# estebanpw/repkiller

Measured on AMD Instinct MI355X. Metric: fragments/sec filtered + achieved HBM GB/s, 50M-frag human self-cmp, 1/2/4/8 GPU, higher is better.
Workload: dtype u64/f64; 1 GPU; cfg3: 50M fragments, 3 Gbp human-scale self-comparison; fragments_per_gpu=50000000, genome_bp=3000000000, parallelism=single GPU

## Files before the change

repkiller_amd/csrc/rk_api.hip:

```cpp
#include <algorithm>
#include <cstdio>
#include <cstdlib>
#include <cstring>
#include <string>
#include <vector>

#include "rk_ctx.h"

namespace rk {
const char *const kKernelNames[KID_COUNT] = {
    "k_prep_keys",     "k_digit_hist",      "k_digit_scatter", "k_gather_proc",
    "k_sort_keys",     "k_csr_fill_x",      "k_run_bounds",    "k_sweep_tile",
    "k_sweep_fast",    "k_sweep_fast_more", "k_sweep_wave",    "k_csr_fill_y",    "k_jump",
    "k_assign_gid",    "k_group_offsets",   "k_build_records",
    "k_sort_small",    "k_sort_groups_reg", "k_sort_groups_lds", "k_sort_groups_split",
    "k_emit",          "k_part (sharded)", "exchange (sharded)", "k_aux (sharded)",
    "k_row_keys (sharded)", "k_fill_y (sharded)", "k_y_results (sharded)", "k_x_own (sharded)",
    "k_merge_yx (sharded)", "k_sort_segments", "k_sweep_long32", "k_nw_order_hist",
    "k_onesweep", "k_nw_xchunk", "k_nw_fill_y", "k_nw_assign", "k_nw_xcount", "k_nw_x_bits",
    "k_heap_segments", "k_seg_fine (order)", "k_seg_fine (members)", "k_seg_fine (Y)",
};
}

namespace rk {

void collect_kernel_timing(rk_ctx *ctx) {
  g_ktimer = nullptr;
  if (ctx->kt.n) (void)hipEventSynchronize(ctx->kt.ev[2 * ctx->kt.n - 1]);
  if (ctx->kt.tier_counts) {
    const uint32_t nb = ctx->kt.tier_nblk;
    std::vector<uint32_t> h((size_t)KernelTimer::TIERS * nb);
    if (hipMemcpy(h.data(), ctx->kt.tier_counts, (size_t)GS_NTIER * nb * 4,
                  hipMemcpyDeviceToHost) == hipSuccess) {
      for (int u = 0; u < GS_NTIER; ++u) {
        double mem = 0;
        for (uint32_t b = 0; b < nb; ++b) mem += h[(size_t)u * nb + b];
        const int sl = ctx->kt.tier_slot[u];
        if (sl >= 0 && sl < ctx->kt.n) ctx->kt.bytes[sl] = 12.0 * mem;
        const int s2 = u == GS_NTIER - 1 ? ctx->kt.tier_slot[GS_NTIER] : -1;
        if (s2 >= 0 && s2 < ctx->kt.n) ctx->kt.bytes[s2] = 12.0 * mem;
      }
    }
    ctx->kt.tier_counts = nullptr;
  }
  bool any_units = false;
  for (int i = 0; i < ctx->kt.n; ++i) any_units |= ctx->kt.unit_bytes[i] > 0.0;
  if (any_units) {
    std::vector<uint32_t> u(ctx->kt.n);
    if (hipMemcpy(u.data(), ctx->kt.units, (size_t)ctx->kt.n * 4, hipMemcpyDeviceToHost) ==
        hipSuccess)
      for (int i = 0; i < ctx->kt.n; ++i)
        if (ctx->kt.unit_bytes[i] > 0.0) ctx->kt.bytes[i] = ctx->kt.unit_bytes[i] * u[i];
  }
  for (int i = 0; i < ctx->kt.n; ++i) {
    float ms = 0;
    if (hipEventElapsedTime(&ms, ctx->kt.ev[2 * i], ctx->kt.ev[2 * i + 1]) == hipSuccess) {
      const int k = ctx->kt.kid[i];
      ctx->kt_ms[k] += ms;
      ctx->kt_bytes[k] += ctx->kt.bytes[i];
      ctx->kt_launches[k]++;
    }
  }
  ctx->kt.n = 0;
}

int readback(rk_ctx *ctx, const uint32_t *dev, uint32_t count) {
  ++ctx->readbacks;
  HIPCHK(ctx, hipMemcpyAsync(ctx->host, dev, count * sizeof(uint32_t), hipMemcpyDeviceToHost,
                             ctx->stream));
  HIPCHK(ctx, hipStreamSynchronize(ctx->stream));
  return RK_OK;
}

int err_status(rk_ctx *ctx, uint32_t bits) {
  if (bits & ERRB_UB_BUCKET) {
    ctx->err = "xStart/10 >= vsize: the reference indexes FragmentsDatabase out of bounds "
               "(FragmentsDatabase.cpp:96-97)";
    return RK_E_UB_BUCKET;
  }
  if (bits & ERRB_UB_CENTER) {
    ctx->err = "a fragment centre probes past an occupancy array "
               "(SequenceOcupationList.cpp:17,80)";
    return RK_E_UB_CENTER;
  }
  if (bits & ERRB_INTERNAL) {
    ctx->err = "device consistency check failed";
    return RK_E_INTERNAL;
  }
  return RK_OK;
}

int resolve_axis(rk_ctx *ctx, const Axis &ax, SweepScratch sc, bool fast32, uint32_t *sweeps) {
  uint32_t *counters = sc.counters;
  uint8_t *rpend = sc.rpend;
  RunList rl{sc.runs, sc.wpend, 0, 0, fast32};
  build_runs(ax, rl, sc.dev_count, ctx->host + 128, ctx->stream);
  HIPCHK(ctx, hipGetLastError());
  if (!fast32) HIPCHK(ctx, hipMemsetAsync(rpend, 1, ax.m, ctx->stream));
  *sweeps = 0;
  for (;;) {
    if (*sweeps > ax.m + 2) {
      ctx->err = "occupancy sweeps did not converge";
      return RK_E_INTERNAL;
    }
    occupancy_sweep(ax, rl, rpend, counters, *sweeps == 0, ctx->stream);
    HIPCHK(ctx, hipGetLastError());
    ++*sweeps;
    static const uint32_t blind = [] {
      const char *e = getenv("RK_SWEEP_BLIND");
      const int v = e ? atoi(e) : 3;
      return (uint32_t)(v < 1 ? 1 : v > 8 ? 8 : v);
    }();
    if (*sweeps < blind && ax.m > 0) continue;
    int rc = readback(ctx, counters, PEND_WORDS);
    if (rc) return rc;
    uint64_t pending = 0;
    for (uint32_t k = 0; k < PEND_WORDS; ++k) pending += ctx->host[k];
    if (!pending) break;
  }
  return RK_OK;
}

__global__ void k_pend_flag(const uint32_t *counters, uint32_t *pend) {
  uint32_t s = 0;
  for (uint32_t k = threadIdx.x; k < PEND_WORDS; k += 64) s |= counters[k];
  if (__ballot(s != 0) && threadIdx.x == 0) *pend = 1u;
}

int resolve_axis_queued(rk_ctx *ctx, const Axis &ax, SweepScratch sc, uint32_t sweeps,
                        uint32_t *pend, uint32_t *junk) {
  if (!ax.m) return RK_OK;
  RunList rl{sc.runs, sc.wpend, 0, 0, true};
  build_runs(ax, rl, sc.dev_count, ctx->host + 128, ctx->stream);
  for (uint32_t s = 0; s < sweeps; ++s)
    occupancy_sweep(ax, rl, sc.rpend, junk && s + 1 < sweeps ? junk : sc.counters, s == 0,
                    ctx->stream, !junk);
  if (pend) k_pend_flag<<<1, 64, 0, ctx->stream>>>(sc.counters, pend);
  HIPCHK(ctx, hipGetLastError());
  return RK_OK;
}

}

static const char *kPhaseNames[RK_N_PHASES] = {
    "prep_keys",      "order_csr",  "gather_proc", "occupancy_csr", "sweep_x", "sweep_y",
    "group_roots",    "member_csr", "group_sort",  "emit",
};

namespace {

using rk::align_up;
using rk::Carve;
using rk::readback;
using rk::err_status;

struct Plan {
  uint64_t n, vsize, max_x, max_y;
  uint32_t nbx, nby;
};

struct Work {
  uint32_t *ctrl;
  uint32_t *pkey_in, *tk, *tv, *tk2, *tv2;
  uint32_t *radix, *radix2;
  size_t radix_words;
  rk::Proc p;
  rk::Csr cx, cy;
  uint32_t *isnew, *newrank, *sgid, *gmem, *goff, *tag, *otag;
  void *gsort;
  uint64_t *reckey;
  uint32_t *rpend, *runs, *rlen_at, *rbeg_at;
  uint8_t *wpend;
  uint32_t *scan;
  size_t scan_cap;
};

size_t carve(Carve &c, const Plan &pl, Work &w) {
  const size_t n = pl.n + 1;
  w.ctrl = c.take<uint32_t>(64 + rk::PEND_WORDS);
  w.pkey_in = c.take<uint32_t>(n);
  w.tk = c.take<uint32_t>(n);
  w.tv = c.take<uint32_t>(n);
  w.tk2 = c.take<uint32_t>(n);
  w.tv2 = c.take<uint32_t>(n);
  w.radix_words = rk::radix_scratch_words((uint32_t)n);
  w.radix = c.take<uint32_t>(w.radix_words);
  w.radix2 = c.take<uint32_t>(w.radix_words);
  w.p.rec = c.take<ulonglong2>(2 * n + 64);
  {
    char *r = reinterpret_cast<char *>(w.p.rec);
    const size_t o1 = rk::align_up(16 * n + 64), o2 = o1 + rk::align_up(8 * n + 64),
                 o3 = o2 + rk::align_up(4 * n + 64);
    w.p.hrec = reinterpret_cast<ulonglong2 *>(r);
    w.reckey = reinterpret_cast<uint64_t *>(r + o1);
    w.tag = reinterpret_cast<uint32_t *>(r + o2);
    w.otag = reinterpret_cast<uint32_t *>(r + o3);
  }
  w.p.ys = c.take<uint64_t>(n);
  w.p.pkey = c.take<uint32_t>(n);
  w.p.row = c.take<uint32_t>(n);
  w.p.xrec = c.take<ulonglong2>(n);
  w.p.yrec = c.take<ulonglong2>(n);
  w.p.ylenhi = nullptr;
  w.p.keyx = c.take<uint32_t>(n);
  w.p.keyy = c.take<uint32_t>(n);
  w.p.par = c.take<uint32_t>(n);
  w.p.gid = c.take<uint32_t>(n);
  w.p.grow = nullptr;
  for (rk::Csr *cs : {&w.cx, &w.cy}) {
    cs->key = c.take<uint32_t>(n);
    cs->ent = c.take<uint32_t>(n);
    cs->cen = cs->len = nullptr;
    cs->state = c.take<uint8_t>(n);
    cs->pk = c.take<uint2>(n);
    cs->nbd = c.take<uint8_t>(n);
  }
  w.isnew = c.take<uint32_t>(n);
  w.newrank = c.take<uint32_t>(n);
  w.sgid = c.take<uint32_t>(n);
  w.gmem = c.take<uint32_t>(n);
  w.goff = c.take<uint32_t>(n);
  w.gsort = c.take<uint8_t>(rk::groupsort_scratch_bytes((uint32_t)n));
  w.rpend = c.take<uint32_t>(n / 4 + 1);
  w.wpend = c.take<uint8_t>(n / 64 + 1);
  w.runs = c.take<uint32_t>(rk::runs_scratch_words((uint32_t)n));
  w.rlen_at = c.take<uint32_t>(n);
  w.rbeg_at = c.take<uint32_t>(n);
  w.scan_cap = rk::scan_blocks(n + 1) + 64;
  w.scan = c.take<uint32_t>(w.scan_cap);
  return c.off;
}

int ensure_ws(rk_ctx *ctx, const Plan &pl, Work &w) {
  Carve probe{nullptr};
  size_t need = carve(probe, pl, w);
  if (need > ctx->ws_cap) {
    if (ctx->ws) (void)hipFree(ctx->ws);
    ctx->ws = nullptr;
    ctx->ws_cap = 0;
    hipError_t e = hipMalloc(&ctx->ws, need);
    if (e != hipSuccess) {
      ctx->err = std::string("workspace hipMalloc(") + std::to_string(need) + "): " +
                 hipGetErrorString(e);
      return e == hipErrorOutOfMemory ? RK_E_NOMEM : RK_E_HIP;
    }
    ctx->ws_cap = need;
  }
  Carve real{(char *)ctx->ws};
  carve(real, pl, w);
  return RK_OK;
}

rk::SweepScratch sweep_scratch(const Work &w) {
  return rk::SweepScratch{w.runs, w.wpend, reinterpret_cast<uint8_t *>(w.rpend), w.ctrl + 64,
                          w.ctrl + 2};
}

int ensure_wide(rk_ctx *ctx, size_t n1, Work &w) {
  const size_t n = n1 + 1;
  auto carve_wide = [&](Carve &c) {
    w.p.ylenhi = c.take<uint32_t>(n);
    w.cx.cen = c.take<uint64_t>(n);
    w.cx.len = c.take<uint64_t>(n);
    w.cy.cen = c.take<uint64_t>(n);
    w.cy.len = c.take<uint64_t>(n);
  };
  Carve probe{nullptr};
  carve_wide(probe);
  const size_t need = probe.off;
  if (need > ctx->ws_wide_cap) {
    if (ctx->ws_wide) (void)hipFree(ctx->ws_wide);
    ctx->ws_wide = nullptr;
    ctx->ws_wide_cap = 0;
    hipError_t e = hipMalloc(&ctx->ws_wide, need);
    if (e != hipSuccess) {
      ctx->err = std::string("64-bit workspace hipMalloc: ") + hipGetErrorString(e);
      return e == hipErrorOutOfMemory ? RK_E_NOMEM : RK_E_HIP;
    }
    ctx->ws_wide_cap = need;
  }
  Carve c{(char *)ctx->ws_wide};
  carve_wide(c);
  return RK_OK;
}

void mark(rk_ctx *ctx, int ph) {
  if (!ctx->profiling) return;
  if (ph == RK_PH_PREP) {
    ctx->kt.n = 0;
    rk::g_ktimer = &ctx->kt;
  }
  (void)hipEventRecord(ctx->pev[ph], ctx->stream);
  ctx->pev_used[ph] = true;
}

void collect_phases(rk_ctx *ctx) {
  if (!ctx->profiling) return;
  rk::collect_kernel_timing(ctx);
  (void)hipEventSynchronize(ctx->pev[RK_N_PHASES]);
  for (int ph = 0; ph < RK_N_PHASES; ++ph) {
    if (!ctx->pev_used[ph]) continue;
    int nx = ph + 1;
    while (nx <= RK_N_PHASES && !ctx->pev_used[nx]) ++nx;
    if (nx > RK_N_PHASES) break;
    float ms = 0;
    if (hipEventElapsedTime(&ms, ctx->pev[ph], ctx->pev[nx]) == hipSuccess) {
      ctx->phase_ms[ph] += ms;
      ctx->phase_calls[ph]++;
    }
  }
  for (auto &u : ctx->pev_used) u = false;
}

struct NWork {
  uint32_t *ctrl, *ahist, *yhist, *ehist;
  uint32_t *astatus, *ystatus, *xcnt, *xoff;
  uint4 *Ra, *Rb, *yrec, *erec;
  rk::Csr cx, cy;
  uint32_t *xpos, *xbits;
  uint32_t *par, *isnew, *newrank, *sgid, *tag, *otag, *mrow, *goff;
  uint64_t *reckey;
  void *gsort;
  uint32_t *rpend, *runs, *rlen_at, *rbeg_at;
  uint8_t *wpend;
  uint32_t *scan;
  size_t scan_cap;
  uint32_t *chist, *coff;
};

size_t carve_nw(Carve &c, uint64_t n1, uint32_t nbx, NWork &w) {
  const size_t n = n1 + 1;
  const size_t sw = rk::nw_status_words((uint32_t)n);
  w.astatus = c.take<uint32_t>(sw);
  w.ystatus = c.take<uint32_t>(sw);
  w.xcnt = c.take<uint32_t>((size_t)3 * (nbx / 64 + 2) + 64);
  w.xoff = c.take<uint32_t>((size_t)3 * (nbx / 64 + 2) + 64);
  w.Ra = c.take<uint4>(n);
  w.Rb = c.take<uint4>(n);
  w.yrec = c.take<uint4>(n);
  w.erec = c.take<uint4>(n);
  for (rk::Csr *cs : {&w.cx, &w.cy}) {
    cs->key = c.take<uint32_t>(n);
    cs->ent = c.take<uint32_t>(n);
    cs->cen = cs->len = nullptr;
    cs->state = c.take<uint8_t>(n);
    cs->pk = c.take<uint2>(n);
    cs->nbd = c.take<uint8_t>(n);
  }
  w.xpos = c.take<uint32_t>(n);
  w.xbits = c.take<uint32_t>(n / 32 + 2);
  w.par = c.take<uint32_t>(n);
  w.isnew = c.take<uint32_t>(n);
  w.newrank = c.take<uint32_t>(n);
  w.sgid = c.take<uint32_t>(n);
  w.tag = c.take<uint32_t>(n);
  w.otag = c.take<uint32_t>(n);
  w.mrow = c.take<uint32_t>(n);
  w.goff = c.take<uint32_t>(n);
  w.reckey = c.take<uint64_t>(n);
  w.gsort = c.take<uint8_t>(rk::groupsort_scratch_bytes((uint32_t)n));
  w.rpend = c.take<uint32_t>(n / 4 + 1);
  w.wpend = c.take<uint8_t>(n / 64 + 1);
  w.runs = c.take<uint32_t>(rk::runs_scratch_words((uint32_t)n));
  w.rlen_at = c.take<uint32_t>(n);
  w.rbeg_at = c.take<uint32_t>(n);
  w.scan_cap = rk::scan_blocks(n + 1) + 64;
  w.scan = c.take<uint32_t>(w.scan_cap);
  w.chist = c.take<uint32_t>(rk::nw_seg_words(n));
  w.coff = c.take<uint32_t>(rk::nw_seg_words(n));
  return c.off;
}

constexpr size_t NW_CTRL_WORDS = 64 + 3 * rk::PEND_WORDS;
constexpr size_t NW_SMALL_WORDS = NW_CTRL_WORDS + 3 * 4096;

int ensure_nw_small(rk_ctx *ctx, NWork &w) {
  if (!ctx->nw_small) {
    const hipError_t e = hipMalloc(&ctx->nw_small, NW_SMALL_WORDS * sizeof(uint32_t));
    if (e != hipSuccess) {
      ctx->nw_small = nullptr;
      ctx->err = std::string("record-pipeline control hipMalloc: ") + hipGetErrorString(e);
      return e == hipErrorOutOfMemory ? RK_E_NOMEM : RK_E_HIP;
    }
  }
  w.ctrl = static_cast<uint32_t *>(ctx->nw_small);
  w.ahist = w.ctrl + NW_CTRL_WORDS;
  w.yhist = w.ahist + 4096;
  w.ehist = w.ahist + 8192;
  return RK_OK;
}

int ensure_nw(rk_ctx *ctx, uint64_t n, uint32_t nbx, NWork &w) {
  Carve probe{nullptr};
  const size_t need = carve_nw(probe, n, nbx, w);
  if (need > ctx->ws_nw_cap) {
    if (ctx->ws_nw) (void)hipFree(ctx->ws_nw);
    ctx->ws_nw = nullptr;
    ctx->ws_nw_cap = 0;
    hipError_t e = hipMalloc(&ctx->ws_nw, need);
    if (e == hipErrorOutOfMemory && (ctx->ws || ctx->ws_wide)) {
      (void)hipGetLastError();
      if (ctx->ws) (void)hipFree(ctx->ws);
      if (ctx->ws_wide) (void)hipFree(ctx->ws_wide);
      ctx->ws = ctx->ws_wide = nullptr;
      ctx->ws_cap = ctx->ws_wide_cap = 0;
      e = hipMalloc(&ctx->ws_nw, need);
    }
    if (e != hipSuccess) {
      ctx->err = std::string("record-pipeline workspace hipMalloc(") + std::to_string(need) +
                 "): " + hipGetErrorString(e);
      return e == hipErrorOutOfMemory ? RK_E_NOMEM : RK_E_HIP;
    }
    ctx->ws_nw_cap = need;
  }
  Carve real{(char *)ctx->ws_nw};
  carve_nw(real, n, nbx, w);
  return RK_OK;
}

bool record_pipeline_enabled() {
  static const bool on = [] {
    const char *e = std::getenv("RK_RECORD_PIPELINE");
    return !(e && e[0] == '0');
  }();
  return on;
}

int classify_narrow(rk_ctx *ctx, const rk_frags_soa *in, const rk_params *prms, uint32_t npairs,
                    rk_result *outs, const Plan &pl, bool *fallback, const uint3 *wire,
                    bool fused_roots = true) {
  *fallback = false;
  static const bool fused_on = [] {
    const char *e = getenv("RK_ROOTS_FUSED");
    return !(e && e[0] == '0');
  }();
  fused_roots = fused_roots && fused_on;
  const uint32_t n = (uint32_t)pl.n;
  NWork w{};
  int rc = ensure_nw_small(ctx, w);
  if (rc) return rc;
  hipStream_t st = ctx->stream, st2 = ctx->stream2;
  ctx->stats.n_in = n;
  const rk::NwDigits ad = rk::nw_plan(rk::bit_length(pl.vsize - 1));
  const rk::NwOrderPlan op = rk::nw_order_split(n, pl.vsize, rk::bit_length(pl.vsize - 1),
                                                 rk::NW_SEG_CAP_ORDER);
  const bool split = op.coarse.passes > 0;
  static const int bits12 = [] {
    const char *e = getenv("RK_NW_YBITS");
    const int b = e ? atoi(e) : 9;
    return b < 8 ? 8 : b > 9 ? 9 : b;
  }();
  const rk::NwDigits yd = rk::nw_plan(rk::bit_length(2ull * pl.nby - 1), bits12);
  static const bool ysplit_on = [] {
    const char *e = getenv("RK_NW_YSPLIT");
    return !(e && e[0] == '0');
  }();
  static const bool y_overlap = [] {
    const char *e = getenv("RK_Y_OVERLAP");
    return e && e[0] == '1';
  }();
  const rk::NwOrderPlan yp = ysplit_on && !y_overlap
                                 ? rk::nw_order_split(n, 2ull * pl.nby,
                                                      rk::bit_length(2ull * pl.nby - 1),
                                                      rk::NW_SEG_CAP_Y)
                                 : rk::NwOrderPlan{};
  const bool ysplit = yp.coarse.passes > 0;

  bool early = false;
  if (split && !ctx->nw_fell_back) {
    Carve probe{nullptr};
    NWork tmpw = w;
    early = carve_nw(probe, pl.n, pl.nbx, tmpw) <= ctx->ws_nw_cap;
  }
  rk::ZeroRegion cr[4] = {};
  if (early) {
    if ((rc = ensure_nw(ctx, pl.n, pl.nbx, w))) return rc;
    rk::nw_order_coarse_regions(
        (uint32_t)pl.n, op, w.astatus, w.chist,
        rk::ZeroRegion{w.xcnt, ((size_t)3 * (pl.nbx / 64 + 2) + 1) * sizeof(uint32_t)}, cr);
  }
  HIPCHK(ctx, hipEventRecord(ctx->ev0, st));
  rk::zero_regions(st, {{w.ctrl, (64 + 2 * rk::PEND_WORDS) * sizeof(uint32_t)},
                        {w.ahist, 3 * 4096 * sizeof(uint32_t)}, cr[0], cr[1], cr[2], cr[3]});
  mark(ctx, RK_PH_PREP);
  rk::nw_order_hist(*in, pl.vsize, pl.max_x, pl.max_y, pl.nby, split ? op.coarse : ad,
                    ysplit ? yp.coarse : yd, w.ahist, w.yhist, w.ctrl, st, wire);
  HIPCHK(ctx, hipGetLastError());
  if (early) {
    HIPCHK(ctx, hipMemcpyAsync(ctx->host, w.ctrl, 9 * sizeof(uint32_t), hipMemcpyDeviceToHost,
                               st));
    HIPCHK(ctx, hipEventRecord(ctx->aux, st));
    mark(ctx, RK_PH_ORDER);
    rk::nw_order_sort_split_coarse(*in, op, w.ahist, w.astatus, w.Ra, w.Rb, w.chist,
                                   rk::ZeroRegion{}, pl.vsize, st, wire, true);
    HIPCHK(ctx, hipGetLastError());
    HIPCHK(ctx, hipEventSynchronize(ctx->aux));
  } else if ((rc = readback(ctx, w.ctrl, 9))) {
    return rc;
  }
  if ((rc = err_status(ctx, ctx->host[0]))) return rc;
  if (ctx->host[3]) {
    *fallback = true;
    ctx->stats.record_fallback = 1;
    ctx->nw_fell_back = true;
    return RK_OK;
  }
  ctx->nw_fell_back = false;
  if (!early && (rc = ensure_nw(ctx, pl.n, pl.nbx, w))) return rc;
  rk::ScanScratch ss{w.scan, w.scan_cap};
  const uint32_t m = ctx->host[1], maxlen = ctx->host[4];
  ctx->stats.n_proc = m;
  for (uint32_t q = 0; q < npairs; ++q) outs[q].n_out = m, outs[q].n_groups = 0;
  if (m == 0) {
    mark(ctx, RK_N_PHASES);
    collect_phases(ctx);
    HIPCHK(ctx, hipEventRecord(ctx->ev1, st));
    HIPCHK(ctx, hipStreamSynchronize(st));
    return RK_OK;
  }
  rk::NwChunkCounts cc{};
  cc.W = rk::nw_chunk_width(m, pl.nbx);
  while ((1u << cc.lgW) < cc.W) ++cc.lgW;
  cc.nch = rk::nw_chunks(pl.nbx, cc.W);
  cc.cnts = w.xcnt;
  if (!early) mark(ctx, RK_PH_ORDER);
  if (early) {
    rk::nw_order_sort_split_fine((uint32_t)pl.n, m, pl.nby, op, w.Ra, w.Rb, w.yrec, w.erec,
                                 w.chist, w.coff, ss, &cc, st);
  } else if (split) {
    rk::nw_order_sort_split(*in, m, pl.nby, op, w.ahist, w.astatus, w.Ra, w.Rb, w.yrec, w.erec,
                            w.chist, w.coff, ss, &cc, pl.vsize, st, wire);
  } else {
    rk::nw_order_sort(*in, pl.vsize, pl.nby, ad, w.ahist, w.astatus, w.Ra, w.Rb, w.yrec, st, wire);
    rk::nw_x_count(w.Ra, m, cc, st);
  }
  rk::exclusive_scan_u32(w.xcnt, w.xoff, (size_t)3 * cc.nch + 1, ss, st);
  HIPCHK(ctx, hipGetLastError());
  if (y_overlap) {
    HIPCHK(ctx, hipEventRecord(ctx->fork, st));
    HIPCHK(ctx, hipStreamWaitEvent(st2, ctx->fork, 0));
    rk::nw_y_sort_head(w.yrec, w.Rb, m, yd, w.yhist, w.ystatus, st2);
    HIPCHK(ctx, hipEventRecord(ctx->join, st2));
  }
  mark(ctx, RK_PH_GATHER);
  rk::nw_x_chunks(w.Ra, m, pl.nbx, pl.max_x, maxlen, w.xoff, w.cx, w.xpos, w.erec, w.ctrl, cc.W,
                  st);
  if (ctx->batch_tables) rk::batch_nbd(*ctx->batch_tables, false, w.cx, m, pl.nbx, st);
  HIPCHK(ctx, hipGetLastError());
  mark(ctx, RK_PH_OCC_CSR);
  rk::SweepScratch sc{w.runs, w.wpend, reinterpret_cast<uint8_t *>(w.rpend), w.ctrl + 64,
                      w.ctrl + 2};
  rk::SweepScratch scy = sc;
  scy.counters = w.ctrl + 64 + rk::PEND_WORDS;
  uint32_t *const junk = w.ctrl + 64 + 2 * rk::PEND_WORDS;
  static const bool queued_on = [] {
    const char *e = getenv("RK_SWEEP_QUEUED");
    return !(e && e[0] == '0');
  }();
  static const uint32_t blind = [] {
    const char *e = getenv("RK_SWEEP_BLIND");
    const int v = e ? atoi(e) : 3;
    return (uint32_t)(v < 1 ? 1 : v > 8 ? 8 : v);
  }();
  for (uint32_t q = 0; q < npairs; ++q) {
    const rk_params &pq = prms[q];
    rk_result *out = &outs[q];
    const bool prof = q == 0;
    uint32_t rounds = 0, G = 0;
    bool narrow_keys = true;
    for (int attempt = 0; attempt < 2; ++attempt) {
    const bool queued = queued_on && attempt == 0;
    if (q > 0 || attempt > 0) HIPCHK(ctx, hipMemsetAsync(w.cx.state, rk::ST_UNKNOWN, m, st));
    if (queued && q > 0)
      rk::zero_regions(st, {{w.ctrl + 10, 2 * sizeof(uint32_t)},
                            {w.ctrl + 64, 2 * rk::PEND_WORDS * sizeof(uint32_t)}});
    if (prof) mark(ctx, RK_PH_SWEEP_X);
    rk::Axis ax{w.cx.key, w.cx.ent, nullptr, nullptr, w.cx.state, nullptr, w.par,
                w.cx.pk, w.cx.nbd, w.rlen_at, w.rbeg_at, m, pl.max_x, pq.len_ratio,
                pq.pos_ratio};
    uint32_t sweeps = blind;
    if ((rc = queued ? rk::resolve_axis_queued(ctx, ax, sc, blind,
                                               fused_roots ? nullptr : w.ctrl + 10, junk)
                     : rk::resolve_axis(ctx, ax, sc, true, &sweeps)))
      return rc;
    ctx->stats.x_sweeps = sweeps;
    if (prof) mark(ctx, RK_PH_SWEEP_Y);
    rk::nw_x_bits(w.xpos, w.cx.state, m, w.xbits, st);
    if (q == 0 && attempt == 0 && y_overlap) {
      HIPCHK(ctx, hipStreamWaitEvent(st, ctx->join, 0));
      rk::nw_y_sort_tail(w.yrec, w.Rb, m, yd, w.yhist, w.ystatus, w.cy, pl.nby, pl.max_y,
                         w.xbits, st);
    } else if (q == 0 && attempt == 0 && ysplit) {
      rk::nw_y_sort_split_after_x(w.yrec, w.Rb, w.Ra, m, yp, w.yhist, w.ystatus, w.cy, pl.nby,
                                  pl.max_y, w.xbits, w.chist, w.coff, ss, st);
    } else if (q == 0 && attempt == 0) {
      rk::nw_y_sort_after_x(w.yrec, w.Rb, m, yd, w.yhist, w.ystatus, w.cy, pl.nby, pl.max_y,
                            w.xbits, st);
    } else
      rk::nw_fill_y(w.cy.ent, w.xbits, w.cy.state, m, st);
    if (ctx->batch_tables && q == 0 && attempt == 0)
      rk::batch_nbd(*ctx->batch_tables, true, w.cy, m, pl.nby, st);
    rk::Axis ay{w.cy.key, w.cy.ent, nullptr, nullptr, w.cy.state, nullptr, w.par,
                w.cy.pk, w.cy.nbd, w.rlen_at, w.rbeg_at, m, pl.max_y, pq.len_ratio,
                pq.pos_ratio};
    ay.par_dev = true;
    sweeps = blind;
    if ((rc = queued ? rk::resolve_axis_queued(ctx, ay, scy, blind,
                                               fused_roots ? nullptr : w.ctrl + 11, junk)
                     : rk::resolve_axis(ctx, ay, sc, true, &sweeps)))
      return rc;
    ctx->stats.y_sweeps = sweeps;

    if (prof) mark(ctx, RK_PH_ROOTS);
    rk::Proc pr{};
    pr.par = w.par;
    rounds = 0;
    G = 0;
    bool open_axes = false;
    if (fused_roots) {
      rk::zero_regions(st, {{q > 0 ? w.ehist : nullptr, 4096 * sizeof(uint32_t)},
                            {q > 0 ? w.ctrl + 12 : nullptr, sizeof(uint32_t)}});
      rk::exclusive_scan_roots(w.par, m, w.newrank, ss, st, w.ctrl + 32);
      if ((rc = readback(ctx, w.ctrl + 5, 64 - 5 + 2 * rk::PEND_WORDS))) return rc;
      uint32_t pending = 0;
      for (uint32_t k = 0; k < 2 * rk::PEND_WORDS; ++k) pending |= ctx->host[64 - 5 + k];
      if (queued && pending) {
        open_axes = true;
      } else {
        G = ctx->host[27];
        narrow_keys = ctx->host[1] == 0;
        rounds = 1;
      }
    } else {
    rk::zero_regions(st, {{w.isnew + m, sizeof(uint32_t)},
                          {w.ctrl + 5, sizeof(uint32_t)},
                          {q > 0 ? w.ehist : nullptr, 4096 * sizeof(uint32_t)}});
    for (;;) {
      if (rounds > 0) HIPCHK(ctx, hipMemsetAsync(w.ctrl + 5, 0, sizeof(uint32_t), st));
      rk::jump_round(pr, m, w.ctrl + 5, rounds == 0 ? w.isnew : nullptr, w.ctrl, st,
                     queued && rounds == 0 ? w.ctrl + 10 : nullptr);
      if (rounds == 0) {
        rk::exclusive_scan_u32(w.isnew, w.newrank, (size_t)m + 1, ss, st);
        HIPCHK(ctx, hipMemcpyAsync(w.ctrl + 32, w.newrank + m, sizeof(uint32_t),
                                   hipMemcpyDeviceToDevice, st));
      }
      if ((rc = readback(ctx, w.ctrl + 5, 28))) return rc;
      if (rounds == 0 && queued && (ctx->host[5] || ctx->host[6])) {
        open_axes = true;
        break;
      }
      if (rounds == 0) G = ctx->host[27];
      ++rounds;
      narrow_keys = ctx->host[1] == 0;
      if (!ctx->host[0]) break;
      if (rounds > 64) {
        ctx->err = "pointer jumping did not converge";
        return RK_E_INTERNAL;
      }
    }
    }
    if (!open_axes) break;
    ++ctx->stats.sweep_repeats;
    }
    ctx->stats.jump_rounds = rounds;
    out->n_groups = G;
    ctx->stats.n_groups = G;
    const rk::NwDigits ed = rk::nw_plan(rk::bit_length(G ? G - 1 : 0), narrow_keys ? bits12 : 8);
    static const bool msplit_on = [] {
      const char *e = getenv("RK_NW_MSPLIT");
      return e && e[0] == '1';
    }();
    const rk::NwOrderPlan mp = narrow_keys && msplit_on
                                   ? rk::nw_order_split(m, G, rk::bit_length(G ? G - 1 : 0),
                                                        rk::NW_SEG_CAP_MEMBERS)
                                   : rk::NwOrderPlan{};
    const bool msplit = mp.coarse.passes > 0;
    if (fused_roots)
      rk::nw_assign_jump(w.par, w.newrank, w.isnew, m, msplit ? mp.coarse : ed, w.ehist, w.otag,
                         w.ctrl, st);
    else
      rk::nw_assign(w.par, w.newrank, w.isnew, m, msplit ? mp.coarse : ed, w.ehist, st);

    if (prof) mark(ctx, RK_PH_MEMBERS);
    if (msplit) {
      rk::nw_member_sort_split(w.erec, w.isnew, w.Ra, w.Rb, w.yrec, m, G, mp, w.ehist, w.astatus,
                               w.sgid, w.reckey, w.tag, w.mrow, w.goff, w.chist, w.coff, ss, st);
    } else {
      rk::nw_member_sort(w.erec, w.isnew, w.Ra, w.Rb, m, ed, w.ehist, w.astatus, w.sgid,
                         w.reckey, w.tag, w.mrow, narrow_keys, st);
      rk::group_offsets(w.sgid, m, G, w.goff, st);
    }
    if (prof) mark(ctx, RK_PH_GROUP_SORT);
    if ((rc = rk::sort_groups_exact(w.sgid, w.goff, G, m, w.reckey, w.tag, w.otag, w.gsort, ss,
                                    ctx->host + 128, narrow_keys, st, st2, ctx->fork, ctx->join,
                                    npairs == 1 ? w.ctrl + 33 : nullptr))) {
      ctx->err = "depth-limit heap segments: buffer allocation failed";
      return rc;
    }
    if (prof) mark(ctx, RK_PH_EMIT);
    rk::emit_result(w.otag, w.sgid, w.goff, w.mrow, m, out->gid, out->repval, out->out_order,
                    st);
    HIPCHK(ctx, hipGetLastError());
    if (prof) mark(ctx, RK_N_PHASES);
  }
  HIPCHK(ctx, hipEventRecord(ctx->ev1, st));
  if ((rc = readback(ctx, w.ctrl, npairs == 1 ? 34 : 14))) return rc;
  if (fused_roots && ctx->host[13]) {
    collect_phases(ctx);
    return classify_narrow(ctx, in, prms, npairs, outs, pl, fallback, wire, false);
  }
  if (npairs == 1 && m && ctx->host[33]) {
    const uint32_t G = outs[0].n_groups;
    if ((rc = rk::sort_groups_heap_deferred(G, m, w.reckey, w.tag, w.otag, w.gsort, ctx->host[33],
                                            ctx->host + 128, st))) {
      ctx->err = "depth-limit heap segments: buffer allocation failed";
      return rc;
    }
    rk::emit_result(w.otag, w.sgid, w.goff, w.mrow, m, outs[0].gid, outs[0].repval,
                    outs[0].out_order, st);
    HIPCHK(ctx, hipGetLastError());
    HIPCHK(ctx, hipEventRecord(ctx->ev1, st));
    if ((rc = readback(ctx, w.ctrl, 1))) return rc;
  }
  collect_phases(ctx);
  if ((rc = err_status(ctx, ctx->host[0]))) return rc;
  float ms = 0;
  HIPCHK(ctx, hipEventElapsedTime(&ms, ctx->ev0, ctx->ev1));
  ctx->stats.device_ms = ms;
  ctx->stats.pipeline = 1;
  rk::nw_trace_dump(st);
  return RK_OK;
}

bool record_eligible(const rk_ctx *ctx, uint64_t n) {
  return ctx->pipeline == RK_PIPELINE_AUTO && record_pipeline_enabled() && n > 0 &&
         n < (1ull << 30);
}

int classify_device(rk_ctx *ctx, const rk_frags_soa *in, const rk_params *prms, uint32_t npairs,
                    rk_result *outs, const uint3 *wire = nullptr) {
  if (!ctx || !in || !prms || !outs || npairs == 0) return RK_E_ARG;
  if (in->n >= 0xFFFFFFFFull) return RK_E_TOO_MANY;
  for (uint32_t q = 0; q < npairs; ++q) {
    const rk_params &pq = prms[q];
    if (pq.len_ratio <= 0 || pq.pos_ratio <= 0) {
      ctx->err = "ratios must be greater than zero (commonFunctions.cpp:26-27)";
      return RK_E_ARG;
    }
    if (pq.len_x_hdr != prms[0].len_x_hdr || pq.len_y_hdr != prms[0].len_y_hdr) {
      ctx->err = "all pairs must describe the same fragment set (header lengths differ)";
      return RK_E_ARG;
    }
    if (in->n && (!outs[q].gid || !outs[q].repval || !outs[q].out_order)) return RK_E_ARG;
  }
  if (in->n && !wire && (!in->x_start || !in->y_start || !in->length || !in->strand))
    return RK_E_ARG;
  if (wire && !record_eligible(ctx, in->n)) {
    ctx->err = "wire rows need the record pipeline";
    return RK_E_INTERNAL;
  }
  HIPCHK(ctx, hipSetDevice(ctx->device));
  std::memset(&ctx->stats, 0, sizeof ctx->stats);
  rk::stats_numa_unknown(&ctx->stats);
  hipStream_t st = ctx->stream;
  const rk_params *prm = &prms[0];

  Plan pl{};
  pl.n = in->n;
  const uint64_t len_x = prm->len_x_hdr + 1, len_y = prm->len_y_hdr + 1;
  pl.vsize = 1 + len_x / 10;
  pl.max_x = len_x / 100;
  pl.max_y = len_y / 100;
  if (pl.vsize - 1 >= 0xFFFFFFF0ull || 2 * (pl.max_x + 1) >= 0xFFFFFFF0ull ||
      2 * (pl.max_y + 1) >= 0xFFFFFFF0ull) {
    ctx->err = "sequence length too large for 32-bit bucket ids";
    return RK_E_ARG;
  }
  pl.nbx = (uint32_t)(pl.max_x + 1);
  pl.nby = (uint32_t)(pl.max_y + 1);
  int rc;
  if (record_eligible(ctx, pl.n)) {
    bool fallback = false;
    rc = classify_narrow(ctx, in, prms, npairs, outs, pl, &fallback, wire);
    if (rc || !fallback) return rc;
    if (wire) {
      ctx->err = "wire rows did not pack";
      return RK_E_INTERNAL;
    }
    (void)hipStreamSynchronize(ctx->stream2);
    (void)hipFree(ctx->ws_nw);
    ctx->ws_nw = nullptr;
    ctx->ws_nw_cap = 0;
    if (ctx->profiling) ctx->kt.n = 0;
    const uint32_t why = ctx->stats.record_fallback;
    std::memset(&ctx->stats, 0, sizeof ctx->stats);
    rk::stats_numa_unknown(&ctx->stats);
    ctx->stats.record_fallback = why;
  }
  Work w{};
  rc = ensure_ws(ctx, pl, w);
  if (rc) return rc;
  const uint32_t n = (uint32_t)pl.n;
  rk::ScanScratch ss{w.scan, w.scan_cap};
  ctx->stats.n_in = n;

  HIPCHK(ctx, hipEventRecord(ctx->ev0, st));
  HIPCHK(ctx, hipMemsetAsync(w.ctrl, 0, (64 + rk::PEND_WORDS) * sizeof(uint32_t), st));
  rk::Frags f{in->x_start, in->y_start, in->length, in->strand, n};
  mark(ctx, RK_PH_PREP);

  rk::prep_keys(f, pl.vsize, pl.max_x, pl.max_y, w.pkey_in, w.p.rec, w.ctrl + 1, w.ctrl, st);
  mark(ctx, RK_PH_ORDER);
  rk::radix_sort_pairs(w.pkey_in, nullptr, w.p.pkey, w.p.row, w.tk, w.tv, n,
                       rk::bit_length(pl.vsize - 1), w.radix, w.radix_words, st);
  HIPCHK(ctx, hipGetLastError());
  if ((rc = readback(ctx, w.ctrl, 2))) return rc;
  if ((rc = err_status(ctx, ctx->host[0]))) return rc;
  const bool fast32 = !(ctx->host[0] & rk::ERRB_WIDE_LENGTH);
  const uint32_t m = ctx->host[1];
  ctx->stats.n_proc = m;
  for (uint32_t q = 0; q < npairs; ++q) outs[q].n_out = m, outs[q].n_groups = 0;
  if (m == 0) {
    mark(ctx, RK_N_PHASES);
    collect_phases(ctx);
    HIPCHK(ctx, hipEventRecord(ctx->ev1, st));
    HIPCHK(ctx, hipStreamSynchronize(st));
    return RK_OK;
  }

  mark(ctx, RK_PH_GATHER);
  if (!fast32 && (rc = ensure_wide(ctx, pl.n, w))) return rc;
  rk::gather_proc(f, w.p, m, pl.nbx, pl.nby, st);

  HIPCHK(ctx, hipEventRecord(ctx->fork, st));
  HIPCHK(ctx, hipStreamWaitEvent(ctx->stream2, ctx->fork, 0));
  rk::radix_sort_pairs(w.p.keyy, nullptr, w.cy.key, w.cy.ent, w.tk2, w.tv2, m,
                       rk::bit_length(2ull * pl.nby - 1), w.radix2, w.radix_words, ctx->stream2);
  rk::sort_keys(w.p, m, w.ctrl + 6, ctx->stream2);
  HIPCHK(ctx, hipEventRecord(ctx->join, ctx->stream2));
  mark(ctx, RK_PH_OCC_CSR);
  rk::radix_sort_pairs(w.p.keyx, nullptr, w.cx.key, w.cx.ent, w.tk, w.tv, m,
                       rk::bit_length(2ull * pl.nbx - 1), w.radix, w.radix_words, st);
  rk::csr_fill_x(w.cx, w.p.xrec, m, pl.max_x, st);
  HIPCHK(ctx, hipGetLastError());

  for (uint32_t q = 0; q < npairs; ++q) {
    const rk_params &pq = prms[q];
    rk_result *out = &outs[q];
    const bool prof = q == 0;
    if (q > 0) HIPCHK(ctx, hipMemsetAsync(w.cx.state, rk::ST_UNKNOWN, m, st));

    if (prof) mark(ctx, RK_PH_SWEEP_X);
    rk::Axis ax{w.cx.key, w.cx.ent, w.cx.cen, w.cx.len, w.cx.state,
                reinterpret_cast<uint32_t *>(w.p.yrec), w.p.par,
                w.cx.pk, w.cx.nbd, w.rlen_at, w.rbeg_at, m, pl.max_x, pq.len_ratio,
                pq.pos_ratio};
    uint32_t sweeps = 0;
    if ((rc = rk::resolve_axis(ctx, ax, sweep_scratch(w), fast32, &sweeps))) return rc;
    ctx->stats.x_sweeps = sweeps;
    if (prof) mark(ctx, RK_PH_SWEEP_Y);
    if (q == 0) HIPCHK(ctx, hipStreamWaitEvent(st, ctx->join, 0));
    rk::csr_fill_y(w.cy, w.p.yrec, w.p.ylenhi, m, pl.max_y, st);
    rk::Axis ay{w.cy.key, w.cy.ent, w.cy.cen, w.cy.len, w.cy.state, nullptr, w.p.par,
                w.cy.pk, w.cy.nbd, w.rlen_at, w.rbeg_at, m, pl.max_y, pq.len_ratio,
                pq.pos_ratio};
    ay.par_dev = true;
    if ((rc = rk::resolve_axis(ctx, ay, sweep_scratch(w), fast32, &sweeps))) return rc;
    ctx->stats.y_sweeps = sweeps;

    if (prof) mark(ctx, RK_PH_ROOTS);
    HIPCHK(ctx, hipMemsetAsync(w.isnew + m, 0, sizeof(uint32_t), st));
    uint32_t rounds = 0;
    for (;;) {
      HIPCHK(ctx, hipMemsetAsync(w.ctrl + 5, 0, sizeof(uint32_t), st));
      rk::jump_round(w.p, m, w.ctrl + 5, rounds == 0 ? w.isnew : nullptr, w.ctrl, st);
      if ((rc = readback(ctx, w.ctrl + 5, 2))) return rc;
      ++rounds;
      if (!ctx->host[0]) break;
      if (rounds > 64) {
        ctx->err = "pointer jumping did not converge";
        return RK_E_INTERNAL;
      }
    }
    ctx->stats.jump_rounds = rounds;
    const bool narrow_keys = ctx->host[1] == 0;
    rk::exclusive_scan_u32(w.isnew, w.newrank, (size_t)m + 1, ss, st);
    if ((rc = readback(ctx, w.newrank + m, 1))) return rc;
    const uint32_t G = ctx->host[0];
    out->n_groups = G;
    ctx->stats.n_groups = G;
    rk::assign_gid(w.p, m, w.newrank, st);

    if (prof) mark(ctx, RK_PH_MEMBERS);
    rk::radix_sort_pairs(w.p.gid, nullptr, w.sgid, w.gmem, w.tk, w.tv, m,
                         rk::bit_length(G - 1), w.radix, w.radix_words, st);
    rk::group_offsets(w.sgid, m, G, w.goff, st);
    rk::build_records(w.gmem, w.p.hrec, m, w.reckey, w.tag, st);
    if (prof) mark(ctx, RK_PH_GROUP_SORT);
    if ((rc = rk::sort_groups_exact(w.sgid, w.goff, G, m, w.reckey, w.tag, w.otag, w.gsort, ss,
                                    ctx->host + 128, narrow_keys, st, ctx->stream2, ctx->fork,
                                    ctx->join))) {
      ctx->err = "depth-limit heap segments: buffer allocation failed";
      return rc;
    }
    if (prof) mark(ctx, RK_PH_EMIT);
    rk::emit_result(w.otag, w.sgid, w.goff, w.gmem, m, out->gid, out->repval,
                    out->out_order, st);
    HIPCHK(ctx, hipGetLastError());
    if (prof) mark(ctx, RK_N_PHASES);
  }
  HIPCHK(ctx, hipEventRecord(ctx->ev1, st));
  if ((rc = readback(ctx, w.ctrl, 1))) return rc;
  collect_phases(ctx);
  if ((rc = err_status(ctx, ctx->host[0]))) return rc;
  float ms = 0;
  HIPCHK(ctx, hipEventElapsedTime(&ms, ctx->ev0, ctx->ev1));
  ctx->stats.device_ms = ms;
  ctx->stats.pipeline = 2;
  return RK_OK;
}

}

static hipError_t create_stream2(hipStream_t *s) {
  const char *e = std::getenv("RK_S2_PRIO");
  if (!(e && e[0] == '0')) {
    int least = 0, greatest = 0;
    if (hipDeviceGetStreamPriorityRange(&least, &greatest) == hipSuccess)
      return hipStreamCreateWithPriority(s, hipStreamNonBlocking, greatest);
  }
  return hipStreamCreateWithFlags(s, hipStreamNonBlocking);
}

extern "C" int rk_create(rk_ctx **out, int device) {
  if (!out) return RK_E_ARG;
  *out = nullptr;
  int count = 0;
  if (hipGetDeviceCount(&count) != hipSuccess || count <= 0 || device < 0 || device >= count)
    return RK_E_NODEVICE;
  hipDeviceProp_t prop;
  if (hipGetDeviceProperties(&prop, device) != hipSuccess) return RK_E_NODEVICE;
  if (std::strncmp(prop.gcnArchName, "gfx950", 6) != 0) return RK_E_NODEVICE;
  auto ctx = new (std::nothrow) rk_ctx;
  if (!ctx) return RK_E_NOMEM;
  ctx->device = device;
  const char *one = std::getenv("RK_ONE_STREAM");
  if (hipSetDevice(device) != hipSuccess ||
      hipStreamCreateWithFlags(&ctx->stream, hipStreamNonBlocking) != hipSuccess ||
      (one && one[0] == '1' ? (ctx->stream2 = ctx->stream, hipSuccess)
                            : create_stream2(&ctx->stream2)) !=
          hipSuccess ||
      hipEventCreate(&ctx->ev0) != hipSuccess || hipEventCreate(&ctx->ev1) != hipSuccess ||
      hipEventCreateWithFlags(&ctx->fork, hipEventDisableTiming) != hipSuccess ||
      hipEventCreateWithFlags(&ctx->join, hipEventDisableTiming) != hipSuccess ||
      hipEventCreateWithFlags(&ctx->aux, hipEventDisableTiming) != hipSuccess ||
      hipHostMalloc((void **)&ctx->host, 256 * sizeof(uint32_t), hipHostMallocDefault) !=
          hipSuccess) {
    rk_destroy(ctx);
    return RK_E_HIP;
  }
  if (hipMalloc((void **)&ctx->kt.units, rk::KernelTimer::MAX * sizeof(uint32_t)) != hipSuccess) {
    rk_destroy(ctx);
    return RK_E_HIP;
  }
  for (auto &e : ctx->kt.ev)
    if (hipEventCreateWithFlags(&e, hipEventDisableSystemFence) != hipSuccess) {
      rk_destroy(ctx);
      return RK_E_HIP;
    }
  for (auto &e : ctx->pev)
    if (hipEventCreateWithFlags(&e, hipEventDisableSystemFence) != hipSuccess) {
    rk_destroy(ctx);
    return RK_E_HIP;
  }
  *out = ctx;
  return RK_OK;
}

extern "C" void rk_destroy(rk_ctx *ctx) {
  if (!ctx) return;
  if (ctx->device >= 0) (void)hipSetDevice(ctx->device);
  if (ctx->stream) (void)hipStreamSynchronize(ctx->stream);
  if (ctx->stream2) (void)hipStreamSynchronize(ctx->stream2);
  rk::io_destroy(ctx);
  rk::batch_destroy(ctx);
  if (ctx->ws) (void)hipFree(ctx->ws);
  if (ctx->io) (void)hipFree(ctx->io);
  if (ctx->ws_wide) (void)hipFree(ctx->ws_wide);
  if (ctx->kt.units) (void)hipFree(ctx->kt.units);
  if (ctx->ws_nw) (void)hipFree(ctx->ws_nw);
  if (ctx->nw_small) (void)hipFree(ctx->nw_small);
  for (void *p : ctx->pool.ptr)
    if (p) (void)hipFree(p);
  if (ctx->host) (void)hipHostFree(ctx->host);
  if (ctx->sh_msg) (void)hipHostFree(ctx->sh_msg);
  if (ctx->ev0) (void)hipEventDestroy(ctx->ev0);
  if (ctx->ev1) (void)hipEventDestroy(ctx->ev1);
  for (auto &e : ctx->pev)
    if (e) (void)hipEventDestroy(e);
  for (auto &e : ctx->kt.ev)
    if (e) (void)hipEventDestroy(e);
  if (ctx->fork) (void)hipEventDestroy(ctx->fork);
  if (ctx->join) (void)hipEventDestroy(ctx->join);
  if (ctx->aux) (void)hipEventDestroy(ctx->aux);
  if (ctx->stream2 && ctx->stream2 != ctx->stream) (void)hipStreamDestroy(ctx->stream2);
  if (ctx->stream) (void)hipStreamDestroy(ctx->stream);
  delete ctx;
}

extern "C" const char *rk_last_error(const rk_ctx *ctx) { return ctx ? ctx->err.c_str() : ""; }

extern "C" int rk_set_profiling(rk_ctx *ctx, int enable) {
  if (!ctx) return RK_E_ARG;
  if (enable >= 2 + rk::KID_COUNT) return RK_E_ARG;
  ctx->profiling = enable != 0;
  ctx->kt.only = enable >= 2 ? enable - 2 : -1;
  return RK_OK;
}

extern "C" int rk_get_phase_ms(const rk_ctx *ctx, double *ms, uint32_t *calls) {
  if (!ctx || !ms) return RK_E_ARG;
  for (int i = 0; i < RK_N_PHASES; ++i) {
// ... 240 lines not shown
```

repkiller_amd/csrc/rk_groups.hip:

```cpp
#include "rk_internal.h"

namespace rk {
namespace {

#define GRID_STRIDE(i, n)                                                      \
  for (uint32_t i = blockIdx.x * blockDim.x + threadIdx.x; i < (n);           \
       i += gridDim.x * blockDim.x)

__device__ __forceinline__ uint64_t probe_max_bucket(uint64_t c, uint64_t max_index) {
  uint64_t b = c / 100;
  if (c < max_index && (c + 1) / 100 > b) b = (c + 1) / 100;
  if (c < max_index - 1 && (c + 2) / 100 > b) b = (c + 2) / 100;
  return b;
}

__global__ void k_prep_keys(Frags f, uint64_t vsize, uint64_t max_x, uint64_t max_y,
                            uint32_t *pkey, ulonglong2 *rec, uint32_t *kept, uint32_t *err) {
  uint32_t mine = 0;
  bool wide = false;
  GRID_STRIDE(i, f.n) {
    const uint64_t x = f.x[i];
    wide |= f.len[i] >= 0x80000000ull;
    const uint64_t pk = x / 10;
    if (rec) {
      rec[2 * (size_t)i] = make_ulonglong2(x, f.y[i]);
      rec[2 * (size_t)i + 1] = make_ulonglong2(f.len[i], f.strand[i]);
    }
    uint32_t key = (uint32_t)(vsize - 1);
    if (pk >= vsize) {
      atomicOr(err, ERRB_UB_BUCKET);
    } else if (pk != vsize - 1) {
      const uint64_t h = f.len[i] / 2;
      if (probe_max_bucket(x + h, max_x) > max_x || probe_max_bucket(f.y[i] + h, max_y) > max_y)
        atomicOr(err, ERRB_UB_CENTER);
      key = (uint32_t)pk;
      ++mine;
    }
    pkey[i] = key;
  }
  __shared__ uint32_t part[4];
  for (int off = 32; off > 0; off >>= 1) mine += __shfl_xor(mine, off);
  if ((threadIdx.x & 63) == 0) part[threadIdx.x >> 6] = mine;
  __syncthreads();
  if (threadIdx.x == 0) {
    const uint32_t t = part[0] + part[1] + part[2] + part[3];
    if (t) atomicAdd(kept, t);
  }
  const uint64_t any_wide = __ballot(wide);
  if ((threadIdx.x & 63) == 0 && any_wide) atomicOr(err, ERRB_WIDE_LENGTH);
}

__global__ void k_gather_proc(Proc p, uint32_t m, uint32_t nbx, uint32_t nby) {
  GRID_STRIDE(k, m) {
    const uint32_t r = p.row[k];
    const ulonglong2 a = p.rec[2 * (size_t)r], b = p.rec[2 * (size_t)r + 1];
    const uint64_t x = a.x, y = a.y, L = b.x;
    const uint64_t xc = x + L / 2;
    const uint32_t s = (uint8_t)b.y == 'f' ? 0u : 1u;
    p.ys[k] = y;
    p.xrec[k] = make_ulonglong2(xc, L);
    p.yrec[k] = make_ulonglong2(y + L / 2, L & 0xFFFFFFFFull);
    if (p.ylenhi) p.ylenhi[k] = (uint32_t)(L >> 32);
    if (p.grow) p.grow[k] = (uint32_t)(b.y >> 32);
    p.keyx[k] = s * nbx + (uint32_t)(xc / 100);
    p.keyy[k] = s * nby + (uint32_t)((y + L / 2) / 100);
  }
}

__global__ void __launch_bounds__(256) k_sort_keys(Proc p, uint32_t m, uint32_t *wide) {
  const uint32_t lane = threadIdx.x & 63;
  bool wd = false;
  for (uint32_t base = (blockIdx.x * blockDim.x + threadIdx.x) & ~63u; base < m;
       base += gridDim.x * blockDim.x) {
    const uint32_t k = base + lane;
    const bool in = k < m;
    const uint32_t key = in ? p.pkey[k] : 0u;
    const uint64_t y = in ? p.ys[k] : 0ull;
    const bool end = in && (k + 1 == m || p.pkey[k + 1] != key);
    const uint64_t ends = __ballot(end) & ~((1ull << lane) - 1ull);
    const int src = ends ? __ffsll((unsigned long long)ends) - 1 : 63;
    uint64_t d = __shfl(y, src);
    if (__ballot(in && !ends)) {
      const uint32_t klast = __shfl(key, 63);
      uint32_t e = 0;
      for (uint32_t b = base + 64;; b += 64) {
        const uint32_t q = b + lane;
        const uint64_t stop = __ballot(q >= m || p.pkey[q] != klast);
        if (stop) {
          e = b + __builtin_ctzll(stop) - 1;
          break;
        }
      }
      if (in && !ends) d = p.ys[e];
    }
    const uint64_t h = y > d ? y - d : d - y;
    if (in) p.hrec[k] = make_ulonglong2(h, p.row[k]);
    wd |= in && (h >> 32) != 0;
  }
  if (__ballot(wd) && lane == 0 && *(volatile uint32_t *)wide == 0) atomicOr(wide, 1u);
}

__device__ __forceinline__ uint8_t nbd_code(uint64_t c, uint64_t max_index) {
  const int d = neighbour_dir(c, max_index);
  return d < 0 ? 1 : d > 0 ? 2 : 0;
}

__global__ void k_csr_fill_x(Csr c, const ulonglong2 *xrec, uint32_t m, uint64_t max_index) {
  GRID_STRIDE(q, m) {
    const ulonglong2 r = xrec[c.ent[q]];
    if (c.cen) c.cen[q] = r.x, c.len[q] = r.y;
    c.pk[q] = make_uint2((uint32_t)r.x, (uint32_t)r.y);
    c.nbd[q] = nbd_code(r.x, max_index);
    c.state[q] = ST_UNKNOWN;
  }
}

__global__ void k_csr_fill_y(Csr c, const ulonglong2 *yrec, const uint32_t *ylenhi, uint32_t m,
                             uint64_t max_index) {
  GRID_STRIDE(q, m) {
    const size_t k = c.ent[q];
    const ulonglong2 a = yrec[k];
    if (c.cen) {
      c.cen[q] = a.x;
      c.len[q] = (a.y & 0xFFFFFFFFull) | (ylenhi ? (uint64_t)ylenhi[k] << 32 : 0ull);
    }
    c.pk[q] = make_uint2((uint32_t)a.x, (uint32_t)a.y);
    c.nbd[q] = nbd_code(a.x, max_index);
    c.state[q] = (uint32_t)(a.y >> 32) != NONE ? ST_ACTIVE : ST_UNKNOWN;
  }
}

__global__ void k_group_offsets_unaligned(const uint32_t *sgid, uint32_t m, uint32_t ngroups,
                                          uint32_t *goff) {
  GRID_STRIDE(q, m) {
    if (q == 0 || sgid[q] != sgid[q - 1]) goff[sgid[q]] = q;
  }
  if (blockIdx.x == 0 && threadIdx.x == 0) goff[ngroups] = m;
}
__global__ void __launch_bounds__(256) k_group_offsets(const uint32_t *sgid, uint32_t m,
                                                        uint32_t ngroups, uint32_t *goff) {
  const uint32_t nq = (m + 3) / 4;
  for (uint32_t t = blockIdx.x * blockDim.x + threadIdx.x; t < nq; t += gridDim.x * blockDim.x) {
    const uint32_t q0 = t * 4;
    uint32_t g[4];
    if (q0 + 4 <= m) {
      const uint4 v = *reinterpret_cast<const uint4 *>(sgid + q0);
      g[0] = v.x, g[1] = v.y, g[2] = v.z, g[3] = v.w;
    } else {
#pragma unroll
      for (int j = 0; j < 4; ++j) g[j] = q0 + j < m ? sgid[q0 + j] : 0u;
    }
    uint32_t prev = q0 ? sgid[q0 - 1] : ~0u;
#pragma unroll
    for (int j = 0; j < 4; ++j) {
      if (q0 + j < m && g[j] != prev) goff[g[j]] = q0 + j;
      prev = g[j];
    }
  }
  if (blockIdx.x == 0 && threadIdx.x == 0) goff[ngroups] = m;
}

__global__ void k_jump(Proc p, uint32_t m, uint32_t *changed, uint32_t *isnew, uint32_t *err,
                       const uint32_t *open) {
  if (open && (open[0] | open[1])) return;
  bool ch = false;
  GRID_STRIDE(k, m) {
    const uint32_t a0 = p.par[k];
    uint32_t a = a0;
    if (isnew && a > k) {
      atomicOr(err, ERRB_INTERNAL);
      a = k;
      p.par[k] = k;
    }
    if (isnew) isnew[k] = a == k;
    int step = 0;
    for (; step < 32; ++step) {
      const uint32_t b = p.par[a];
      if (b == a) break;
      a = b;
    }
    if (a != a0) p.par[k] = a;
    if (step == 32) ch = true;
  }
  if (ch) *changed = 1u;
}

__global__ void k_jump_list(Proc p, uint32_t m, uint32_t *isnew, uint32_t *err, uint32_t *list,
                            uint32_t *count) {
  const uint32_t lane = threadIdx.x & 63;
  for (uint32_t k = blockIdx.x * blockDim.x + threadIdx.x; k - lane < m;
       k += gridDim.x * blockDim.x) {
    bool open = false;
    if (k < m) {
      const uint32_t a0 = p.par[k];
      uint32_t a = a0;
      if (a > k) {
        atomicOr(err, ERRB_INTERNAL);
        a = k;
        p.par[k] = k;
      }
      isnew[k] = a == k;
      int step = 0;
      for (; step < 32; ++step) {
        const uint32_t b = p.par[a];
        if (b == a) break;
        a = b;
      }
      if (a != a0) p.par[k] = a;
      open = step == 32;
    }
    const uint64_t b = __ballot(open);
    if (b) {
      uint32_t at = 0;
      if (lane == 0) at = atomicAdd(count, (uint32_t)__popcll(b));
      at = (uint32_t)__shfl((int)at, 0);
      if (open) list[at + __popcll(b & ((1ull << lane) - 1ull))] = k;
    }
  }
}

__global__ void k_jump_rest(Proc p, const uint32_t *list, const uint32_t *count,
                            uint32_t *changed) {
  const uint32_t n = *count;
  bool ch = false;
  for (uint32_t i = blockIdx.x * blockDim.x + threadIdx.x; i < n; i += gridDim.x * blockDim.x) {
    const uint32_t k = list[i];
    uint32_t a = p.par[k];
    int step = 0;
    for (; step < 4096; ++step) {
      const uint32_t b = p.par[a];
      if (b == a) break;
      a = b;
    }
    p.par[k] = a;
    ch |= step == 4096;
  }
  if (ch) *changed = 1u;
}

__global__ void k_assign_gid(Proc p, uint32_t m, const uint32_t *newrank) {
  GRID_STRIDE(k, m) p.gid[k] = newrank[p.par[k]];
}

__global__ void k_build_records(uint32_t *gmem, const ulonglong2 *hrec, uint32_t m,
                                uint64_t *key, uint32_t *tag) {
  GRID_STRIDE(t, m) {
    const ulonglong2 r = hrec[gmem[t]];
    key[t] = r.x;
    tag[t] = t;
    gmem[t] = (uint32_t)r.y;
  }
}

__global__ void k_emit(const uint32_t *otag, const uint32_t *sgid, const uint32_t *goff,
                       const uint32_t *mrow, uint32_t m, uint32_t *out_gid, uint8_t *out_rep,
                       uint32_t *out_order) {
  GRID_STRIDE(t, m) {
    const uint32_t g = sgid[t];
    const uint32_t o = otag[t];
    const uint32_t b = goff[g], e = goff[g + 1];
    out_order[t] = mrow[e - b == 1 ? t : o];
    out_gid[t] = g;
    out_rep[t] = e - b == 1 ? 0 : (t == b ? 1 : 2);
  }
}

}

void prep_keys(const Frags &f, uint64_t vsize, uint64_t max_x, uint64_t max_y, uint32_t *pkey,
               ulonglong2 *rec, uint32_t *kept, uint32_t *err, hipStream_t st) {
  if (f.n)
  {
    kt_begin(st, KID_PREP);
    k_prep_keys<<<grid_for(f.n, 256, 2048), 256, 0, st>>>(f, vsize, max_x, max_y, pkey, rec, kept,
                                                           err);
    kt_end(st, KID_PREP, (rec ? 61.0 : 29.0) * f.n);
  }
}
void gather_proc(const Frags &f, Proc p, uint32_t m, uint32_t nbx, uint32_t nby, hipStream_t st) {
  if (!m) return;
  (void)f;
  kt_begin(st, KID_GATHER);
  k_gather_proc<<<grid_for(m, 256), 256, 0, st>>>(p, m, nbx, nby);
  kt_end(st, KID_GATHER, 84.0 * m);
}
void sort_keys(Proc p, uint32_t m, uint32_t *wide, hipStream_t st) {
  if (!m) return;
  kt_begin(st, KID_SORT_KEYS);
  k_sort_keys<<<grid_for(m, 256), 256, 0, st>>>(p, m, wide);
  kt_end(st, KID_SORT_KEYS, 32.0 * m);
}
void csr_fill_x(Csr c, const ulonglong2 *xrec, uint32_t m, uint64_t max_index, hipStream_t st) {
  if (!m) return;
  kt_begin(st, KID_CSR_FILL_X);
  k_csr_fill_x<<<grid_for(m, 256), 256, 0, st>>>(c, xrec, m, max_index);
  kt_end(st, KID_CSR_FILL_X, (c.cen ? 46.0 : 30.0) * m);
}
void csr_fill_y(Csr c, const ulonglong2 *yrec, const uint32_t *ylenhi, uint32_t m,
                uint64_t max_index, hipStream_t st) {
  if (!m) return;
  kt_begin(st, KID_CSR_FILL_Y);
  k_csr_fill_y<<<grid_for(m, 256), 256, 0, st>>>(c, yrec, ylenhi, m, max_index);
  kt_end(st, KID_CSR_FILL_Y, (c.cen ? 46.0 : 30.0) * m);
}
void group_offsets(const uint32_t *sgid, uint32_t m, uint32_t ngroups, uint32_t *goff,
                   hipStream_t st) {
  kt_begin(st, KID_GROUP_OFFSETS);
  if ((reinterpret_cast<uintptr_t>(sgid) & 15) == 0)
    k_group_offsets<<<grid_for((m + 3) / 4, 256, 16384), 256, 0, st>>>(sgid, m, ngroups, goff);
  else
    k_group_offsets_unaligned<<<grid_for(m, 256), 256, 0, st>>>(sgid, m, ngroups, goff);
  kt_end(st, KID_GROUP_OFFSETS, 4.0 * m + 4.0 * ngroups);
}
void jump_round(Proc p, uint32_t m, uint32_t *changed, uint32_t *isnew, uint32_t *err,
                hipStream_t st, const uint32_t *open) {
  if (!m) return;
  kt_begin(st, KID_JUMP);
  k_jump<<<grid_for(m, 256, (size_t)1 << 20), 256, 0, st>>>(p, m, changed, isnew, err, open);
  kt_end(st, KID_JUMP, (isnew ? 16.0 : 12.0) * m);
}
void jump_listed(Proc p, uint32_t m, uint32_t *isnew, uint32_t *err, uint32_t *list,
                 uint32_t *count, uint32_t *changed, hipStream_t st) {
  if (!m) return;
  (void)hipMemsetAsync(count, 0, 4, st);
  kt_begin(st, KID_JUMP);
  k_jump_list<<<grid_for(m, 256, (size_t)1 << 20), 256, 0, st>>>(p, m, isnew, err, list, count);
  kt_end(st, KID_JUMP, 16.0 * m);
  kt_begin(st, KID_JUMP);
  k_jump_rest<<<1024, 256, 0, st>>>(p, list, count, changed);
  kt_end(st, KID_JUMP, 0.0);
}
void assign_gid(Proc p, uint32_t m, const uint32_t *newrank, hipStream_t st) {
  if (!m) return;
  kt_begin(st, KID_ASSIGN_GID);
  k_assign_gid<<<grid_for(m, 256), 256, 0, st>>>(p, m, newrank);
  kt_end(st, KID_ASSIGN_GID, 12.0 * m);
}
void build_records(uint32_t *gmem, const ulonglong2 *hrec, uint32_t m, uint64_t *key,
                   uint32_t *tag, hipStream_t st) {
  if (!m) return;
  kt_begin(st, KID_BUILD_RECORDS);
  k_build_records<<<grid_for(m, 256), 256, 0, st>>>(gmem, hrec, m, key, tag);
  kt_end(st, KID_BUILD_RECORDS, 36.0 * m);
}
void emit_result(const uint32_t *otag, const uint32_t *sgid, const uint32_t *goff,
                 const uint32_t *mrow, uint32_t m, uint32_t *out_gid, uint8_t *out_rep,
                 uint32_t *out_order, hipStream_t st) {
  if (!m) return;
  kt_begin(st, KID_EMIT);
  k_emit<<<grid_for(m, 256), 256, 0, st>>>(otag, sgid, goff, mrow, m, out_gid, out_rep,
                                           out_order);
  kt_end(st, KID_EMIT, 29.0 * m);
}

}
```

repkiller_amd/csrc/rk_groupsort.hip:

```cpp
#include "rk_internal.h"

#include <algorithm>
#include <cstdio>
#include <cstdlib>
#include <vector>

namespace rk {
namespace {

constexpr int THRESH = 16;

__device__ __forceinline__ void wave_sync() {
  __builtin_amdgcn_fence(__ATOMIC_SEQ_CST, "wavefront");
  __builtin_amdgcn_wave_barrier();
  __builtin_amdgcn_fence(__ATOMIC_SEQ_CST, "wavefront");
}

__device__ __forceinline__ void wave_sync_global() {
  __builtin_amdgcn_fence(__ATOMIC_RELEASE, "agent");
  __builtin_amdgcn_wave_barrier();
  __builtin_amdgcn_fence(__ATOMIC_ACQUIRE, "agent");
}

template <bool GLOBAL>
__device__ __forceinline__ void sync_mem() {
  if (GLOBAL) wave_sync_global();
  else wave_sync();
}

template <class KT_, class PT_, class TT_ = uint32_t>
struct ViewT {
  using key_t = KT_;
  using tag_t = TT_;
  KT_ *K;
  TT_ *T;
  PT_ *PL, *PR;
  uint8_t *B;
};
using GView = ViewT<uint64_t, uint32_t>;

template <class V>
__device__ __forceinline__ void vswap(const V &v, uint32_t a, uint32_t b) {
  const typename V::key_t k = v.K[a];
  v.K[a] = v.K[b];
  v.K[b] = k;
  const uint32_t t = v.T[a];
  v.T[a] = v.T[b];
  v.T[b] = t;
}

template <class V>
__device__ __forceinline__ void median_to_first(const V &v, uint32_t f, uint32_t l) {
  const uint32_t a = f + 1, b = f + (l - f) / 2, c = l - 1;
  const typename V::key_t ka = v.K[a], kb = v.K[b], kc = v.K[c];
  uint32_t m;
  if (ka < kb) m = kb < kc ? b : (ka < kc ? c : a);
  else m = ka < kc ? a : (kb < kc ? c : b);
  vswap(v, f, m);
}

template <class V>
__device__ void adjust_heap(const V &v, uint32_t base, long hole, long len,
                            typename V::key_t vk, uint32_t vt) {
  const long top = hole;
  long child = hole;
  typename V::key_t *K = v.K + base;
  typename V::tag_t *T = v.T + base;
  while (child < (len - 1) / 2) {
    child = 2 * (child + 1);
    if (K[child] < K[child - 1]) child--;
    K[hole] = K[child];
    T[hole] = T[child];
    hole = child;
  }
  if ((len & 1) == 0 && child == (len - 2) / 2) {
    child = 2 * (child + 1);
    K[hole] = K[child - 1];
    T[hole] = T[child - 1];
    hole = child - 1;
  }
  long parent = (hole - 1) / 2;
  while (hole > top && K[parent] < vk) {
    K[hole] = K[parent];
    T[hole] = T[parent];
    hole = parent;
    parent = (hole - 1) / 2;
  }
  K[hole] = vk;
  T[hole] = vt;
}

template <class V>
__device__ void heap_sort_segment(const V &v, uint32_t f, uint32_t l) {
  const long len = (long)(l - f);
  if (len >= 2) {
    for (long parent = (len - 2) / 2;; --parent) {
      adjust_heap(v, f, parent, len, v.K[f + parent], v.T[f + parent]);
      if (parent == 0) break;
    }
  }
  for (long last = len; last > 1;) {
    --last;
    const typename V::key_t vk = v.K[f + last];
    const uint32_t vt = v.T[f + last];
    v.K[f + last] = v.K[f];
    v.T[f + last] = v.T[f];
    adjust_heap(v, f, 0, last, vk, vt);
  }
  if (v.B)
    for (uint32_t x = f; x < l; ++x) v.B[x] = 2;
}

constexpr uint32_t HEAP_BLOCK_MIN = 2048;
constexpr int HLV = 13;
#if defined(__HIP_DEVICE_COMPILE__) && !defined(__gfx950__)
#error "rk_groupsort.hip: k_heap_segments needs gfx950 (160 KB of LDS per workgroup)"
#endif
constexpr uint32_t HTOP = (1u << HLV) - 1;
constexpr int HR = 6;
constexpr uint32_t HR_LAST = (1u << HR) - 2, HR_NODES = (2u << HR) - 2;
static_assert(HR_NODES <= 128, "two logical nodes per lane");
constexpr int HRMAX = 6;

struct HeapMem {
  uint64_t *K;
  uint32_t *T;
  uint64_t *lk;
  uint32_t *lt;
  __device__ __forceinline__ uint64_t key(uint32_t x) const {
    uint64_t v = lk[x < HTOP ? x : HTOP];
    if (x >= HTOP) v = K[x];
    return v;
  }
  __device__ __forceinline__ uint32_t tag(uint32_t x) const {
    uint32_t v = lt[x < HTOP ? x : HTOP];
    if (x >= HTOP) v = T[x];
    return v;
  }
  __device__ __forceinline__ void put(uint32_t x, uint64_t k, uint32_t t) const {
    const uint32_t y = x < HTOP ? x : HTOP;
    lk[y] = k, lt[y] = t;
    if (x >= HTOP) K[x] = k, T[x] = t;
  }
};

__device__ void wave_sort_heap(const HeapMem &h, uint32_t n, uint32_t lane) {
  for (uint32_t last = n - 1; last > 0; --last) {
    const uint64_t vk = h.key(last);
    const uint32_t vt = h.tag(last);
    const uint64_t rk = h.key(0);
    const uint32_t rt = h.tag(0);
    if (lane == 0) h.put(last, rk, rt);
    const uint32_t len = last;
    const uint32_t two_lim = (len - 1) / 2;
    uint64_t pm0[HRMAX], pm1[HRMAX];
    uint64_t k0[HRMAX], k1[HRMAX];
    uint32_t t0[HRMAX], t1[HRMAX];
    uint32_t x0[HRMAX], x1[HRMAX];
    uint32_t hole = 0;
    int rounds = 0;
    bool more = true;
#pragma unroll
    for (int r = 0; r < HRMAX; ++r) {
      pm0[r] = pm1[r] = 0;
      k0[r] = k1[r] = 0;
      t0[r] = t1[r] = 0;
      x0[r] = x1[r] = 0;
      if (!more) continue;
      ++rounds;
      uint64_t kk[2];
      uint32_t tt[2], xx[2];
#pragma unroll
      for (int s = 0; s < 2; ++s) {
        const uint32_t c = lane + 64 * s;
        const int d = 31 - __clz((int)(c + 2));
        const uint64_t pos = ((uint64_t)hole + 1) * (1ull << d) - 1 + (c + 2 - (1u << d));
        const bool in = c < HR_NODES && pos < len;
        xx[s] = in ? (uint32_t)pos : 0u;
        kk[s] = in ? h.key((uint32_t)pos) : 0ull;
        tt[s] = in ? h.tag((uint32_t)pos) : 0u;
      }
      uint64_t dir[2];
#pragma unroll
      for (int s = 0; s < 2; ++s) {
        const uint32_t lo = (uint32_t)kk[s], hi = (uint32_t)(kk[s] >> 32);
        const uint64_t sib = (uint64_t)(uint32_t)__shfl_xor((int)hi, 1) << 32 |
                             (uint32_t)__shfl_xor((int)lo, 1);
        dir[s] = __ballot((lane & 1) && !(kk[s] < sib));
      }
      uint32_t J = 0, x = hole;
      more = false;
      for (;;) {
        if (x >= two_lim) {
          if ((len & 1) == 0 && x == (len - 2) / 2) {
            const uint32_t c = 2 * J;
            if (c < 64) pm0[r] |= 1ull << c;
            else pm1[r] |= 1ull << (c - 64);
          }
          break;
        }
        const uint32_t cr = 2 * J + 1;
        const bool right = ((cr < 64 ? dir[0] >> cr : dir[1] >> (cr - 64)) & 1ull) != 0;
        const uint32_t c = right ? cr : cr - 1;
        if (c < 64) pm0[r] |= 1ull << c;
        else pm1[r] |= 1ull << (c - 64);
        x = 2 * x + (right ? 2 : 1);
        if (c >= HR_LAST) {
          hole = x;
          more = true;
          break;
        }
        J = c + 1;
      }
      k0[r] = kk[0], k1[r] = kk[1];
      t0[r] = tt[0], t1[r] = tt[1];
      x0[r] = xx[0], x1[r] = xx[1];
    }
    uint32_t D = 0, below = 0;
#pragma unroll
    for (int r = 0; r < HRMAX; ++r) {
      if (r >= rounds) break;
      D += __popcll(pm0[r]) + __popcll(pm1[r]);
      below += __popcll(__ballot(((pm0[r] >> lane) & 1) && k0[r] < vk)) +
               __popcll(__ballot(((pm1[r] >> lane) & 1) && k1[r] < vk));
    }
    const uint32_t j = D - below;
    uint32_t before = 0;
    const uint64_t lt = (1ull << lane) - 1ull;
#pragma unroll
    for (int r = 0; r < HRMAX; ++r) {
      if (r >= rounds) break;
      const bool on0 = (pm0[r] >> lane) & 1, on1 = (pm1[r] >> lane) & 1;
      const uint32_t p0 = before + __popcll(pm0[r] & lt) + 1;
      const uint32_t p1 = before + __popcll(pm0[r]) + __popcll(pm1[r] & lt) + 1;
      if (on0 && p0 <= j) {
        h.put((x0[r] - 1) / 2, k0[r], t0[r]);
        if (p0 == j) h.put(x0[r], vk, vt);
      }
      if (on1 && p1 <= j) {
        h.put((x1[r] - 1) / 2, k1[r], t1[r]);
        if (p1 == j) h.put(x1[r], vk, vt);
      }
      before += __popcll(pm0[r]) + __popcll(pm1[r]);
    }
    if (j == 0 && lane == 0) h.put(0, vk, vt);
    wave_sync();
  }
}

__device__ void wave_sort_heap_equal(uint32_t *T, uint32_t n, uint32_t lane) {
  auto sp = [](uint32_t j) { return (2ull << j) - 2; };
  uint32_t s = lane < 32 && sp(lane) < n ? T[sp(lane)] : 0u;
  uint32_t L = n - 1, m = 0;
  while (sp(m) < (L - 1) / 2) ++m;
  uint32_t head = 0, pv = 0;
  bool pend = false;
  int64_t B = L;
  auto ld = [&](int64_t q) { return T[q >= 0 ? q : 0]; };
  uint32_t ca = ld(B - lane), cb = ld(B - 64 - lane), cc = ld(B - 128 - lane), ob = 0;
  __builtin_amdgcn_s_waitcnt(0);
  auto chunk = [&](const uint32_t c0, const uint32_t c1) {
    auto at = [&](int64_t q) {
      const int i = (int)(B - q);
      return (uint32_t)(i < 64 ? __builtin_amdgcn_readlane((int)c0, i)
                               : __builtin_amdgcn_readlane((int)c1, i - 64));
    };
    const int64_t lo = B - 63;
    const int64_t shrink_at = m > 0 ? (int64_t)(2 * sp(m - 1) + 2) : -1;
    const int64_t special_at = (int64_t)(2 * sp(m) + 2);
    const int kb = 31 - __clz((int)(B + 2));
    const bool spine_in = ((1ll << kb) - 2) >= lo;
    if (lo >= 1 && !pend && shrink_at < lo && !(special_at >= lo && special_at <= B) && !spine_in) {
      const uint32_t mp1 = m + 1, hl = head + lane;
      const uint32_t from_s = (uint32_t)__shfl((int)s, (int)(hl < mp1 ? hl : hl - mp1));
      const uint32_t from_c = (uint32_t)__shfl((int)c0, (int)(lane - mp1) & 63);
      const uint32_t ring = (uint32_t)__shfl((int)c0, (int)(64 - mp1 + lane) & 63);
      ob = lane < mp1 ? from_s : from_c;
      s = lane < mp1 ? ring : s;
      head = 0;
      L -= 64;
    }
    for (; L > 0 && B - L < 64; --L) {
      while (m > 0 && sp(m - 1) >= (L - 1) / 2) {
        s = (uint32_t)__shfl((int)s, lane <= m ? (int)((head + lane) % (m + 1)) : (int)lane);
        head = 0;
        --m;
      }
      uint32_t v;
      if (pend) v = pv;
      else if (((L + 2) & (L + 1)) == 0)
        v = (uint32_t)__builtin_amdgcn_readlane((int)s, 30 - __clz((int)(L + 2)));
      else v = at(L);
      const uint32_t root = (uint32_t)__builtin_amdgcn_readlane((int)s, (int)head);
      ob = lane == (uint32_t)(B - L) ? root : ob;
      const bool special = (L & 1) == 0 && sp(m) == (L - 2) / 2;
      const uint32_t bottom = special ? at(L - 1) : v;
      s = lane == head ? bottom : s;
      head = head == m ? 0 : head + 1;
      pend = special;
      pv = v;
    }
    if ((int64_t)lane < B - L) T[B - lane] = ob;
    B -= 64;
  };
  for (;;) {
    chunk(ca, cb);
    if (L == 0) break;
    ca = ld(B - 128 - lane);
    chunk(cb, cc);
    if (L == 0) break;
    cb = ld(B - 128 - lane);
    chunk(cc, ca);
    if (L == 0) break;
    cc = ld(B - 128 - lane);
  }
  if (lane == 0) T[0] = (uint32_t)__builtin_amdgcn_readlane((int)s, (int)head);
}

__device__ void block_make_heap(uint64_t *K, uint32_t *T, uint32_t n) {
  const uint32_t tid = threadIdx.x;
  if (n < 2) return;
  const uint32_t last_parent = (n - 2) / 2;
  for (int lv = 31 - __clz((int)(last_parent + 1)); lv >= 0; --lv) {
    const uint32_t a = (1u << lv) - 1;
    const uint32_t e = min((1u << (lv + 1)) - 2, last_parent);
    for (uint32_t x = a + tid; x <= e; x += blockDim.x)
      adjust_heap(GView{K, T, nullptr, nullptr, nullptr}, 0, x, n, K[x], T[x]);
    __syncthreads();
  }
}

__device__ void block_heap_sort(uint64_t *K, uint32_t *T, uint32_t n, uint32_t *out, uint64_t *lk,
                                uint32_t *lt) {
  const uint32_t tid = threadIdx.x;
  if (n < 2) {
    for (uint32_t x = tid; x < n; x += blockDim.x) out[x] = T[x];
    __syncthreads();
    return;
  }
  int neq = 0;
  for (uint32_t x = tid; x < n; x += blockDim.x) neq |= K[x] != K[0];
  const bool equal = __syncthreads_or(neq) == 0;
  {
    block_make_heap(K, T, n);
    if (equal) {
      if (tid < 64) wave_sort_heap_equal(T, n, tid);
      __syncthreads();
      for (uint32_t x = tid; x < n; x += blockDim.x) out[x] = T[x];
      __syncthreads();
      return;
    }
    for (uint32_t x = tid; x < n && x < HTOP; x += blockDim.x) lk[x] = K[x], lt[x] = T[x];
    __syncthreads();
    if (tid < 64) wave_sort_heap(HeapMem{K, T, lk, lt}, n, tid);
    __syncthreads();
  }
  for (uint32_t x = tid; x < n; x += blockDim.x) out[x] = x < HTOP ? lt[x] : T[x];
  __syncthreads();
}

__device__ __forceinline__ uint32_t pull(int src, uint32_t v) {
  return (uint32_t)__builtin_amdgcn_ds_bpermute(src << 2, (int)v);
}
__device__ __forceinline__ uint64_t pull(int src, uint64_t v) {
  return (uint64_t)pull(src, (uint32_t)v) | (uint64_t)pull(src, (uint32_t)(v >> 32)) << 32;
}
__device__ __forceinline__ uint32_t push(int dst, uint32_t v) {
  return (uint32_t)__builtin_amdgcn_ds_permute(dst << 2, (int)v);
}
__device__ __forceinline__ int below_count(uint64_t m) {
  return (int)__builtin_amdgcn_mbcnt_hi((uint32_t)(m >> 32),
                                        __builtin_amdgcn_mbcnt_lo((uint32_t)m, 0u));
}

template <bool GLOBAL, class KT, class V>
__device__ void reg_sort_core(const V &v, bool in, uint32_t mpos, int &sf, int &sl, int sd,
                              uint32_t lane, KT &k, uint32_t &t, bool &heaped) {
  const int x = (int)lane;
  heaped = false;
  for (;;) {
    bool active = in && !heaped && sl - sf > THRESH;
    const bool need_heap = active && sd == 0;
    if (__ballot(need_heap)) {
      if (in) v.K[mpos] = (typename V::key_t)k, v.T[mpos] = t;
      sync_mem<GLOBAL>();
      if (need_heap && x == sf) heap_sort_segment(v, mpos, mpos + (sl - sf));
      sync_mem<GLOBAL>();
      if (in) k = (KT)v.K[mpos], t = v.T[mpos];
      heaped |= need_heap;
      active &= !need_heap;
    }
    if (!__ballot(active)) break;
    const int len = sl - sf;
    const int a = active ? sf + 1 : x, b = active ? sf + len / 2 : x, c = active ? sl - 1 : x;
    const KT ka = pull(a, k), kb = pull(b, k), kc = pull(c, k);
    int med;
    if (ka < kb) med = kb < kc ? b : (ka < kc ? c : a);
    else med = ka < kc ? a : (kb < kc ? c : b);
    int src = x;
    if (active) src = x == sf ? med : (x == med ? sf : x);
    k = pull(src, k);
    t = pull(src, t);
    const KT p = pull(active ? sf : x, k);
    const uint64_t segm = (sl >= 64 ? ~0ull : (1ull << sl) - 1ull) & ~((1ull << sf) - 1ull);
    const bool lf = active && x > sf && !(k < p);
    const bool rf = active && !(p < k);
    const uint64_t BL = __ballot(lf), BR = __ballot(rf);
    const uint64_t Ls = BL & segm, Rs = BR & segm;
    const int nL = __popcll(Ls), nR = __popcll(Rs);
    const int pL = below_count(BL), pR = below_count(BR);
    const uint64_t lowseg = (1ull << sf) - 1ull;
    const int offL = __popcll(BL & lowseg), offR = __popcll(BR & lowseg);
    const int rl = pL - offL;
    const int rr = nR - 1 - (pR - offR);
    const int rabove = nR - (pR - offR) - (rf ? 1 : 0);
    const uint64_t stopm = __ballot(lf && rabove <= rl) & segm;
    const int lim = nL < nR ? nL : nR;
    const int K = stopm ? __popcll(Ls & ((1ull << __builtin_ctzll(stopm)) - 1ull)) : lim;
    const int nBL = __popcll(BL), nBR = __popcll(BR);
    const uint32_t LL = push(lf ? pL : nBL + (x - pL), (uint32_t)x);
    const uint32_t RL = push(rf ? pR : nBR + (x - pR), (uint32_t)x);
    const bool swl = lf && rl < K, swr = rf && rr < K;
    const int idx = swl ? offR + nR - 1 - rl : swr ? offL + rr : x;
    const uint32_t g = pull(idx, LL | RL << 8);
    const int s2 = swl ? (int)(g >> 8) : swr ? (int)(g & 0xff) : x;
    k = pull(s2, k);
    t = pull(s2, t);
    const uint64_t cm = __ballot((lf && rl == K) || (K > 0 && rf && rr == K - 1)) & segm;
    if (active) {
      const int cut = __builtin_ctzll(cm);
      if (x < cut) sl = cut;
      else sf = cut;
      --sd;
    }
  }
}

template <bool GLOBAL, class KT, class V>
__device__ void reg_finish(const V &v, bool in, int bl, uint32_t bm, int len, int d,
                           uint32_t lane, uint64_t k64, uint32_t t, uint32_t *out,
                           uint32_t tbase) {
  const int x = (int)lane;
  KT k = in ? (KT)k64 : (KT)~(KT)0;
  int sf = in ? bl : x, sl = in ? bl + len : x + 1;
  bool heaped;
  const uint32_t mpos = bm + (uint32_t)(x - bl);
  reg_sort_core<GLOBAL, KT, V>(v, in, mpos, sf, sl, d, lane, k, t, heaped);
  uint32_t r = 0;
  const int my = in && !heaped ? sl - sf : 0;
  for (int j = 0; __ballot(j < my); ++j) {
    const int y = sf + j;
    const KT ky = pull(y < 64 ? y : 63, k);
    r += (j < my) && (ky < k || (ky == k && y < x));
  }
  if (in) {
    out[heaped ? mpos : bm + (uint32_t)(sf - bl) + r] = tbase + t;
    if (v.B) v.B[mpos] = 3;
  }
}

template <bool GLOBAL, class V>
__device__ void reg_batch(const V &v, bool in, int bl, uint32_t bm, int len, int d,
                          uint32_t lane, uint32_t *out, uint32_t tbase = 0) {
  const uint32_t mpos = bm + (uint32_t)((int)lane - bl);
  const uint64_t k = in ? (uint64_t)v.K[mpos] : ~0ull;
  const uint32_t t = in ? (GLOBAL ? mpos : v.T[mpos]) : 0u;
  if (sizeof(typename V::key_t) == 8 && __ballot(in && (k >> 32) != 0))
    reg_finish<GLOBAL, uint64_t, V>(v, in, bl, bm, len, d, lane, k, t, out, tbase);
  else
    reg_finish<GLOBAL, uint32_t, V>(v, in, bl, bm, len, d, lane, k, t, out, tbase);
}

template <int W>
struct GLanes {
  uint32_t lane;
  uint32_t base;
  __device__ __forceinline__ uint64_t ballot(bool p) const {
    return W == 64 ? (uint64_t)__ballot(p) : ((uint64_t)__ballot(p) >> base) & 0xffffffffull;
  }
  __device__ __forceinline__ uint32_t bcast(uint32_t x) const {
    return (uint32_t)__shfl((int)x, (int)base);
  }
};

template <bool GLOBAL, class V, int W>
__device__ uint32_t wave_partition(const V &v, uint32_t f, uint32_t l, GLanes<W> L) {
  const uint32_t lane = L.lane;
  typename V::key_t p = 0;
  if (lane == 0) {
    const uint32_t a = f + 1, b = f + (l - f) / 2, c = l - 1;
    const typename V::key_t ka = v.K[a], kb = v.K[b], kc = v.K[c], kf = v.K[f];
    const uint32_t tf = v.T[f];
    uint32_t m;
    typename V::key_t km;
    if (ka < kb) {
      if (kb < kc) m = b, km = kb;
      else if (ka < kc) m = c, km = kc;
      else m = a, km = ka;
    } else {
      if (ka < kc) m = a, km = ka;
      else if (kb < kc) m = c, km = kc;
      else m = b, km = kb;
    }
    const uint32_t tm = v.T[m];
    v.K[m] = kf;
    v.T[m] = tf;
    v.K[f] = km;
    v.T[f] = tm;
    p = km;
  }
  if (sizeof(p) == 8) {
    const uint64_t p64 = (uint64_t)p;
    p = (typename V::key_t)((uint64_t)L.bcast((uint32_t)p64) |
                            (uint64_t)L.bcast((uint32_t)(p64 >> 32)) << 32);
  } else {
    p = (typename V::key_t)L.bcast((uint32_t)p);
  }
  sync_mem<GLOBAL>();
  const uint64_t lt = (1ull << lane) - 1ull;
  uint32_t nL = 0, nR = 0;
  for (uint32_t c = f; c < l; c += W) {
    const uint32_t x = c + lane;
    const bool in = x < l;
    const typename V::key_t k = in ? v.K[x] : 0;
    const bool lf = in && x > f && !(k < p);
    const bool rf = in && !(p < k);
    const uint64_t bl = L.ballot(lf), br = L.ballot(rf);
    if (lf) v.PL[nL + __popcll(bl & lt)] = x;
    if (rf) v.PR[nR + __popcll(br & lt)] = x;
    nL += __popcll(bl);
    nR += __popcll(br);
  }
  sync_mem<GLOBAL>();
  const uint32_t lim = nL < nR ? nL : nR;
  uint32_t K = lim;
  for (uint32_t c = 0; c < lim; c += W) {
    const uint32_t k = c + lane;
    const bool stop = k < lim && v.PL[k] >= v.PR[nR - 1 - k];
    const uint64_t b = L.ballot(stop);
    if (b) {
      K = c + (uint32_t)__ffsll((unsigned long long)b) - 1;
      break;
    }
  }
  for (uint32_t c = 0; c < K; c += W) {
    const uint32_t k = c + lane;
    if (k < K) vswap(v, v.PL[k], v.PR[nR - 1 - k]);
  }
  uint32_t cut;
  if (K == 0) {
    cut = v.PL[0];
  } else {
    cut = v.PR[nR - K];
    if (K < nL && v.PL[K] < cut) cut = v.PL[K];
  }
  sync_mem<GLOBAL>();
  return cut;
}

template <class KT>
__device__ __forceinline__ KT lane_key(KT k, uint32_t src) {
  if (sizeof(KT) == 8) {
    const uint64_t v = (uint64_t)k;
    return (KT)((uint64_t)(uint32_t)__builtin_amdgcn_readlane((int)(uint32_t)v, (int)src) |
                (uint64_t)(uint32_t)__builtin_amdgcn_readlane((int)(uint32_t)(v >> 32), (int)src)
                    << 32);
  }
  return (KT)(uint32_t)__builtin_amdgcn_readlane((int)(uint32_t)k, (int)src);
}

template <bool GLOBAL, class V>
__device__ uint32_t wave_partition_small(const V &v, uint32_t f, uint32_t l, uint32_t lane) {
  using KT = typename V::key_t;
  const uint32_t len = l - f;
  const bool in = lane < len;
  const uint32_t x = f + (in ? lane : 0u);
  KT k = v.K[x];
  uint32_t t = v.T[x];
  const uint32_t la = 1, lb = len / 2, lc = len - 1;
  const KT ka = lane_key(k, la), kb = lane_key(k, lb), kc = lane_key(k, lc);
  uint32_t mi;
  if (ka < kb) mi = kb < kc ? lb : (ka < kc ? lc : la);
  else mi = ka < kc ? la : (kb < kc ? lc : lb);
  mi = (uint32_t)__builtin_amdgcn_readfirstlane((int)mi);
  const KT k0 = lane_key(k, 0u), p = lane_key(k, mi);
  const uint32_t t0 = (uint32_t)__builtin_amdgcn_readlane((int)t, 0),
                 tm = (uint32_t)__builtin_amdgcn_readlane((int)t, (int)mi);
  if (lane == 0) k = p, t = tm;
  else if (lane == mi) k = k0, t = t0;
  const bool lf = in && lane > 0 && !(k < p);
  const bool rf = in && !(p < k);
  const uint64_t BL = __ballot(lf), BR = __ballot(rf);
  const uint32_t nL = (uint32_t)__popcll(BL), nR = (uint32_t)__popcll(BR);
  const uint32_t pL = (uint32_t)below_count(BL), pR = (uint32_t)below_count(BR);
  const uint32_t ra = nR - pR - (rf ? 1u : 0u);
  const uint64_t SB = __ballot(lf && ra <= pL);
  const uint32_t lim = nL < nR ? nL : nR;
  const uint32_t K =
      SB ? (uint32_t)__popcll(BL & ((1ull << __builtin_ctzll(SB)) - 1ull)) : lim;
  const uint32_t LL = push((int)(lf ? pL : nL + (lane - pL)), lane);
  const uint32_t RL = push((int)(rf ? pR : nR + (lane - pR)), lane);
  const bool swl = lf && pL < K, swr = rf && ra < K;
  const uint32_t g = pull((int)(swl ? nR - 1u - pL : swr ? ra : lane), LL | RL << 8);
  const uint32_t src = swl ? g >> 8 : swr ? g & 0xffu : lane;
  k = pull((int)src, k);
  t = pull((int)src, t);
  if (in) {
    v.K[x] = k;
    v.T[x] = (typename V::tag_t)t;
  }
  const uint64_t cm = __ballot((lf && pL == K) || (K > 0 && rf && ra == K - 1u));
  const uint32_t cut = f + (uint32_t)__builtin_ctzll(cm);
  sync_mem<GLOBAL>();
  return cut;
}

struct Frame {
  uint32_t f, l;
  int d;
};

#ifdef RK_GS_PROF
__device__ unsigned long long g_gs_prof[8];
#define GS_T(k) const uint64_t _g##k = __builtin_amdgcn_s_memtime()
#define GS_ADD(slot, v) do { if (lane == 0) atomicAdd(&g_gs_prof[slot], (unsigned long long)(v)); } while (0)
#else
#define GS_T(k)
#define GS_ADD(slot, v)
#endif

template <bool GLOBAL, class V, int W = 64>
__device__ void wave_std_sort(const V &v, uint32_t n, uint32_t *out, Frame *stack,
                              Frame *smallq, Frame *heapq, GLanes<W> L, int d0,
                              uint32_t reg_max, uint32_t tbase = 0, bool small_part = true) {
  static_assert(W == 64 || W == 32, "a wavefront or a half");
  const uint32_t lane = L.lane;
  if (W != 64) reg_max = 0;
  GS_T(0);
#ifdef RK_GS_PROF
  uint64_t part_cyc = 0, nparts = 0;
#endif
  for (uint32_t x = lane; x < n; x += W) v.B[x] = 0;
  int sp = 0, nsmall = 0, nheap = 0;
  if (lane == 0) stack[0] = {0u, n, d0};
  sp = 1;
  sync_mem<GLOBAL>();
  while (sp) {
    Frame fr = stack[--sp];
    uint32_t f = fr.f, l = fr.l;
    int d = fr.d;
    bool final_leaf = true;
    while (l - f > THRESH) {
      if (d == 0) {
        if (lane == 0) heapq[nheap] = {f, l, 0};
        ++nheap;
        final_leaf = false;
        break;
      }
      if (l - f <= reg_max) {
        if (lane == 0) smallq[nsmall] = {f, l, d};
        ++nsmall;
        final_leaf = false;
        break;
      }
      --d;
#ifdef RK_GS_PROF
      const uint64_t _p0 = __builtin_amdgcn_s_memtime();
#endif
      const uint32_t cut = W == 64 && small_part && l - f <= 64
                               ? wave_partition_small<GLOBAL, V>(v, f, l, lane)
                               : wave_partition<GLOBAL, V, W>(v, f, l, L);
#ifdef RK_GS_PROF
      part_cyc += __builtin_amdgcn_s_memtime() - _p0;
      ++nparts;
#endif
      if (lane == 0) stack[sp] = {cut, l, d};
      ++sp;
      l = cut;
    }
    if (final_leaf && lane == 0) v.B[f] = 1;
    sync_mem<GLOBAL>();
  }
  GS_T(1);
#ifdef RK_GS_PROF
  uint64_t nbatch = 0;
#endif
  for (int q0 = 0; W == 64 && q0 < nsmall;) {
#ifdef RK_GS_PROF
    ++nbatch;
#endif
    int tot = 0, q1 = q0;
    while (q1 < nsmall && tot + (int)(smallq[q1].l - smallq[q1].f) <= 64)
      tot += (int)(smallq[q1].l - smallq[q1].f), ++q1;
    int bl = 0, j = q0;
    while (j + 1 < q1 && (int)lane >= bl + (int)(smallq[j].l - smallq[j].f))
      bl += (int)(smallq[j].l - smallq[j].f), ++j;
    const Frame fr = smallq[j];
    reg_batch<GLOBAL, V>(v, (int)lane < tot, bl, fr.f, (int)(fr.l - fr.f), fr.d, lane, out,
                         tbase);
    q0 = q1;
  }
  sync_mem<GLOBAL>();
  GS_T(2);
  for (int q = (int)lane; q < nheap; q += W) heap_sort_segment(v, heapq[q].f, heapq[q].l);
  sync_mem<GLOBAL>();
  uint32_t carry = 0;
  for (uint32_t c = 0; c < n; c += W) {
    const uint32_t x = c + lane;
    const uint8_t b = x < n ? v.B[x] : 1;
    const uint8_t bn = x + W < n ? v.B[x + W] : 1;
    const uint64_t bd = L.ballot(b != 0), bdn = L.ballot(bn != 0);
    const uint64_t upto = lane == 63 ? ~0ull : (2ull << lane) - 1ull;
    const uint64_t le = bd & upto, gt = bd & ~upto;
    const uint32_t s = le ? c + 63 - (uint32_t)__clzll(le) : carry;
    const uint32_t e = gt ? c + (uint32_t)__builtin_ctzll(gt)
                          : bdn ? c + W + (uint32_t)__builtin_ctzll(bdn) : c + 2 * W;
    if (bd) carry = c + 63 - (uint32_t)__clzll(bd);
    if (x < n && b != 3) {
      if (b == 2) {
        out[x] = tbase + v.T[x];
      } else {
        const typename V::key_t kx = v.K[x];
        uint32_t r = 0;
        typename V::key_t ky[THRESH];
#pragma unroll
        for (int j = 0; j < THRESH; ++j) ky[j] = v.K[s + j < e ? s + j : x];
#pragma unroll
        for (int j = 0; j < THRESH; ++j)
          r += (uint32_t)(s + j < e) &
               ((uint32_t)(ky[j] < kx) | ((uint32_t)(ky[j] == kx) & (uint32_t)(s + j < x)));
        out[s + r] = tbase + v.T[x];
      }
    }
  }
#ifdef RK_GS_PROF
  GS_T(3);
  if (!GLOBAL) {
    GS_ADD(0, _g1 - _g0 - part_cyc);
    GS_ADD(1, part_cyc);
    GS_ADD(2, _g2 - _g1);
    GS_ADD(3, _g3 - _g2);
    GS_ADD(4, nparts);
    GS_ADD(5, nbatch);
    GS_ADD(6, 1);
    GS_ADD(7, n);
  }
#endif
}

struct TierLists {
  const uint32_t *list, *off;
  uint32_t nblk;
  __device__ __forceinline__ void range(int u, uint32_t &lo, uint32_t &hi) const {
    lo = off[(size_t)u * nblk];
    hi = off[(size_t)(u + 1) * nblk];
  }
};

template <int PACK>
__global__ void __launch_bounds__(256) k_sort_groups_reg(TierLists tl, int tier,
                                                         const uint32_t *goff, uint64_t *key,
                                                         uint32_t *tag, uint32_t *otag) {
  constexpr int SPAN = 64 / PACK;
  const uint32_t lane = threadIdx.x & 63;
  const int j = (int)lane / SPAN;
  uint32_t lo, hi;
  tl.range(tier, lo, hi);
  const GView v{key, tag, nullptr, nullptr, nullptr};
  for (uint32_t w = lo + ((blockIdx.x * blockDim.x + threadIdx.x) >> 6) * PACK; w < hi;
       w += ((gridDim.x * blockDim.x) >> 6) * PACK) {
    const bool has = w + j < hi;
    const uint32_t g = has ? tl.list[w + j] : 0u;
    const uint32_t b = has ? goff[g] : 0u, n = has ? goff[g + 1] - b : 0u;
    const int bl = j * SPAN;
    reg_batch<true, GView>(v, (int)lane - bl < (int)n, bl, b, (int)n,
                           n ? 2 * (31 - __clz((int)n)) : 0, lane, otag);
  }
}

__host__ __device__ constexpr uint32_t lds_stack(uint32_t cap) {
  return 2 * (31 - __builtin_clz(cap)) + 4;
}
template <class KT, int WPB, int W = 64>
__global__ void __launch_bounds__(64 * WPB)
__attribute__((amdgpu_waves_per_eu(W == 32 && sizeof(KT) == 4 ? 8 : 1))) k_sort_groups_lds(TierLists tl, int tier,
                                                              const uint32_t *goff,
                                                              const uint64_t *key,
                                                              const uint32_t *tag, uint32_t *otag,
                                                              uint32_t cap, uint32_t reg_max,
                                                              uint32_t slab, bool small_part) {
  extern __shared__ __align__(16) uint8_t smem_all[];
  constexpr uint32_t GPW = 64 / W;
  const uint32_t wl = threadIdx.x & 63,
                 wv = WPB == 1 ? 0u : __builtin_amdgcn_readfirstlane(threadIdx.x >> 6);
  const uint32_t half = W == 64 ? 0u : wl / W;
  const GLanes<W> L{wl & (W - 1), half * W};
  const uint32_t lane = L.lane;
  uint8_t *smem = smem_all + ((size_t)wv * GPW + half) * slab;
  const uint32_t nfr = cap / (THRESH + 1) + 2;
  KT *K = reinterpret_cast<KT *>(smem);
  uint16_t *T = reinterpret_cast<uint16_t *>(K + cap);
  Frame *stack = reinterpret_cast<Frame *>(T + cap);
  Frame *smallq = stack + lds_stack(cap);
  Frame *heapq = reg_max ? smallq + nfr : smallq;
  uint16_t *PL = reinterpret_cast<uint16_t *>(heapq + nfr);
  uint16_t *PR = PL + cap;
  uint8_t *B = reinterpret_cast<uint8_t *>(PR + cap);
  const ViewT<KT, uint16_t, uint16_t> v{K, T, PL, PR, B};
  uint32_t lo, hi;
  tl.range(tier, lo, hi);
  for (uint32_t w = lo + (blockIdx.x * WPB + wv) * GPW + half; w < hi;
       w += gridDim.x * WPB * GPW) {
    const uint32_t g = tl.list[w];
    const uint32_t b = goff[g], n = goff[g + 1] - b;
    for (uint32_t x = lane; x < n; x += W) {
      K[x] = (KT)key[b + x];
      T[x] = (uint16_t)x;
    }
    wave_sync();
    wave_std_sort<false, ViewT<KT, uint16_t, uint16_t>, W>(v, n, otag + b, stack, smallq, heapq,
                                                           L, 2 * (31 - __clz((int)n)), reg_max,
                                                           b, small_part);
    wave_sync();
  }
}

#ifndef RK_SPLIT_T
#define RK_SPLIT_T 512
#endif
constexpr uint32_t SPLIT_T = RK_SPLIT_T;
constexpr int SPLIT_STACK = 72;

struct StopperMap {
  uint32_t off[5];
  uint32_t at[4];
  __device__ __forceinline__ uint32_t pos(const uint32_t *P, uint32_t k) const {
    const uint32_t w = (k >= off[1]) + (k >= off[2]) + (k >= off[3]);
    return P[at[w] + (k - off[w])];
  }
};

__device__ uint32_t block_partition(uint64_t *K, uint32_t *T, uint32_t *PL, uint32_t *PR,
                                    uint32_t f, uint32_t l, uint32_t *s_w) {
  const uint32_t tid = threadIdx.x, lane = tid & 63, wv = tid >> 6;
  if (tid == 0) median_to_first(GView{K, T, nullptr, nullptr, nullptr}, f, l);
  __syncthreads();
  const uint64_t p = K[f];
  const uint32_t len = l - f;
  const uint32_t per = ((len + 3) / 4 + 255) & ~255u;
  const uint32_t a = f + wv * per < l ? f + wv * per : l;
  const uint32_t e = a + per < l ? a + per : l;
  const uint64_t lt = (1ull << lane) - 1ull;
  uint32_t cl = 0, cr = 0;
  for (uint32_t c = a; c < e; c += 256) {
    uint64_t k[4];
#pragma unroll
    for (int u = 0; u < 4; ++u) {
      const uint32_t x = c + 64 * u + lane;
      k[u] = x < e ? K[x] : 0;
    }
#pragma unroll
    for (int u = 0; u < 4; ++u) {
      const uint32_t x = c + 64 * u + lane;
      const bool lf = x < e && x > f && !(k[u] < p);
      const bool rf = x < e && !(p < k[u]);
      const uint64_t bl = __ballot(lf), br = __ballot(rf);
      if (lf) PL[a + cl + __popcll(bl & lt)] = x;
      if (rf) PR[a + cr + __popcll(br & lt)] = x;
      cl += __popcll(bl);
      cr += __popcll(br);
    }
  }
  if (lane == 0) s_w[wv] = cl, s_w[4 + wv] = cr;
  __syncthreads();
  StopperMap ML, MR;
  ML.off[0] = MR.off[0] = 0;
#pragma unroll
  for (uint32_t u = 0; u < 4; ++u) {
    ML.off[u + 1] = ML.off[u] + s_w[u];
    MR.off[u + 1] = MR.off[u] + s_w[4 + u];
    const uint32_t au = f + u * per;
    ML.at[u] = MR.at[u] = au < l ? au : l;
  }
  const uint32_t nL = ML.off[4], nR = MR.off[4];
  const uint32_t lim = nL < nR ? nL : nR;
  uint32_t lo = 0, hi = lim;
  while (lo < hi) {
    const uint32_t span = hi - lo;
    const uint32_t k = lo + (uint32_t)(((uint64_t)span * tid) / 256);
    const bool probe = tid == 0 || k != lo + (uint32_t)(((uint64_t)span * (tid - 1)) / 256);
    const bool stop = probe && ML.pos(PL, k) >= MR.pos(PR, nR - 1 - k);
    if (tid == 0) s_w[8] = 0xFFFFFFFFu;
    __syncthreads();
    if (stop) atomicMin(&s_w[8], k);
    __syncthreads();
    const uint32_t first = s_w[8];
    uint32_t nlo = lo;
    {
      const uint32_t bound = first == 0xFFFFFFFFu ? hi : first;
      const bool f_ok = probe && !stop && k < bound;
      if (tid == 0) s_w[9] = 0;
      __syncthreads();
      if (f_ok) atomicMax(&s_w[9], k + 1);
      __syncthreads();
      nlo = s_w[9] > lo ? s_w[9] : lo;
      hi = bound;
    }
    lo = nlo;
    __syncthreads();
  }
  const uint32_t Kc = lo;
  for (uint32_t k = tid; k < Kc; k += 256) {
    const uint32_t xa = ML.pos(PL, k), xb = MR.pos(PR, nR - 1 - k);
    const uint64_t ka = K[xa];
    K[xa] = K[xb];
    K[xb] = ka;
    const uint32_t ta = T[xa];
    T[xa] = T[xb];
    T[xb] = ta;
  }
  uint32_t cut;
  if (Kc == 0) {
    cut = ML.pos(PL, 0);
  } else {
    cut = MR.pos(PR, nR - Kc);
    if (Kc < nL) {
      const uint32_t c2 = ML.pos(PL, Kc);
      if (c2 < cut) cut = c2;
    }
  }
  __syncthreads();
  return cut;
}

#ifndef RK_QP_PER
#define RK_QP_PER 1
#endif
constexpr int QP_PER = RK_QP_PER;
constexpr uint32_t QP_C = 256 * QP_PER;
constexpr uint32_t QP_CAP = 2 * QP_C;
constexpr uint32_t QP_M = QP_CAP - 1;
struct QPart {
  uint64_t lk[QP_CAP], rk[QP_CAP];
  uint32_t lp[QP_CAP], rp[QP_CAP], lt[QP_CAP], rt[QP_CAP];
  uint32_t cnt[2][QP_PER * 4];
  uint32_t cross[2];
};

__device__ uint32_t block_partition_q(uint64_t *K, uint32_t *T, uint32_t f, uint32_t l,
                                      QPart &q) {
  const uint32_t tid = threadIdx.x, lane = tid & 63, wv = tid >> 6;
  const uint64_t lt = (1ull << lane) - 1ull;
#ifndef RK_QP_FOLD
#define RK_QP_FOLD 1
#endif
  if (!RK_QP_FOLD) {
    if (tid == 0) median_to_first(GView{K, T, nullptr, nullptr, nullptr}, f, l);
    __syncthreads();
  }
  const uint32_t ca = f + 1, cb = f + (l - f) / 2, cc = l - 1;
  const uint64_t ka = K[ca], kb = K[cb], kc = K[cc], k0 = K[f];
  const uint32_t ta = T[ca], tb = T[cb], tc = T[cc], t0 = T[f];
  uint32_t lpos = f + 1, rpos = l;
  uint32_t qlh = 0, qlt = 0, qrh = 0, qrt = 0;
  uint32_t lastR = 0;
  uint64_t ak[QP_PER], bk[QP_PER];
  uint32_t at[QP_PER], bt[QP_PER];
  uint32_t m = 0xFFFFFFFFu, fp = 0xFFFFFFFFu;
  uint64_t p = 0;
  uint32_t tm = 0;
  auto load_left = [&]() {
#pragma unroll
    for (int u = 0; u < QP_PER; ++u) {
      const uint32_t x = lpos + 256 * u + tid;
      const bool ok = x < l;
      const uint64_t k = ok ? K[x] : 0;
      const uint32_t t = ok ? T[x] : 0;
      ak[u] = x == m ? k0 : k;
      at[u] = x == m ? t0 : t;
    }
  };
  auto load_right = [&]() {
#pragma unroll
    for (int u = 0; u < QP_PER; ++u) {
      const uint32_t o = 256 * u + tid;
      const bool ok = o < rpos - f;
      const uint32_t x = ok ? rpos - 1 - o : f;
      const uint64_t k = ok ? K[x] : 0;
      const uint32_t t = ok ? T[x] : 0;
      bk[u] = x == m ? k0 : (x == fp ? p : k);
      bt[u] = x == m ? t0 : (x == fp ? tm : t);
    }
  };
  load_left();
  load_right();
  if (!RK_QP_FOLD) m = f;
  else if (ka < kb) m = kb < kc ? cb : (ka < kc ? cc : ca);
  else m = ka < kc ? ca : (kb < kc ? cc : cb);
  p = m == f ? k0 : m == ca ? ka : (m == cb ? kb : kc);
  tm = m == f ? t0 : m == ca ? ta : (m == cb ? tb : tc);
  fp = f;
#pragma unroll
  for (int u = 0; u < QP_PER; ++u) {
    const uint32_t x = lpos + 256 * u + tid;
    if (x == m) ak[u] = k0, at[u] = t0;
    const uint32_t o = 256 * u + tid;
    const uint32_t y = o < rpos - f ? rpos - 1 - o : 0xFFFFFFFFu;
    if (y == m) bk[u] = k0, bt[u] = t0;
    if (y == f) bk[u] = p, bt[u] = tm;
  }
  bool first = true;
  uint32_t par = 0;
  uint32_t cut = 0;
  for (;;) {
    const bool addl = qlt - qlh < QP_C && lpos < l;
    const bool addr = qrt - qrh < QP_C && rpos > f;
    if (!addl && qlt == qlh) {
      cut = qrh ? lastR : (qrt > qrh ? q.rp[qrh & QP_M] : f + 1);
      break;
    }
    if (!addr && qrt == qrh) {
      cut = q.lp[qlh & QP_M];
      break;
    }
    uint64_t bl[QP_PER], br[QP_PER];
#pragma unroll
    for (int u = 0; u < QP_PER; ++u) {
      const bool okl = addl && lpos + 256 * u + tid < l;
      const bool okr = addr && 256 * u + tid < rpos - f;
      bl[u] = __ballot(okl && !(ak[u] < p));
      br[u] = __ballot(okr && !(p < bk[u]));
      if (lane == 0) q.cnt[0][u * 4 + wv] = __popcll(bl[u]), q.cnt[1][u * 4 + wv] = __popcll(br[u]);
    }
    if (tid == 0) q.cross[par] = 0xFFFFFFFFu;
    __syncthreads();
    if (first && tid == 0) {
      K[f] = p;
      T[f] = tm;
      K[m] = k0;
      T[m] = t0;
    }
    first = false;
    uint32_t nl = 0, nr = 0, ol[QP_PER], orr[QP_PER];
#pragma unroll
    for (int j = 0; j < QP_PER * 4; ++j) {
      const uint32_t cl = q.cnt[0][j], cr = q.cnt[1][j];
      if (j % 4 == (int)wv) ol[j / 4] = nl, orr[j / 4] = nr;
      nl += cl;
      nr += cr;
    }
#pragma unroll
    for (int u = 0; u < QP_PER; ++u) {
      if ((bl[u] >> lane) & 1ull) {
        const uint32_t s = (qlt + ol[u] + __popcll(bl[u] & lt)) & QP_M;
        q.lk[s] = ak[u];
        q.lt[s] = at[u];
        q.lp[s] = lpos + 256 * u + tid;
      }
      if ((br[u] >> lane) & 1ull) {
        const uint32_t s = (qrt + orr[u] + __popcll(br[u] & lt)) & QP_M;
        q.rk[s] = bk[u];
        q.rt[s] = bt[u];
        q.rp[s] = rpos - 1 - (256 * u + tid);
      }
    }
    if (addl) {
      qlt += nl;
      lpos += QP_C;
      if (lpos < l) load_left();
    }
    if (addr) {
      qrt += nr;
      rpos = rpos - f > QP_C ? rpos - QP_C : f;
      if (rpos > f) load_right();
    }
    __syncthreads();
    uint32_t m = qlt - qlh < qrt - qrh ? qlt - qlh : qrt - qrh;
    if (m > QP_C) m = QP_C;
    for (uint32_t i = tid; i < m; i += 256)
      if (q.lp[(qlh + i) & QP_M] >= q.rp[(qrh + i) & QP_M]) atomicMin(&q.cross[par], i);
    __syncthreads();
    const uint32_t cr = q.cross[par];
    const uint32_t kc = cr < m ? cr : m;
    for (uint32_t i = tid; i < kc; i += 256) {
      const uint32_t sl = (qlh + i) & QP_M, sr = (qrh + i) & QP_M;
      const uint32_t xl = q.lp[sl], xr = q.rp[sr];
      K[xl] = q.rk[sr];
      K[xr] = q.lk[sl];
      T[xl] = q.rt[sr];
      T[xr] = q.lt[sl];
    }
    if (kc) lastR = q.rp[(qrh + kc - 1) & QP_M];
    if (cr < m) {
      const uint32_t cl = q.lp[(qlh + kc) & QP_M];
      cut = qrh + kc ? (cl < lastR ? cl : lastR) : cl;
      break;
    }
    qlh += kc;
    qrh += kc;
    par ^= 1u;
  }
  __syncthreads();
  return cut;
}

struct HeapSeg {
  uint32_t b, f, n, pad;
};
constexpr uint32_t HEAPQ_CAP = 512;

#ifndef RK_SPLIT_WPE
#define RK_SPLIT_WPE 8
#endif
#if RK_SPLIT_WPE
#define RK_SPLIT_WPE_ATTR __attribute__((amdgpu_waves_per_eu(RK_SPLIT_WPE)))
#else
#define RK_SPLIT_WPE_ATTR
#endif
template <bool qpart>
__global__ void __launch_bounds__(256) RK_SPLIT_WPE_ATTR k_sort_groups_split(TierLists tl, int tier,
                                                           const uint32_t *goff, uint64_t *key,
                                                           uint32_t *tag, uint32_t *otag,
                                                           uint32_t *pl, uint32_t *pr,
// ... 437 lines not shown
    }
    const bool rt = (2 * B < len) & (kr >= kl);
    const uint32_t kc = rt ? kr : kl;
    const bool cont = (2 * B <= len) & (kc >= vk);
    const uint32_t nv = cont ? kc : vk;
    const bool gw = (B >= TOPB) & (len != 0);
    const uint32_t Bw = gw ? HD + 1 : B;
    if constexpr (P == 8) {
      LB[Bw] = (uint8_t)nv;
    } else {
      const uint32_t bh = Bw * P, sh = bh & 31;
      __hip_atomic_fetch_and(LW + (bh >> 5), ~(M << sh), __ATOMIC_RELAXED,
                             __HIP_MEMORY_SCOPE_WORKGROUP);
      __hip_atomic_fetch_or(LW + (bh >> 5), nv << sh, __ATOMIC_RELAXED,
                            __HIP_MEMORY_SCOPE_WORKGROUP);
    }
    R[gw ? B : 0u] = (uint8_t)nv;
    const uint64_t gm = __builtin_amdgcn_ballot_w64(gw);
    const int gi = gm ? (int)__builtin_ctzll(gm) : 0;
    const uint32_t gb = (uint32_t)__builtin_amdgcn_readlane((int)B, gi);
    const uint32_t gv = (uint32_t)__builtin_amdgcn_readlane((int)nv, gi);
    rb1 = rb0, rv1 = rv0;
    rb0 = gm ? gb : 0u, rv0 = gv;
    const bool fin = (len != 0) & !cont;
    const uint64_t fm = __builtin_amdgcn_ballot_w64(fin);
    logb[fin ? k : npop] = B;
    ndone += (uint32_t)__popcll(fm);
    busy &= ~fm;
    B = cont ? 2 * B + (rt ? 1u : 0u) : fin ? HD + 1 : B;
    len = fin ? 0u : len;
    const uint32_t pa = ((B >= QTR) & (B < HALF) & (4 * B <= RMAX)) ? 4 * B : 0u;
    pf = *(const uint32_t *)(R + pa);
    const uint32_t y2 = n - 1 - knext;
    vg = *(const uint32_t *)(R + (((y2 + 1 >= TOPB ? y2 + 1 : 0u) & ~3u) + vzero));
  };
  while (ndone < npop) {
    tick(pf0, vg0);
    if (ndone >= npop) break;
    tick(pf1, vg1);
  }
}

__global__ void k_heap_log_split(uint32_t *logb, uint16_t *logq, uint32_t npop,
                                 const uint32_t *mode) {
  if (mode[0] != HM_RANK) return;
  for (uint32_t t = blockIdx.x * blockDim.x + threadIdx.x; t < npop; t += gridDim.x * blockDim.x) {
    const uint32_t b = logb[t], j = 31 - __clz((int)b);
    logb[t] = b ^ (1u << j);
    logq[t] = (uint16_t)(j | j << 8);
  }
}

__host__ __device__ constexpr uint32_t pipe_lds_bytes(uint32_t n, uint32_t P) {
  return ((n + 1) * P + 31) / 32 * 4 + 16;
}
__global__ void __launch_bounds__(256) k_heap_pipe_pops(uint8_t *R, uint32_t n, uint32_t P,
                                                       uint32_t tailL, uint32_t *logb,
                                                       uint16_t *logq, const uint32_t *mode) {
  extern __shared__ uint32_t lw[];
  if (mode[0] != HM_RANK) return;
  lds_u32 *LW = (lds_u32 *)lw;
  const uint32_t ntop = tailL ? (1u << tailL) - 1u : n;
  const uint32_t per = 32 / P, nw = (pipe_lds_bytes(ntop, P) - 16) / 4;
  for (uint32_t q = threadIdx.x; q < nw; q += blockDim.x) {
    uint32_t v = 0;
    for (uint32_t i = 0; i < per; i += 4) {
      const uint32_t p0 = q * per + i;
      const uint32_t r4 = p0 <= n ? *(const uint32_t *)(R + p0) : 0u;
#pragma unroll
      for (uint32_t b = 0; b < 4; ++b) {
        const uint32_t p = p0 + b;
        if (p >= 1 && p <= ntop) v |= ((r4 >> (8 * b)) & 0xffu) << ((i + b) * P);
      }
    }
    LW[q] = v;
  }
  if (threadIdx.x < 4) LW[nw + threadIdx.x] = 0;
  __syncthreads();
  if (threadIdx.x >= 64) return;
  lds_u8 *LB = (lds_u8 *)lw;
  const uint32_t HD = nw * per - 1;
  if (tailL) {
    switch (P) {
      case 1: pipe_pops_tail<1>(LB, LW, R, n, tailL, HD, logb, threadIdx.x); break;
      case 2: pipe_pops_tail<2>(LB, LW, R, n, tailL, HD, logb, threadIdx.x); break;
      default: pipe_pops_tail<4>(LB, LW, R, n, tailL, HD, logb, threadIdx.x); break;
    }
    return;
  }
  switch (P) {
    case 1: pipe_pops<1>(LB, LW, n, HD, logb, logq, threadIdx.x); break;
    case 2: pipe_pops<2>(LB, LW, n, HD, logb, logq, threadIdx.x); break;
    case 4: pipe_pops<4>(LB, LW, n, HD, logb, logq, threadIdx.x); break;
    default: pipe_pops<8>(LB, LW, n, HD, logb, logq, threadIdx.x); break;
  }
}

__global__ void k_heap_pair_counts(const uint16_t *logq, uint32_t npop, uint32_t *cnt) {
  for (uint32_t t = blockIdx.x * blockDim.x + threadIdx.x; t < npop + 1; t += gridDim.x * blockDim.x)
    cnt[t] = t < npop ? (uint32_t)(logq[t] >> 8) + 1u : 0u;
}
__global__ void k_heap_pairs(const uint32_t *logb, const uint16_t *logq, const uint32_t *off,
                             uint32_t npop, uint32_t *key, uint32_t *val) {
  for (uint32_t t = blockIdx.x * blockDim.x + threadIdx.x; t < npop; t += gridDim.x * blockDim.x) {
    const uint32_t b = logb[t], q = logq[t], D = q & 255u, j = q >> 8;
    uint32_t y = 0;
    const uint32_t o = off[t];
    for (uint32_t i = 0;; ++i) {
      key[o + i] = y;
      val[o + i] = t;
      if (i == j) break;
      y = 2 * y + 1 + ((b >> (D - 1 - i)) & 1u);
    }
  }
}
__global__ void k_heap_node_starts(const uint32_t *skey, uint32_t P, uint32_t n, uint32_t *noff) {
  for (uint32_t y = blockIdx.x * blockDim.x + threadIdx.x; y <= n; y += gridDim.x * blockDim.x) {
    uint32_t a = 0, b = P;
    while (a < b) {
      const uint32_t mid = a + (b - a) / 2;
      if (skey[mid] < y) a = mid + 1;
      else b = mid;
    }
    noff[y] = a;
  }
}
__global__ void k_heap_trace(const uint32_t *sval, const uint32_t *noff, const uint32_t *logb,
                             const uint16_t *logq, const uint32_t *T, uint32_t n, uint32_t *out) {
  for (uint32_t x = blockIdx.x * blockDim.x + threadIdx.x; x < n; x += gridDim.x * blockDim.x) {
    uint32_t y = 0, t = n - 1 - x;
    for (;;) {
      const uint32_t lo = noff[y], hi = noff[y + 1];
      uint32_t a = lo, b = hi;
      while (a < b) {
        const uint32_t mid = a + (b - a) / 2;
        if (sval[mid] < t) a = mid + 1;
        else b = mid;
      }
      if (a == lo) break;
      const uint32_t tp = sval[a - 1];
      const uint32_t q = logq[tp], D = q & 255u, j = q >> 8;
      const uint32_t i = 31 - __clz(y + 1);
      y = i < j ? 2 * y + 1 + ((logb[tp] >> (D - 1 - i)) & 1u) : n - 1 - tp;
      t = tp;
    }
    out[x] = T[y];
  }
}

static hipError_t heap_alloc(void **p, size_t bytes, hipStream_t st) {
  static const size_t cap = [] {
    const char *e = getenv("RK_HEAP_ALLOC_CAP");
    return e ? (size_t)strtoull(e, nullptr, 10) : (size_t)0;
  }();
  *p = nullptr;
  if (cap && bytes > cap) return hipErrorOutOfMemory;
  return hipMallocAsync(p, bytes, st);
}
static int heap_status(hipError_t e) {
  return e == hipSuccess ? RK_OK : e == hipErrorOutOfMemory ? RK_E_NOMEM : RK_E_HIP;
}

static int heap_segments(const HeapSeg *dq, uint32_t nheap, uint64_t *key, uint32_t *tag,
                         uint32_t *otag, uint32_t *host_words, hipStream_t st) {
  std::vector<HeapSeg> q(nheap);
  hipError_t e = hipMemcpyAsync(q.data(), dq, nheap * sizeof(HeapSeg), hipMemcpyDeviceToHost, st);
  if (e == hipSuccess) e = hipStreamSynchronize(st);
  if (e != hipSuccess) return RK_E_HIP;
  uint32_t nmax = 0;
  for (const HeapSeg &g : q) nmax = g.n > nmax ? g.n : nmax;
  constexpr uint32_t LDS_MAX = 160 * 1024 - 1024;
  static const bool attr = [] {
    (void)hipFuncSetAttribute((const void *)k_heap_rank_pops<false>,
                              hipFuncAttributeMaxDynamicSharedMemorySize, (int)LDS_MAX);
    (void)hipFuncSetAttribute((const void *)k_heap_rank_pops<true>,
                              hipFuncAttributeMaxDynamicSharedMemorySize, (int)LDS_MAX);
    (void)hipFuncSetAttribute((const void *)k_heap_pipe_pops,
                              hipFuncAttributeMaxDynamicSharedMemorySize, (int)LDS_MAX);
    return true;
  }();
  (void)attr;
  static const bool heap_pipe = [] {
    const char *s = getenv("RK_HEAP_PIPE");
    return !(s && s[0] == '0');
  }();
  static const bool heap_tail = [] {
    const char *s = getenv("RK_HEAP_TAIL");
    return !(s && s[0] == '0');
  }();
  uint8_t *R = nullptr;
  uint32_t *logb = nullptr, *mode = nullptr, *cnt = nullptr, *off = nullptr, *ssb = nullptr;
  uint16_t *logq = nullptr;
  const size_t sscap = scan_blocks((size_t)nmax + 1) + 64;
  int rc = RK_OK;
  {
    void **bufs[7] = {(void **)&R, (void **)&logb, (void **)&logq, (void **)&mode, (void **)&cnt,
                      (void **)&off, (void **)&ssb};
    const size_t sizes[7] = {(size_t)nmax + 16, (size_t)nmax * 4 + 16, (size_t)nmax * 2 + 16, 16,
                             ((size_t)nmax + 1) * 4 + 16, ((size_t)nmax + 1) * 4 + 16, sscap * 4};
    for (int i = 0; i < 7 && !rc; ++i) rc = heap_status(heap_alloc(bufs[i], sizes[i], st));
  }
  for (size_t si = 0; si < q.size() && !rc; ++si) {
    const HeapSeg &g = q[si];
    const size_t o = (size_t)g.b + g.f;
    uint64_t *K = key + o;
    uint32_t *T = tag + o, *out = otag + o;
    const uint32_t n = g.n, RT = (LDS_MAX - 32) | 1u;
    k_heap_prep<<<1, 256, 0, st>>>(K, T, n, R, mode);
    k_heap_equal<<<1, 64, 0, st>>>(T, n, out, mode);
    k_heap_general<<<1, 256, 0, st>>>(K, T, n, out, mode);
    e = hipMemcpyAsync(host_words, mode, 8, hipMemcpyDeviceToHost, st);
    if (e == hipSuccess) e = hipStreamSynchronize(st);
    if ((rc = heap_status(e))) break;
    if (host_words[0] != HM_RANK) continue;
    const uint32_t D = host_words[1];
    const uint32_t bpn = pipe_lds_bytes(n, 8) <= LDS_MAX ? 8u : D <= 2 ? 1u : D <= 4 ? 2u : 4u;
    const uint32_t L = 31 - __builtin_clz(n), tailL =
        pipe_lds_bytes(n, bpn) > LDS_MAX && heap_tail && L >= 6 &&
                pipe_lds_bytes((1u << L) - 1u, bpn) <= LDS_MAX ? L : 0u;
    if (heap_pipe && (tailL || pipe_lds_bytes(n, bpn) <= LDS_MAX)) {
      const uint32_t lds = pipe_lds_bytes(tailL ? (1u << L) - 1u : n, bpn);
      k_heap_pipe_pops<<<1, 256, lds, st>>>(R, n, bpn, tailL, logb, logq, mode);
      k_heap_log_split<<<grid_for(n, 256), 256, 0, st>>>(logb, logq, n - 1, mode);
    }
    else if (n + 16 <= LDS_MAX)
      k_heap_rank_pops<false><<<1, 64, n + 16, st>>>(R, n, n, logb, logq, mode);
    else
      k_heap_rank_pops<true><<<1, 64, RT + 16, st>>>(R, n, RT, logb, logq, mode);
    const uint32_t npop = n - 1;
    k_heap_pair_counts<<<grid_for(npop + 1, 256), 256, 0, st>>>(logq, npop, cnt);
    exclusive_scan_u32(cnt, off, (size_t)npop + 1, ScanScratch{ssb, sscap}, st);
    e = hipMemcpyAsync(host_words, off + npop, 4, hipMemcpyDeviceToHost, st);
    if (e == hipSuccess) e = hipStreamSynchronize(st);
    if ((rc = heap_status(e))) break;
    const uint32_t P = host_words[0];
    const size_t rw = radix_scratch_words(P);
    uint32_t *pk = nullptr, *pv = nullptr, *sk = nullptr, *sv = nullptr, *tk = nullptr,
             *tv = nullptr, *rs = nullptr, *noff = nullptr;
    for (uint32_t **b : {&pk, &pv, &sk, &sv, &tk, &tv})
      if (!rc) rc = heap_status(heap_alloc((void **)b, (size_t)P * 4 + 16, st));
    if (!rc) rc = heap_status(heap_alloc((void **)&rs, rw * 4, st));
    if (!rc) rc = heap_status(heap_alloc((void **)&noff, ((size_t)n + 2) * 4, st));
    if (!rc) {
      k_heap_pairs<<<grid_for(npop, 256), 256, 0, st>>>(logb, logq, off, npop, pk, pv);
      radix_sort_pairs(pk, pv, sk, sv, tk, tv, P, bit_length(n), rs, rw, st);
      k_heap_node_starts<<<grid_for(n + 1, 256), 256, 0, st>>>(sk, P, n, noff);
      k_heap_trace<<<grid_for(n, 256), 256, 0, st>>>(sv, noff, logb, logq, T, n, out);
    }
    for (uint32_t *b : {pk, pv, sk, sv, tk, tv, rs, noff})
      if (b) (void)hipFreeAsync(b, st);
  }
  for (void *b : {(void *)R, (void *)logb, (void *)logq, (void *)mode, (void *)cnt, (void *)off,
                  (void *)ssb})
    if (b) (void)hipFreeAsync(b, st);
  if (!rc && hipGetLastError() != hipSuccess) rc = RK_E_HIP;
  return rc;
}

__host__ __device__ constexpr size_t seg_lds_bytes(uint32_t cap, size_t key_bytes) {
  return (size_t)cap * (key_bytes + 4 + 2 + 2 + 1) +
         (SPLIT_STACK + 2 * (cap / (THRESH + 1) + 2)) * sizeof(Frame) + 16;
}
template <class KT, int WPB>
__global__ void __launch_bounds__(64 * WPB) k_sort_segments(TierLists tl, int tier, uint32_t m,
                                                            const uint8_t *bnd,
                                                            const uint32_t *head,
                                                            const uint64_t *key,
                                                            const uint32_t *tag, uint32_t *otag,
                                                            uint32_t reg_max, uint32_t slab,
                                                            const uint32_t *heapq_n,
                                                            uint32_t *heap_count, bool small_part) {
  if (heap_count && blockIdx.x == 0 && threadIdx.x == 0) *heap_count = *heapq_n;
  {
    uint32_t lo, hi;
    tl.range(tier, lo, hi);
    if (lo == hi) return;
  }
  extern __shared__ __align__(16) uint8_t smem_all[];
  constexpr uint32_t cap = SPLIT_T;
  const uint32_t lane = threadIdx.x & 63,
                 wv = WPB == 1 ? 0u : __builtin_amdgcn_readfirstlane(threadIdx.x >> 6);
  uint8_t *smem = smem_all + (size_t)wv * slab;
  const uint32_t nfr = cap / (THRESH + 1) + 2;
  KT *K = reinterpret_cast<KT *>(smem);
  uint32_t *T = reinterpret_cast<uint32_t *>(K + cap);
  Frame *stack = reinterpret_cast<Frame *>(T + cap);
  Frame *smallq = stack + SPLIT_STACK;
  Frame *heapq = smallq + nfr;
  uint16_t *PL = reinterpret_cast<uint16_t *>(heapq + nfr);
  uint16_t *PR = PL + cap;
  uint8_t *B = reinterpret_cast<uint8_t *>(PR + cap);
  const ViewT<KT, uint16_t> v{K, T, PL, PR, B};
  for (uint32_t w0 = (blockIdx.x * WPB + wv) * 64; w0 < m; w0 += gridDim.x * WPB * 64) {
    uint64_t hb = __ballot(w0 + lane < m && bnd[w0 + lane] == 1);
    while (hb) {
      const uint32_t x = w0 + (uint32_t)__builtin_ctzll(hb);
      hb &= hb - 1;
      const uint32_t h = head[x], n = h & 0xFFFFu;
      for (uint32_t y = lane; y < n; y += 64) {
        K[y] = (KT)key[x + y];
        T[y] = tag[x + y];
      }
      wave_sync();
      wave_std_sort<false>(v, n, otag + x, stack, smallq, heapq, GLanes<64>{lane, 0u},
                           (int)(h >> 16), reg_max, 0u, small_part);
      wave_sync();
    }
  }
}

__global__ void __launch_bounds__(256) k_sort_small(TierLists tl, const uint32_t *goff,
                                                    const uint64_t *key, const uint32_t *tag,
                                                    uint32_t *otag) {
  uint32_t lo, hi;
  tl.range(0, lo, hi);
  const uint32_t l = threadIdx.x & 15;
  for (uint32_t w = lo + ((blockIdx.x * blockDim.x + threadIdx.x) >> 4); w - lo < hi - lo;
       w += (gridDim.x * blockDim.x) >> 4) {
    const uint32_t g = tl.list[w];
    const uint32_t b = goff[g], n = goff[g + 1] - b;
    const bool in = l < n;
    const uint64_t k = in ? key[b + l] : ~0ull;
    uint32_t r = 0;
#pragma unroll
    for (int j = 0; j < THRESH; ++j) {
      const uint64_t kj = __shfl(k, j, 16);
      r += (uint32_t)j < n && (kj < k || (kj == k && (uint32_t)j < l));
    }
    if (in) otag[b + r] = b + l;
  }
}

constexpr int NTIER = GS_NTIER;
constexpr int NLDS = 4;
constexpr int TIER_LDS0 = 3;
static_assert(TIER_LDS0 + NLDS + 1 == NTIER, "tier layout");
struct Caps {
  uint32_t c[NLDS];
};
__host__ __device__ constexpr Caps lds_caps() { return Caps{{128, 256, 512, 2048}}; }

__device__ __forceinline__ int tier_of(uint32_t n) {
  constexpr Caps caps = lds_caps();
  if (n <= 1) return NTIER;
  if (n <= (uint32_t)THRESH) return 0;
  if (n <= 32) return 1;
  if (n <= 64) return 2;
#pragma unroll
  for (int j = 0; j < NLDS; ++j)
    if (n <= caps.c[j]) return TIER_LDS0 + j;
  return NTIER - 1;
}

constexpr uint32_t TCH = 4096;
__global__ void __launch_bounds__(256) k_tier_count(const uint32_t *goff, uint32_t ngroups,
                                                    uint32_t nblk, uint32_t *bc, uint32_t *bm,
                                                    uint32_t *heapq_n) {
  __shared__ uint32_t cnt[NTIER], mem[NTIER];
  if (blockIdx.x == 0 && threadIdx.x < 4) {
    if (threadIdx.x == 3) bc[(size_t)NTIER * nblk] = 0;
    else heapq_n[threadIdx.x] = 0;
  }
  if (threadIdx.x < NTIER) cnt[threadIdx.x] = mem[threadIdx.x] = 0;
  __syncthreads();
  const uint32_t g0 = blockIdx.x * TCH, g1 = min(g0 + TCH, ngroups);
  uint32_t c[NTIER] = {}, mm[NTIER] = {};
  for (uint32_t g = g0 + threadIdx.x; g < g1; g += 256) {
    const uint32_t n = goff[g + 1] - goff[g];
    const int t = tier_of(n);
#pragma unroll
    for (int u = 0; u < NTIER; ++u) c[u] += t == u, mm[u] += t == u ? n : 0;
  }
#pragma unroll
  for (int u = 0; u < NTIER; ++u) {
    uint32_t v = c[u], x = mm[u];
    for (int off = 32; off > 0; off >>= 1) v += __shfl_xor(v, off), x += __shfl_xor(x, off);
    if ((threadIdx.x & 63) == 0 && (v || x)) atomicAdd(&cnt[u], v), atomicAdd(&mem[u], x);
  }
  __syncthreads();
  if (threadIdx.x < NTIER) bc[(size_t)threadIdx.x * nblk + blockIdx.x] = cnt[threadIdx.x];
  if (bm && threadIdx.x < NTIER) bm[(size_t)threadIdx.x * nblk + blockIdx.x] = mem[threadIdx.x];
}

__global__ void __launch_bounds__(256) k_tier_lists(const uint32_t *goff, uint32_t ngroups,
                                                    uint32_t nblk, const uint32_t *off,
                                                    uint32_t *list, uint8_t *bnd, uint32_t m) {
  __shared__ uint32_t wc[4][NTIER];
  if (off[(size_t)(NTIER - 1) * nblk] != off[(size_t)NTIER * nblk]) {
    for (uint32_t x = (blockIdx.x * blockDim.x + threadIdx.x) * 16; x < m;
         x += gridDim.x * blockDim.x * 16) {
      if (x + 16 <= m) {
        *reinterpret_cast<uint4 *>(bnd + x) = make_uint4(0, 0, 0, 0);
      } else {
        for (uint32_t y = x; y < m; ++y) bnd[y] = 0;
      }
    }
  }
  const int lane = threadIdx.x & 63, wv = threadIdx.x >> 6;
  uint32_t run[NTIER];
#pragma unroll
  for (int u = 0; u < NTIER; ++u) run[u] = off[(size_t)u * nblk + blockIdx.x];
  const uint32_t g0 = blockIdx.x * TCH, g1 = min(g0 + TCH, ngroups);
  for (uint32_t c0 = g0; c0 < g1; c0 += 256) {
    const uint32_t g = c0 + threadIdx.x;
    const int t = g < g1 ? tier_of(goff[g + 1] - goff[g]) : 0;
    uint32_t rank = 0;
#pragma unroll
    for (int u = 0; u < NTIER; ++u) {
      const uint64_t b = __ballot(g < g1 && t == u);
      if (t == u) rank = __popcll(b & ((1ull << lane) - 1ull));
      if (lane == 0) wc[wv][u] = (uint32_t)__popcll(b);
    }
    __syncthreads();
    if (g < g1 && t < NTIER) {
      uint32_t before = 0;
      for (int k = 0; k < wv; ++k) before += wc[k][t];
#pragma unroll
      for (int u = 0; u < NTIER; ++u)
        if (u == t) list[run[u] + before + rank] = g;
    }
#pragma unroll
    for (int u = 0; u < NTIER; ++u) run[u] += wc[0][u] + wc[1][u] + wc[2][u] + wc[3][u];
    __syncthreads();
  }
}

size_t lds_bytes(uint32_t cap, size_t key_bytes, uint32_t reg_max) {
  const uint32_t nfr = cap / (THRESH + 1) + 2;
  return (size_t)cap * (key_bytes + 2 + 2 + 2 + 1) +
         (lds_stack(cap) + (reg_max ? 2 : 1) * nfr) * sizeof(Frame) + 16;
}

}

size_t groupsort_scratch_bytes(uint32_t n) {
  const size_t nblk = (size_t)n / TCH + 1;
  return (size_t)n * 4 * 2 + ((size_t)n + 1) * 4 + (size_t)n + 128 +
         (nblk * NTIER + 1) * 4 * 2 + nblk * NTIER * 4 + 256 + 256 +
         (HEAPQ_CAP + 1) * sizeof(HeapSeg) + 64;
}

static HeapSeg *heap_queue(void *scratch, uint32_t m, uint32_t ngroups) {
  const uint32_t nblk = (ngroups + TCH - 1) / TCH;
  uint32_t *pl = reinterpret_cast<uint32_t *>(scratch);
  uint32_t *list = pl + 2 * (size_t)m;
  uint8_t *bnd = reinterpret_cast<uint8_t *>(
      (reinterpret_cast<uintptr_t>(list + ngroups + 1) + 15) & ~(uintptr_t)15);
  uint32_t *bc = reinterpret_cast<uint32_t *>(
      (reinterpret_cast<uintptr_t>(bnd + m) + 63) & ~(uintptr_t)63);
  uint32_t *bm = bc + 2 * ((size_t)NTIER * nblk + 1);
  return reinterpret_cast<HeapSeg *>(
      (reinterpret_cast<uintptr_t>(bm + (size_t)NTIER * nblk) + 63) & ~(uintptr_t)63);
}

int sort_groups_heap_deferred(uint32_t ngroups, uint32_t m, uint64_t *key, uint32_t *tag,
                              uint32_t *otag, void *scratch, uint32_t nheap,
                              uint32_t *host_words, hipStream_t st) {
  nheap = nheap < HEAPQ_CAP ? nheap : HEAPQ_CAP;
  if (!nheap) return RK_OK;
  return heap_segments(heap_queue(scratch, m, ngroups), nheap, key, tag, otag, host_words, st);
}

int sort_groups_exact(const uint32_t *gid_sorted, const uint32_t *goff, uint32_t ngroups,
                       uint32_t m, uint64_t *key, uint32_t *tag, uint32_t *otag, void *scratch,
                       ScanScratch ss, uint32_t *host_words, bool narrow_keys, hipStream_t st,
                       hipStream_t side, hipEvent_t ev_fork, hipEvent_t ev_join,
                       uint32_t *heap_count) {
  if (!m) {
    if (heap_count) (void)hipMemsetAsync(heap_count, 0, 4, st);
    return RK_OK;
  }
  int hrc = RK_OK;
  constexpr int NL = NTIER;
  hipStream_t s2 = side ? side : st;
  constexpr Caps caps = lds_caps();
  const uint32_t nblk = (ngroups + TCH - 1) / TCH;
  uint32_t *pl = reinterpret_cast<uint32_t *>(scratch);
  uint32_t *pr = pl + m;
  uint32_t *list = pr + m;
  uint8_t *bnd = reinterpret_cast<uint8_t *>(
      (reinterpret_cast<uintptr_t>(list + ngroups + 1) + 15) & ~(uintptr_t)15);
  uint32_t *bc = reinterpret_cast<uint32_t *>(
      (reinterpret_cast<uintptr_t>(bnd + m) + 63) & ~(uintptr_t)63);
  uint32_t *boff = bc + (size_t)NL * nblk + 1;
  uint32_t *bm = boff + (size_t)NL * nblk + 1;
  HeapSeg *heapq = heap_queue(scratch, m, ngroups);
  uint32_t *heapq_n = reinterpret_cast<uint32_t *>(heapq + HEAPQ_CAP);
  const bool timing = g_ktimer != nullptr;
  if (timing) {
    g_ktimer->tier_nblk = nblk;
    for (int u = 0; u < KernelTimer::TIERS; ++u) g_ktimer->tier_slot[u] = -1;
  }
  k_tier_count<<<nblk, 256, 0, st>>>(goff, ngroups, nblk, bc, timing ? bm : nullptr, heapq_n);
  exclusive_scan_u32(bc, boff, (size_t)NL * nblk + 1, ss, st);
  k_tier_lists<<<nblk, 256, 0, st>>>(goff, ngroups, nblk, boff, list, bnd, m);
  const TierLists tl{list, boff, nblk};
  if (timing && g_ktimer->only < 0) g_ktimer->tier_counts = bm;
  auto tier_slot = [&](int u) {
    if (timing && g_ktimer->only < 0 && g_ktimer->n > 0) g_ktimer->tier_slot[u] = g_ktimer->n - 1;
  };
  if (side) {
    (void)hipEventRecord(ev_fork, st);
    (void)hipStreamWaitEvent(s2, ev_fork, 0);
  }
  static const uint32_t reg_max = [] {
    const char *e = getenv("RK_GS_REGMAX");
    return e ? (uint32_t)atoi(e) : 0u;
  }();
  static const bool small_part = [] {
    const char *e = getenv("RK_GS_SMALLPART");
    return !(e && e[0] == '0');
  }();
  static const int lds_side = [] {
    const char *e = getenv("RK_GS_SIDE");
    return e ? atoi(e) : 0;
  }();
  static const int lds_big = [] {
    const char *e = getenv("RK_GS_BIG");
    const int b = e ? atoi(e) : 2;
    return b < 0 ? 0 : b > NLDS ? NLDS : b;
  }();
  static const int wpb = [] {
    const char *e = getenv("RK_GS_WPB");
    return e && atoi(e) == 4 ? 4 : 1;
  }();
  static const uint32_t half_cap = [] {
    const char *e = getenv("RK_GS_HALF");
    return e ? (uint32_t)atoi(e) : 0u;
  }();
  auto launch_lds = [&](int j, hipStream_t sj) {
    const uint32_t cap = caps.c[j];
    static const uint32_t gs_mul = [] {
      const char *e = getenv("RK_GS_WAVES_MUL");
      const int v = e ? atoi(e) : 4;
      return v > 0 ? (uint32_t)v : 1u;
    }();
    const uint32_t waves = (cap <= 256 ? 16384 : cap <= 512 ? 8192 : 2048) * gs_mul;
    const int wp = cap <= 512 ? wpb : 1;
    const size_t slab = (lds_bytes(cap, narrow_keys ? 4 : 8, reg_max) + 15) & ~(size_t)15;
    kt_begin(sj, KID_SORT_LDS);
    if (cap <= half_cap && 2 * slab <= 65536) {
      if (narrow_keys)
        k_sort_groups_lds<uint32_t, 1, 32><<<waves / 2, 64, 2 * slab, sj>>>(
            tl, TIER_LDS0 + j, goff, key, tag, otag, cap, 0u, (uint32_t)slab, small_part);
      else
        k_sort_groups_lds<uint64_t, 1, 32><<<waves / 2, 64, 2 * slab, sj>>>(
            tl, TIER_LDS0 + j, goff, key, tag, otag, cap, 0u, (uint32_t)slab, small_part);
    } else if (wp == 4) {
      if (narrow_keys)
        k_sort_groups_lds<uint32_t, 4><<<waves / 4, 256, 4 * slab, sj>>>(
            tl, TIER_LDS0 + j, goff, key, tag, otag, cap, reg_max, (uint32_t)slab, small_part);
      else
        k_sort_groups_lds<uint64_t, 4><<<waves / 4, 256, 4 * slab, sj>>>(
            tl, TIER_LDS0 + j, goff, key, tag, otag, cap, reg_max, (uint32_t)slab, small_part);
    } else {
      if (narrow_keys)
        k_sort_groups_lds<uint32_t, 1><<<waves, 64, slab, sj>>>(tl, TIER_LDS0 + j, goff, key, tag,
                                                                otag, cap, reg_max, (uint32_t)slab, small_part);
      else
        k_sort_groups_lds<uint64_t, 1><<<waves, 64, slab, sj>>>(tl, TIER_LDS0 + j, goff, key, tag,
                                                                otag, cap, reg_max, (uint32_t)slab, small_part);
    }
    kt_end(sj, KID_SORT_LDS, 0.0);
    tier_slot(TIER_LDS0 + j);
  };
  const int big0 = side ? NLDS - lds_big : NLDS;
  for (int j = NLDS - 1; j >= big0; --j) launch_lds(j, s2);
  static const int small_main = [] {
    const char *e = getenv("RK_GS_SMALL1");
    return e ? atoi(e) : 0;
  }();
  auto launch_small = [&](hipStream_t sj) {
    kt_begin(sj, KID_SORT_SMALL);
    k_sort_small<<<2048, 256, 0, sj>>>(tl, goff, key, tag, otag);
    kt_end(sj, KID_SORT_SMALL, 0.0);
    tier_slot(0);
    kt_begin(sj, KID_SORT_REG);
    k_sort_groups_reg<2><<<4096, 256, 0, sj>>>(tl, 1, goff, key, tag, otag);
    kt_end(sj, KID_SORT_REG, 0.0);
    tier_slot(1);
  };
  if (!small_main || !side) launch_small(s2);
  static const int reg1_main = [] {
    const char *e = getenv("RK_GS_REG1");
    return e ? atoi(e) : 1;
  }();
  auto launch_reg1 = [&](hipStream_t sj) {
    kt_begin(sj, KID_SORT_REG);
    k_sort_groups_reg<1><<<4096, 256, 0, sj>>>(tl, 2, goff, key, tag, otag);
    kt_end(sj, KID_SORT_REG, 0.0);
    tier_slot(2);
  };
  if (!reg1_main || !side) launch_reg1(s2);
  for (int pass = 0; pass < 2; ++pass) {
    if (pass == 1 && side) (void)hipEventRecord(ev_join, s2);
    for (int j = 0; j < big0; ++j) {
      if ((j < lds_side) != (pass == 0)) continue;
      launch_lds(j, pass == 0 ? s2 : st);
    }
  }
  if (reg1_main && side) launch_reg1(st);
  if (small_main && side) launch_small(st);
#ifdef RK_GS_PROF
  {
    unsigned long long h[8];
    (void)hipStreamSynchronize(st);
    (void)hipMemcpyFromSymbol(h, HIP_SYMBOL(g_gs_prof), sizeof h);
    const double g = h[6] ? (double)h[6] : 1.0;
    fprintf(stderr, "GSPROF groups=%llu members/group %.1f cyc/group: stack %.0f partitions %.0f batches %.0f final %.0f | partitions/group %.2f batches/group %.2f\n",
            h[6], h[7] / g, h[0] / g, h[1] / g, h[2] / g, h[3] / g, h[4] / g, h[5] / g);
    void *p = nullptr;
    (void)hipGetSymbolAddress(&p, HIP_SYMBOL(g_gs_prof));
    (void)hipMemsetAsync(p, 0, sizeof h, st);
  }
#endif
  static const bool split_dyn = [] {
    const char *e = getenv("RK_SPLIT_DYN");
    return !(e && e[0] == '0');
  }();
  static const uint32_t split_big = [] {
    const char *e = getenv("RK_SPLIT_BIG");
    return e ? (uint32_t)atoi(e) : 65536u;
  }();
  static const uint32_t split_grid = [] {
    const char *e = getenv("RK_SPLIT_GRID");
    const int v = e ? atoi(e) : 0;
    return v > 0 ? (uint32_t)v : 2048u;
  }();
  static const uint32_t split_pad = [] {
    const char *e = getenv("RK_SPLIT_LDSPAD");
    const int v = e ? atoi(e) : 0;
    return v > 0 && v <= 32768 ? (uint32_t)v : 0u;
  }();
  static const bool split_q = [] {
    const char *e = getenv("RK_SPLIT_Q");
    return !(e && e[0] == '0');
  }();
  kt_begin(st, KID_SORT_GLOBAL);
  {
    const uint32_t lds = split_pad + (split_q ? (uint32_t)sizeof(QPart) : 0u);
    auto kern = split_q ? k_sort_groups_split<true> : k_sort_groups_split<false>;
    kern<<<split_grid, 256, lds, st>>>(tl, NTIER - 1, goff, key, tag, otag, pl, pr, bnd, heapq_n,
                                       heapq, split_dyn ? heapq_n + 1 : nullptr, split_big);
  }
  kt_end(st, KID_SORT_GLOBAL, 0.0);
  tier_slot(NTIER - 1);
  static const bool heap_rank = [] {
    const char *e = getenv("RK_HEAP_RANK");
    return !(e && e[0] == '0');
  }();
  kt_begin(st, KID_SORT_HEAP);
  if (heap_rank && heap_count) {
  } else if (heap_rank) {
    (void)hipMemcpyAsync(host_words, heapq_n, 4, hipMemcpyDeviceToHost, st);
    (void)hipStreamSynchronize(st);
    const uint32_t nheap = host_words[0] < HEAPQ_CAP ? host_words[0] : HEAPQ_CAP;
    if (nheap) hrc = heap_segments(heapq, nheap, key, tag, otag, host_words, st);
  } else {
    k_heap_segments<<<64, 256, 0, st>>>(heapq_n, heapq, key, tag, otag);
  }
  kt_end(st, KID_SORT_HEAP, 0.0);
  kt_begin(st, KID_SORT_SEGS);
  {
    const size_t slab = (seg_lds_bytes(SPLIT_T, narrow_keys ? 4 : 8) + 15) & ~(size_t)15;
    if (wpb == 4) {
      if (narrow_keys)
        k_sort_segments<uint32_t, 4><<<2048, 256, 4 * slab, st>>>(
            tl, NTIER - 1, m, bnd, pl, key, tag, otag, reg_max, (uint32_t)slab, heapq_n,
            heap_rank ? heap_count : nullptr, small_part);
      else
        k_sort_segments<uint64_t, 4><<<2048, 256, 4 * slab, st>>>(
            tl, NTIER - 1, m, bnd, pl, key, tag, otag, reg_max, (uint32_t)slab, heapq_n,
            heap_rank ? heap_count : nullptr, small_part);
    } else {
      static const int seg_env = [] {
        const char *e = getenv("RK_SEG_WAVES");
        return e ? atoi(e) : 0;
      }();
      const int seg_waves =
          seg_env > 0 ? seg_env : (int)std::min(131072u, std::max(8192u, m / 8192));
      if (narrow_keys)
        k_sort_segments<uint32_t, 1><<<seg_waves, 64, slab, st>>>(
            tl, NTIER - 1, m, bnd, pl, key, tag, otag, reg_max, (uint32_t)slab, heapq_n,
            heap_rank ? heap_count : nullptr, small_part);
      else
        k_sort_segments<uint64_t, 1><<<seg_waves, 64, slab, st>>>(
            tl, NTIER - 1, m, bnd, pl, key, tag, otag, reg_max, (uint32_t)slab, heapq_n,
            heap_rank ? heap_count : nullptr, small_part);
    }
  }
  kt_end(st, KID_SORT_SEGS, 0.0);
  tier_slot(NTIER);
  if (side) (void)hipStreamWaitEvent(st, ev_join, 0);
  return hrc;
}

}
```

repkiller_amd/csrc/rk_internal.h:

```cpp
#pragma once

#include <initializer_list>
#include <hip/hip_runtime.h>
#include <stdint.h>

#include "../../include/repkiller_amd.h"

namespace rk {

enum : uint8_t {
  ST_UNKNOWN = 0,
  ST_ACTIVE = 1,
  ST_HIT_PENDING = 2,
  ST_HIT = 3,
};

enum : uint32_t {
  ERRB_UB_BUCKET = 1u,
  ERRB_UB_CENTER = 2u,
  ERRB_INTERNAL = 4u,
  ERRB_WIDE_LENGTH = 8u,
};

constexpr uint32_t NONE = 0xFFFFFFFFu;

inline unsigned grid_for(size_t n, int threads, size_t cap = 65536) {
  size_t g = (n + threads - 1) / threads;
  if (g > cap) g = cap;
  return (unsigned)(g ? g : 1);
}

inline int bit_length(uint64_t v) { return v ? 64 - __builtin_clzll(v) : 0; }

struct ScanScratch {
  uint32_t *block_sums;
  size_t cap;
};
size_t scan_blocks(size_t n);
void exclusive_scan_u32(const uint32_t *in, uint32_t *out, size_t n, ScanScratch ss,
                        hipStream_t st);
void exclusive_scan_u32_clear0(uint32_t *in, uint32_t *out, size_t n, ScanScratch ss,
                               hipStream_t st);
void exclusive_scan_roots(const uint32_t *par, uint32_t m, uint32_t *out, ScanScratch ss,
                          hipStream_t st, uint32_t *total = nullptr);

enum KernelId : int {
  KID_PREP, KID_HIST, KID_SCATTER, KID_GATHER, KID_SORT_KEYS, KID_CSR_FILL_X, KID_RUN_BOUNDS,
  KID_SWEEP_TILE, KID_SWEEP_FAST, KID_SWEEP_MORE, KID_SWEEP_WAVE, KID_CSR_FILL_Y, KID_JUMP,
  KID_ASSIGN_GID, KID_GROUP_OFFSETS, KID_BUILD_RECORDS, KID_SORT_SMALL, KID_SORT_REG, KID_SORT_LDS,
  KID_SORT_GLOBAL, KID_EMIT, KID_PART, KID_EXCHANGE, KID_SHARD_AUX, KID_SH_ROWKEYS, KID_SH_FILLY,
  KID_SH_YRES, KID_SH_XOWN, KID_SH_MERGE, KID_SORT_SEGS, KID_SWEEP_LONG, KID_NW_HIST,
  KID_ONESWEEP, KID_NW_XCHUNK, KID_NW_FILLY, KID_NW_ASSIGN, KID_NW_XCOUNT, KID_NW_XBITS,
  KID_SORT_HEAP, KID_NW_FINE, KID_NW_MFINE, KID_NW_YFINE, KID_COUNT
};
extern const char *const kKernelNames[KID_COUNT];
constexpr int GS_NTIER = 8;

struct KernelTimer {
  static constexpr int MAX = 256;
  hipEvent_t ev[2 * MAX];
  int kid[MAX];
  double bytes[MAX];
  int n;
  static constexpr int TIERS = GS_NTIER + 1;
  const uint32_t *tier_counts;
  uint32_t tier_nblk;
  int tier_slot[TIERS];
  int only = -1;
  uint32_t *units = nullptr;
  double unit_bytes[MAX];
};
extern thread_local KernelTimer *g_ktimer;
inline void kt_begin(hipStream_t st, int kid) {
  KernelTimer *t = g_ktimer;
  if (t && t->n < KernelTimer::MAX && (t->only < 0 || t->only == kid))
    (void)hipEventRecord(t->ev[2 * t->n], st);
}
inline void kt_end(hipStream_t st, int kid, double bytes) {
  KernelTimer *t = g_ktimer;
  if (t && t->n < KernelTimer::MAX && (t->only < 0 || t->only == kid)) {
    (void)hipEventRecord(t->ev[2 * t->n + 1], st);
    t->kid[t->n] = kid;
    t->bytes[t->n] = bytes;
    t->unit_bytes[t->n] = 0.0;
    t->n++;
  }
}
inline uint32_t *kt_units(hipStream_t st, int kid) {
  KernelTimer *t = g_ktimer;
  if (!t || !t->units || t->n >= KernelTimer::MAX || !(t->only < 0 || t->only == kid)) return nullptr;
  (void)hipMemsetAsync(t->units + t->n, 0, 4, st);
  return t->units + t->n;
}
inline void kt_end_units(hipStream_t st, int kid, double bytes_per_unit) {
  KernelTimer *t = g_ktimer;
  const int slot = t ? t->n : -1;
  kt_end(st, kid, 0.0);
  if (t && t->n == slot + 1 && t->units) t->unit_bytes[slot] = bytes_per_unit;
}

size_t radix_scratch_words(uint32_t n);
void radix_sort_pairs(const uint32_t *key_in, const uint32_t *val_in, uint32_t *key_out,
                      uint32_t *val_out, uint32_t *key_tmp, uint32_t *val_tmp, uint32_t n,
                      int bits, uint32_t *scratch, size_t scratch_words, hipStream_t st,
                      int max_digit = 0);

struct Axis {
  const uint32_t *key;
  const uint32_t *ent;
  const uint64_t *cen;
  const uint64_t *len;
  uint8_t *state;
  uint32_t *xres;
  uint32_t *par;
  const uint2 *pk;
  const uint8_t *nbd;
  uint32_t *rlen_at;
  uint32_t *rbeg_at;
  uint32_t m;
  uint64_t max_index;
  double len_ratio, pos_ratio;
  bool par_dev = false;
};
struct RunList {
  uint32_t *big;
  uint8_t *wpend;
  uint32_t nbig, nwin;
  bool fast32;
};
size_t runs_scratch_words(uint32_t m);
void build_runs(const Axis &ax, RunList &rl, uint32_t *dev_count, uint32_t *host_words,
                hipStream_t st);
constexpr uint32_t PEND_WORDS = 64;
void occupancy_sweep(const Axis &ax, const RunList &rl, uint8_t *rpend, uint32_t *counters,
                     bool first, hipStream_t st, bool clear = true);

struct Frags {
  const uint64_t *x, *y, *len;
  const uint8_t *strand;
  uint32_t n;
};
struct Proc {
  ulonglong2 *rec;
  uint64_t *ys;
  uint32_t *pkey;
  uint32_t *row;
  ulonglong2 *xrec;
  ulonglong2 *yrec;
  uint32_t *ylenhi;
  ulonglong2 *hrec;
  uint32_t *keyx, *keyy;
  uint32_t *par, *gid;
  uint32_t *grow;
};
struct Csr {
  uint32_t *key, *ent;
  uint64_t *cen, *len;
  uint8_t *state;
  uint2 *pk;
  uint8_t *nbd;
};

__device__ __forceinline__ uint32_t wave_incl_scan(uint32_t v) {
  v += __builtin_amdgcn_update_dpp(0u, v, 0x111, 0xf, 0xf, false);
  v += __builtin_amdgcn_update_dpp(0u, v, 0x112, 0xf, 0xf, false);
  v += __builtin_amdgcn_update_dpp(0u, v, 0x114, 0xf, 0xf, false);
  v += __builtin_amdgcn_update_dpp(0u, v, 0x118, 0xf, 0xf, false);
  v += __builtin_amdgcn_update_dpp(0u, v, 0x142, 0xa, 0xf, false);
  v += __builtin_amdgcn_update_dpp(0u, v, 0x143, 0xc, 0xf, false);
  return v;
}

__device__ __forceinline__ int neighbour_dir(uint64_t c, uint64_t max_index) {
  const uint64_t r = c % 100;
  if (r <= 1 && c >= 100) return -1;
  if ((r == 99 && c < max_index) || (r == 98 && c < max_index - 1)) return 1;
  return 0;
}
void prep_keys(const Frags &f, uint64_t vsize, uint64_t max_x, uint64_t max_y, uint32_t *pkey,
               ulonglong2 *rec, uint32_t *kept, uint32_t *err, hipStream_t st);
void gather_proc(const Frags &f, Proc p, uint32_t m, uint32_t nbx, uint32_t nby, hipStream_t st);
void sort_keys(Proc p, uint32_t m, uint32_t *wide, hipStream_t st);
void csr_fill_x(Csr c, const ulonglong2 *xrec, uint32_t m, uint64_t max_index, hipStream_t st);
void csr_fill_y(Csr c, const ulonglong2 *yrec, const uint32_t *ylenhi, uint32_t m,
                uint64_t max_index, hipStream_t st);
void jump_round(Proc p, uint32_t m, uint32_t *changed, uint32_t *isnew, uint32_t *err,
                hipStream_t st, const uint32_t *open = nullptr);
void jump_listed(Proc p, uint32_t m, uint32_t *isnew, uint32_t *err, uint32_t *list,
                 uint32_t *count, uint32_t *changed, hipStream_t st);
void assign_gid(Proc p, uint32_t m, const uint32_t *newrank, hipStream_t st);
void group_offsets(const uint32_t *sgid, uint32_t m, uint32_t ngroups, uint32_t *goff,
                   hipStream_t st);
void build_records(uint32_t *gmem, const ulonglong2 *hrec, uint32_t m, uint64_t *key,
                   uint32_t *tag, hipStream_t st);
size_t groupsort_scratch_bytes(uint32_t n);
int sort_groups_exact(const uint32_t *gid_sorted, const uint32_t *goff, uint32_t ngroups,
                      uint32_t m, uint64_t *key, uint32_t *tag, uint32_t *otag, void *scratch,
                      ScanScratch ss, uint32_t *host_words, bool narrow_keys, hipStream_t st,
                      hipStream_t side = nullptr, hipEvent_t ev_fork = nullptr,
                      hipEvent_t ev_join = nullptr, uint32_t *heap_count = nullptr);
int sort_groups_heap_deferred(uint32_t ngroups, uint32_t m, uint64_t *key, uint32_t *tag,
                              uint32_t *otag, void *scratch, uint32_t nheap,
                              uint32_t *host_words, hipStream_t st);
void emit_result(const uint32_t *otag, const uint32_t *sgid, const uint32_t *goff,
                 const uint32_t *mrow, uint32_t m, uint32_t *out_gid, uint8_t *out_rep,
                 uint32_t *out_order, hipStream_t st);

struct NwDigits {
  int passes;
  int shift[4], db[4];
};
NwDigits nw_plan(int bits, int max_bits = 0);
void nw_trace_dump(hipStream_t st);
size_t nw_status_words(uint32_t n);
uint32_t nw_chunk_width(uint32_t m, uint32_t nbx);
uint32_t nw_chunks(uint32_t nbx, uint32_t W);
struct NwChunkCounts {
  uint32_t W, lgW, nch;
  uint32_t *cnts;
};
void nw_order_hist(const rk_frags_soa &in, uint64_t vsize, uint64_t max_x, uint64_t max_y,
                   uint32_t nby, const NwDigits &a, const NwDigits &y, uint32_t *ghist,
                   uint32_t *yhist, uint32_t *ctrl, hipStream_t st, const uint3 *wire = nullptr);
void nw_order_sort(const rk_frags_soa &in, uint64_t vsize, uint32_t nby, const NwDigits &a,
                   const uint32_t *ghist, uint32_t *status, uint4 *Ra, uint4 *Rb, uint4 *yrec,
                   hipStream_t st, const uint3 *wire = nullptr);
struct NwOrderPlan {
  int C = 0, F = 0;
  uint32_t nseg = 0;
  NwDigits coarse{};
  uint32_t kbase = 0;
};
struct ZeroRegion {
  void *ptr;
  size_t bytes;
};
void zero_regions(hipStream_t st, std::initializer_list<ZeroRegion> regs);
void nw_order_coarse_regions(uint32_t n, const NwOrderPlan &op, uint32_t *status, uint32_t *chist,
                             ZeroRegion extra, ZeroRegion out[4]);
constexpr uint32_t NW_SEG_CAP_ORDER = 4096, NW_SEG_CAP_Y = 2048, NW_SEG_CAP_MEMBERS = 4096;
NwOrderPlan nw_order_split(uint32_t n, uint64_t nkeys, int bits, uint32_t cap);
NwOrderPlan nw_order_split_range(uint32_t n, uint64_t klo, uint64_t khi);
void nw_order_sort_split_coarse(const rk_frags_soa &in, const NwOrderPlan &op,
                                const uint32_t *ghist, uint32_t *status, uint4 *Ra, uint4 *Rb,
                                uint32_t *chist, ZeroRegion extra, uint64_t vsize,
                                hipStream_t st, const uint3 *wire = nullptr,
                                bool zeroed = false);
void nw_order_sort_split_fine(uint32_t n, uint32_t m, uint32_t nby, const NwOrderPlan &op,
                              uint4 *Ra, uint4 *Rb, uint4 *yrec, uint4 *tmp, uint32_t *chist,
                              uint32_t *coff, ScanScratch ss, const NwChunkCounts *cc,
                              hipStream_t st);
inline size_t nw_seg_words(uint32_t n) { return (size_t)n / 256 + 64; }
void nw_order_sort_recs_split(const uint4 *in, uint32_t m, uint32_t nby, uint32_t base,
                              const NwOrderPlan &op, const uint32_t *ghist, uint32_t *status,
                              uint4 *Ra, uint4 *Rb, uint4 *yrec, uint4 *tmp, uint32_t *chist,
                              uint32_t *coff, ScanScratch ss, const NwChunkCounts *cc,
                              hipStream_t st);
void nw_order_sort_split(const rk_frags_soa &in, uint32_t m, uint32_t nby, const NwOrderPlan &op,
                         const uint32_t *ghist, uint32_t *status, uint4 *Ra, uint4 *Rb,
                         uint4 *yrec, uint4 *tmp, uint32_t *chist, uint32_t *coff,
                         ScanScratch ss, const NwChunkCounts *cc, uint64_t vsize, hipStream_t st,
                         const uint3 *wire = nullptr);
void nw_member_sort_split(const uint4 *erec, const uint32_t *gidp, uint4 *t0, uint4 *t1,
                          uint4 *t2, uint32_t m, uint32_t G, const NwOrderPlan &mp,
                          const uint32_t *ehist, uint32_t *status, uint32_t *sgid, uint64_t *key,
                          uint32_t *tag, uint32_t *mrow, uint32_t *goff, uint32_t *chist,
                          uint32_t *coff, ScanScratch ss, hipStream_t st);
void nw_x_count_add(const uint4 *halo, uint32_t G, const NwChunkCounts &cc, hipStream_t st);
void nw_x_count(const uint4 *R, uint32_t m, const NwChunkCounts &cc, hipStream_t st,
                const uint4 *halo = nullptr, uint32_t G = 0);
void nw_y_sort_head(const uint4 *yrec, uint4 *tmp, uint32_t m, const NwDigits &y,
                    const uint32_t *yhist, uint32_t *status, hipStream_t st,
                    bool arrival_ids = false, const uint4 *src0 = nullptr);
void nw_y_sort_tail(const uint4 *yrec, const uint4 *tmp, uint32_t m, const NwDigits &y,
                    const uint32_t *yhist, uint32_t *status, Csr cy, uint32_t nby,
                    uint64_t max_y, const uint32_t *xbits, hipStream_t st,
                    bool arrival_ids = false, const uint4 *src0 = nullptr);
void nw_y_sort_split_after_x(uint4 *yrec, uint4 *tmp, uint4 *tmp2, uint32_t m,
                             const NwOrderPlan &yp, const uint32_t *yhist, uint32_t *status,
                             Csr cy, uint32_t nby, uint64_t max_y, const uint32_t *xbits,
                             uint32_t *chist, uint32_t *coff, ScanScratch ss, hipStream_t st);
void nw_y_sort_after_x(const uint4 *yrec, uint4 *tmp, uint32_t m, const NwDigits &y,
                       const uint32_t *yhist, uint32_t *status, Csr cy, uint32_t nby,
                       uint64_t max_y, const uint32_t *xbits, hipStream_t st,
                       const uint4 *src0 = nullptr);
void nw_x_chunks(const uint4 *R, uint32_t m, uint32_t nbx, uint64_t max_x, uint32_t maxlen,
                 const uint32_t *xoff, Csr cx, uint32_t *xpos, uint4 *erec, uint32_t *ctrl,
                 uint32_t W, hipStream_t st, const uint4 *halo = nullptr, uint32_t G = 0);
void nw_order_sort_recs(const uint4 *in, uint32_t m, uint32_t nby, uint32_t base,
                        const NwDigits &a, const uint32_t *ghist, uint32_t *status, uint4 *Ra,
                        uint4 *Rb, uint4 *yrec, hipStream_t st);
void nw_rec_hist(const void *recs, int rec_bytes, uint32_t n, uint32_t sub, const NwDigits &d,
                 uint32_t *ghist, hipStream_t st);
void nw_member_sort_recv(const void *recs, bool narrow_keys, uint32_t m, uint32_t g0,
                         const NwDigits &e, const uint32_t *ehist, uint32_t *status, uint4 *t0,
                         uint4 *t1, uint32_t *sgid, uint64_t *key, uint32_t *tag, uint32_t *mrow,
                         hipStream_t st);
void nw_x_bits(const uint32_t *xpos, const uint8_t *xstate, uint32_t m, uint32_t *bits,
               hipStream_t st);
void nw_fill_y(const uint32_t *ent, const uint32_t *bits, uint8_t *state, uint32_t m,
               hipStream_t st);
void nw_assign(const uint32_t *par, const uint32_t *newrank, uint32_t *gidp, uint32_t m,
               const NwDigits &e, uint32_t *ehist, hipStream_t st);
void nw_assign_jump(uint32_t *par, const uint32_t *newrank, uint32_t *gidp, uint32_t m,
                    const NwDigits &e, uint32_t *ehist, uint32_t *list, uint32_t *ctrl,
                    hipStream_t st);
void nw_member_sort(const uint4 *erec, const uint32_t *gidp, uint4 *t0, uint4 *t1, uint32_t m,
                    const NwDigits &e, const uint32_t *ehist, uint32_t *status, uint32_t *sgid,
                    uint64_t *key, uint32_t *tag, uint32_t *mrow, bool narrow_keys,
                    hipStream_t st);

}
```

Baseline: 5.643 billion fragments/s.

## Fuse result emission into group offsets and group sort kernels

Removes the separate emit_result pass. The group-offset kernel now also writes rep flags and singleton order entries, and the per-tier group sort kernels write output rows directly through a RowSink instead of writing intermediate otag. The sgid scratch buffer is dropped in favour of writing group ids straight into the output gid array. A new size-4 tier with a 4-lane small sort is also added. The trade is an extra indirect rows[] load per sorted element, more template instantiations, and a separate emit path for the largest tier.

```diff
diff --git a/repkiller_amd/csrc/rk_api.hip b/repkiller_amd/csrc/rk_api.hip
--- a/repkiller_amd/csrc/rk_api.hip
+++ b/repkiller_amd/csrc/rk_api.hip
@@ -36,7 +36,8 @@
         double mem = 0;
         for (uint32_t b = 0; b < nb; ++b) mem += h[(size_t)u * nb + b];
         const int sl = ctx->kt.tier_slot[u];
-        if (sl >= 0 && sl < ctx->kt.n) ctx->kt.bytes[sl] = 12.0 * mem;
+        if (sl >= 0 && sl < ctx->kt.n)
+          ctx->kt.bytes[sl] = (u == GS_NTIER - 1 ? 12.0 : ctx->kt.tier_member_bytes) * mem;
         const int s2 = u == GS_NTIER - 1 ? ctx->kt.tier_slot[GS_NTIER] : -1;
         if (s2 >= 0 && s2 < ctx->kt.n) ctx->kt.bytes[s2] = 12.0 * mem;
       }
@@ -318,7 +319,7 @@
   uint4 *Ra, *Rb, *yrec, *erec;
   rk::Csr cx, cy;
   uint32_t *xpos, *xbits;
-  uint32_t *par, *isnew, *newrank, *sgid, *tag, *otag, *mrow, *goff;
+  uint32_t *par, *isnew, *newrank, *tag, *otag, *mrow, *goff;
   uint64_t *reckey;
   void *gsort;
   uint32_t *rpend, *runs, *rlen_at, *rbeg_at;
@@ -352,7 +353,6 @@
   w.par = c.take<uint32_t>(n);
   w.isnew = c.take<uint32_t>(n);
   w.newrank = c.take<uint32_t>(n);
-  w.sgid = c.take<uint32_t>(n);
   w.tag = c.take<uint32_t>(n);
   w.otag = c.take<uint32_t>(n);
   w.mrow = c.take<uint32_t>(n);
@@ -561,6 +561,10 @@
     const char *e = getenv("RK_SWEEP_BLIND");
     const int v = e ? atoi(e) : 3;
     return (uint32_t)(v < 1 ? 1 : v > 8 ? 8 : v);
+  }();
+  static const bool emit_direct = [] {
+    const char *e = getenv("RK_EMIT_DIRECT");
+    return !(e && e[0] == '0');
   }();
   for (uint32_t q = 0; q < npairs; ++q) {
     const rk_params &pq = prms[q];
@@ -681,25 +685,34 @@
     else
       rk::nw_assign(w.par, w.newrank, w.isnew, m, msplit ? mp.coarse : ed, w.ehist, st);
 
+    uint32_t *const sgid = out->gid;
+    const rk::DirectEmit de{w.mrow, out->out_order};
     if (prof) mark(ctx, RK_PH_MEMBERS);
     if (msplit) {
       rk::nw_member_sort_split(w.erec, w.isnew, w.Ra, w.Rb, w.yrec, m, G, mp, w.ehist, w.astatus,
-                               w.sgid, w.reckey, w.tag, w.mrow, w.goff, w.chist, w.coff, ss, st);
+                               sgid, w.reckey, w.tag, w.mrow, w.goff, w.chist, w.coff, ss, st);
+      if (emit_direct)
+        rk::group_offsets_emit(sgid, m, G, nullptr, w.mrow, out->repval, out->out_order, st);
     } else {
-      rk::nw_member_sort(w.erec, w.isnew, w.Ra, w.Rb, m, ed, w.ehist, w.astatus, w.sgid,
+      rk::nw_member_sort(w.erec, w.isnew, w.Ra, w.Rb, m, ed, w.ehist, w.astatus, sgid,
                          w.reckey, w.tag, w.mrow, narrow_keys, st);
-      rk::group_offsets(w.sgid, m, G, w.goff, st);
+      if (emit_direct)
+        rk::group_offsets_emit(sgid, m, G, w.goff, w.mrow, out->repval, out->out_order, st);
+      else
+        rk::group_offsets(sgid, m, G, w.goff, st);
     }
     if (prof) mark(ctx, RK_PH_GROUP_SORT);
-    if ((rc = rk::sort_groups_exact(w.sgid, w.goff, G, m, w.reckey, w.tag, w.otag, w.gsort, ss,
+    if ((rc = rk::sort_groups_exact(sgid, w.goff, G, m, w.reckey, w.tag, w.otag, w.gsort, ss,
                                     ctx->host + 128, narrow_keys, st, st2, ctx->fork, ctx->join,
-                                    npairs == 1 ? w.ctrl + 33 : nullptr))) {
+                                    npairs == 1 ? w.ctrl + 33 : nullptr,
+                                    emit_direct ? &de : nullptr))) {
       ctx->err = "depth-limit heap segments: buffer allocation failed";
       return rc;
     }
     if (prof) mark(ctx, RK_PH_EMIT);
-    rk::emit_result(w.otag, w.sgid, w.goff, w.mrow, m, out->gid, out->repval, out->out_order,
-                    st);
+    if (!emit_direct)
+      rk::emit_result(w.otag, sgid, w.goff, w.mrow, m, out->gid, out->repval, out->out_order,
+                      st);
     HIPCHK(ctx, hipGetLastError());
     if (prof) mark(ctx, RK_N_PHASES);
   }
@@ -716,8 +729,12 @@
       ctx->err = "depth-limit heap segments: buffer allocation failed";
       return rc;
     }
-    rk::emit_result(w.otag, w.sgid, w.goff, w.mrow, m, outs[0].gid, outs[0].repval,
-                    outs[0].out_order, st);
+    if (emit_direct)
+      rk::emit_large_groups(G, m, w.goff, w.otag, w.gsort,
+                            rk::DirectEmit{w.mrow, outs[0].out_order}, st);
+    else
+      rk::emit_result(w.otag, outs[0].gid, w.goff, w.mrow, m, outs[0].gid, outs[0].repval,
+                      outs[0].out_order, st);
     HIPCHK(ctx, hipGetLastError());
     HIPCHK(ctx, hipEventRecord(ctx->ev1, st));
     if ((rc = readback(ctx, w.ctrl, 1))) return rc;
diff --git a/repkiller_amd/csrc/rk_groups.hip b/repkiller_amd/csrc/rk_groups.hip
--- a/repkiller_amd/csrc/rk_groups.hip
+++ b/repkiller_amd/csrc/rk_groups.hip
@@ -160,6 +160,64 @@
   if (blockIdx.x == 0 && threadIdx.x == 0) goff[ngroups] = m;
 }
 
+__global__ void k_group_offsets_emit_unaligned(const uint32_t *sgid, uint32_t m,
+                                               uint32_t ngroups, uint32_t *goff,
+                                               const uint32_t *mrow, uint8_t *out_rep,
+                                               uint32_t *out_order) {
+  GRID_STRIDE(q, m) {
+    const uint32_t g = sgid[q];
+    const bool start = q == 0 || g != sgid[q - 1];
+    const bool end = q + 1 == m || sgid[q + 1] != g;
+    if (start && goff) goff[g] = q;
+    out_rep[q] = start ? (end ? 0 : 1) : 2;
+    if (start && end) out_order[q] = mrow[q];
+  }
+  if (goff && blockIdx.x == 0 && threadIdx.x == 0) goff[ngroups] = m;
+}
+__global__ void __launch_bounds__(256) k_group_offsets_emit(const uint32_t *sgid, uint32_t m,
+                                                             uint32_t ngroups, uint32_t *goff,
+                                                             const uint32_t *mrow,
+                                                             uint8_t *out_rep, uint32_t *out_order,
+                                                             bool rep_word) {
+  const uint32_t nq = (m + 3) / 4;
+  for (uint32_t t = blockIdx.x * blockDim.x + threadIdx.x; t < nq; t += gridDim.x * blockDim.x) {
+    const uint32_t q0 = t * 4;
+    const bool full = q0 + 4 <= m;
+    uint32_t g[5];
+    if (full) {
+      const uint4 v = *reinterpret_cast<const uint4 *>(sgid + q0);
+      g[0] = v.x, g[1] = v.y, g[2] = v.z, g[3] = v.w;
+    } else {
+#pragma unroll
+      for (int j = 0; j < 4; ++j) g[j] = q0 + j < m ? sgid[q0 + j] : 0u;
+    }
+    g[4] = q0 + 4 < m ? sgid[q0 + 4] : 0u;
+    uint32_t prev = q0 ? sgid[q0 - 1] : ~0u;
+    uint32_t word = 0;
+    uint8_t f[4];
+#pragma unroll
+    for (int j = 0; j < 4; ++j) {
+      const uint32_t q = q0 + j;
+      const bool in = q < m;
+      const bool start = g[j] != prev;
+      const bool end = q + 1 >= m || g[j + 1] != g[j];
+      if (in && start && goff) goff[g[j]] = q;
+      f[j] = start ? (end ? 0 : 1) : 2;
+      word |= (uint32_t)f[j] << (8 * j);
+      if (in && start && end) out_order[q] = mrow[q];
+      prev = g[j];
+    }
+    if (full && rep_word) {
+      *reinterpret_cast<uint32_t *>(out_rep + q0) = word;
+    } else {
+#pragma unroll
+      for (int j = 0; j < 4; ++j)
+        if (q0 + j < m) out_rep[q0 + j] = f[j];
+    }
+  }
+  if (goff && blockIdx.x == 0 && threadIdx.x == 0) goff[ngroups] = m;
+}
+
 __global__ void k_jump(Proc p, uint32_t m, uint32_t *changed, uint32_t *isnew, uint32_t *err,
                        const uint32_t *open) {
   if (open && (open[0] | open[1])) return;
@@ -312,6 +370,19 @@
     k_group_offsets_unaligned<<<grid_for(m, 256), 256, 0, st>>>(sgid, m, ngroups, goff);
   kt_end(st, KID_GROUP_OFFSETS, 4.0 * m + 4.0 * ngroups);
 }
+void group_offsets_emit(const uint32_t *sgid, uint32_t m, uint32_t ngroups, uint32_t *goff,
+                        const uint32_t *mrow, uint8_t *out_rep, uint32_t *out_order,
+                        hipStream_t st) {
+  kt_begin(st, KID_GROUP_OFFSETS);
+  if ((reinterpret_cast<uintptr_t>(sgid) & 15) == 0)
+    k_group_offsets_emit<<<grid_for((m + 3) / 4, 256, 16384), 256, 0, st>>>(
+        sgid, m, ngroups, goff, mrow, out_rep, out_order,
+        (reinterpret_cast<uintptr_t>(out_rep) & 3) == 0);
+  else
+    k_group_offsets_emit_unaligned<<<grid_for(m, 256), 256, 0, st>>>(sgid, m, ngroups, goff, mrow,
+                                                                     out_rep, out_order);
+  kt_end(st, KID_GROUP_OFFSETS, 5.0 * m + (goff ? 4.0 : 0.0) * ngroups + 8.0 * ngroups);
+}
 void jump_round(Proc p, uint32_t m, uint32_t *changed, uint32_t *isnew, uint32_t *err,
                 hipStream_t st, const uint32_t *open) {
   if (!m) return;
diff --git a/repkiller_amd/csrc/rk_groupsort.hip b/repkiller_amd/csrc/rk_groupsort.hip
--- a/repkiller_amd/csrc/rk_groupsort.hip
+++ b/repkiller_amd/csrc/rk_groupsort.hip
@@ -21,6 +21,18 @@
   __builtin_amdgcn_wave_barrier();
   __builtin_amdgcn_fence(__ATOMIC_ACQUIRE, "agent");
 }
+
+struct TagSink {
+  uint32_t *out;
+  __device__ __forceinline__ void put(uint32_t slot, uint32_t tag) const { out[slot] = tag; }
+  __device__ __forceinline__ TagSink at(uint32_t b) const { return TagSink{out + b}; }
+};
+struct RowSink {
+  uint32_t *out;
+  const uint32_t *rows;
+  __device__ __forceinline__ void put(uint32_t slot, uint32_t tag) const { out[slot] = rows[tag]; }
+  __device__ __forceinline__ RowSink at(uint32_t b) const { return RowSink{out + b, rows}; }
+};
 
 template <bool GLOBAL>
 __device__ __forceinline__ void sync_mem() {
@@ -436,9 +448,9 @@
   }
 }
 
-template <bool GLOBAL, class KT, class V>
+template <bool GLOBAL, class KT, class V, class SK>
 __device__ void reg_finish(const V &v, bool in, int bl, uint32_t bm, int len, int d,
-                           uint32_t lane, uint64_t k64, uint32_t t, uint32_t *out,
+                           uint32_t lane, uint64_t k64, uint32_t t, const SK &out,
                            uint32_t tbase) {
   const int x = (int)lane;
   KT k = in ? (KT)k64 : (KT)~(KT)0;
@@ -454,21 +466,21 @@
     r += (j < my) && (ky < k || (ky == k && y < x));
   }
   if (in) {
-    out[heaped ? mpos : bm + (uint32_t)(sf - bl) + r] = tbase + t;
+    out.put(heaped ? mpos : bm + (uint32_t)(sf - bl) + r, tbase + t);
     if (v.B) v.B[mpos] = 3;
   }
 }
 
-template <bool GLOBAL, class V>
+template <bool GLOBAL, class V, class SK>
 __device__ void reg_batch(const V &v, bool in, int bl, uint32_t bm, int len, int d,
-                          uint32_t lane, uint32_t *out, uint32_t tbase = 0) {
+                          uint32_t lane, const SK &out, uint32_t tbase = 0) {
   const uint32_t mpos = bm + (uint32_t)((int)lane - bl);
   const uint64_t k = in ? (uint64_t)v.K[mpos] : ~0ull;
   const uint32_t t = in ? (GLOBAL ? mpos : v.T[mpos]) : 0u;
   if (sizeof(typename V::key_t) == 8 && __ballot(in && (k >> 32) != 0))
-    reg_finish<GLOBAL, uint64_t, V>(v, in, bl, bm, len, d, lane, k, t, out, tbase);
+    reg_finish<GLOBAL, uint64_t, V, SK>(v, in, bl, bm, len, d, lane, k, t, out, tbase);
   else
-    reg_finish<GLOBAL, uint32_t, V>(v, in, bl, bm, len, d, lane, k, t, out, tbase);
+    reg_finish<GLOBAL, uint32_t, V, SK>(v, in, bl, bm, len, d, lane, k, t, out, tbase);
 }
 
 template <int W>
@@ -629,8 +641,8 @@
 #define GS_ADD(slot, v)
 #endif
 
-template <bool GLOBAL, class V, int W = 64>
-__device__ void wave_std_sort(const V &v, uint32_t n, uint32_t *out, Frame *stack,
+template <bool GLOBAL, class V, int W = 64, class SK>
+__device__ void wave_std_sort(const V &v, uint32_t n, const SK &out, Frame *stack,
                               Frame *smallq, Frame *heapq, GLanes<W> L, int d0,
                               uint32_t reg_max, uint32_t tbase = 0, bool small_part = true) {
   static_assert(W == 64 || W == 32, "a wavefront or a half");
@@ -718,7 +730,7 @@
     if (bd) carry = c + 63 - (uint32_t)__clzll(bd);
     if (x < n && b != 3) {
       if (b == 2) {
-        out[x] = tbase + v.T[x];
+        out.put(x, tbase + v.T[x]);
       } else {
         const typename V::key_t kx = v.K[x];
         uint32_t r = 0;
@@ -729,7 +741,7 @@
         for (int j = 0; j < THRESH; ++j)
           r += (uint32_t)(s + j < e) &
                ((uint32_t)(ky[j] < kx) | ((uint32_t)(ky[j] == kx) & (uint32_t)(s + j < x)));
-        out[s + r] = tbase + v.T[x];
+        out.put(s + r, tbase + v.T[x]);
       }
     }
   }
@@ -757,10 +769,10 @@
   }
 };
 
-template <int PACK>
+template <int PACK, class SK>
 __global__ void __launch_bounds__(256) k_sort_groups_reg(TierLists tl, int tier,
                                                          const uint32_t *goff, uint64_t *key,
-                                                         uint32_t *tag, uint32_t *otag) {
+                                                         uint32_t *tag, SK otag) {
   constexpr int SPAN = 64 / PACK;
   const uint32_t lane = threadIdx.x & 63;
   const int j = (int)lane / SPAN;
@@ -781,12 +793,12 @@
 __host__ __device__ constexpr uint32_t lds_stack(uint32_t cap) {
   return 2 * (31 - __builtin_clz(cap)) + 4;
 }
-template <class KT, int WPB, int W = 64>
+template <class KT, int WPB, int W = 64, class SK = TagSink>
 __global__ void __launch_bounds__(64 * WPB)
 __attribute__((amdgpu_waves_per_eu(W == 32 && sizeof(KT) == 4 ? 8 : 1))) k_sort_groups_lds(TierLists tl, int tier,
                                                               const uint32_t *goff,
                                                               const uint64_t *key,
-                                                              const uint32_t *tag, uint32_t *otag,
+                                                              const uint32_t *tag, SK otag,
                                                               uint32_t cap, uint32_t reg_max,
                                                               uint32_t slab, bool small_part) {
   extern __shared__ __align__(16) uint8_t smem_all[];
@@ -818,7 +830,7 @@
       T[x] = (uint16_t)x;
     }
     wave_sync();
-    wave_std_sort<false, ViewT<KT, uint16_t, uint16_t>, W>(v, n, otag + b, stack, smallq, heapq,
+    wave_std_sort<false, ViewT<KT, uint16_t, uint16_t>, W>(v, n, otag.at(b), stack, smallq, heapq,
                                                            L, 2 * (31 - __clz((int)n)), reg_max,
                                                            b, small_part);
     wave_sync();
@@ -1862,38 +1874,41 @@
         T[y] = tag[x + y];
       }
       wave_sync();
-      wave_std_sort<false>(v, n, otag + x, stack, smallq, heapq, GLanes<64>{lane, 0u},
+      wave_std_sort<false>(v, n, TagSink{otag + x}, stack, smallq, heapq, GLanes<64>{lane, 0u},
                            (int)(h >> 16), reg_max, 0u, small_part);
       wave_sync();
     }
   }
 }
 
-__global__ void __launch_bounds__(256) k_sort_small(TierLists tl, const uint32_t *goff,
+template <int LANES, class SK>
+__global__ void __launch_bounds__(256) k_sort_small(TierLists tl, int tier, const uint32_t *goff,
                                                     const uint64_t *key, const uint32_t *tag,
-                                                    uint32_t *otag) {
+                                                    SK otag) {
+  static_assert(LANES == 4 || LANES == 16, "lanes per group");
+  constexpr int LG = LANES == 4 ? 2 : 4;
   uint32_t lo, hi;
-  tl.range(0, lo, hi);
-  const uint32_t l = threadIdx.x & 15;
-  for (uint32_t w = lo + ((blockIdx.x * blockDim.x + threadIdx.x) >> 4); w - lo < hi - lo;
-       w += (gridDim.x * blockDim.x) >> 4) {
+  tl.range(tier, lo, hi);
+  const uint32_t l = threadIdx.x & (LANES - 1);
+  for (uint32_t w = lo + ((blockIdx.x * blockDim.x + threadIdx.x) >> LG); w - lo < hi - lo;
+       w += (gridDim.x * blockDim.x) >> LG) {
     const uint32_t g = tl.list[w];
     const uint32_t b = goff[g], n = goff[g + 1] - b;
     const bool in = l < n;
     const uint64_t k = in ? key[b + l] : ~0ull;
     uint32_t r = 0;
 #pragma unroll
-    for (int j = 0; j < THRESH; ++j) {
-      const uint64_t kj = __shfl(k, j, 16);
+    for (int j = 0; j < LANES; ++j) {
+      const uint64_t kj = __shfl(k, j, LANES);
       r += (uint32_t)j < n && (kj < k || (kj == k && (uint32_t)j < l));
     }
-    if (in) otag[b + r] = b + l;
+    if (in) otag.put(b + r, b + l);
   }
 }
 
 constexpr int NTIER = GS_NTIER;
 constexpr int NLDS = 4;
-constexpr int TIER_LDS0 = 3;
+constexpr int TIER_LDS0 = 4;
 static_assert(TIER_LDS0 + NLDS + 1 == NTIER, "tier layout");
 struct Caps {
   uint32_t c[NLDS];
@@ -1903,9 +1918,10 @@
 __device__ __forceinline__ int tier_of(uint32_t n) {
   constexpr Caps caps = lds_caps();
   if (n <= 1) return NTIER;
-  if (n <= (uint32_t)THRESH) return 0;
-  if (n <= 32) return 1;
-  if (n <= 64) return 2;
+  if (n <= 4) return 0;
+  if (n <= (uint32_t)THRESH) return 1;
+  if (n <= 32) return 2;
+  if (n <= 64) return 3;
 #pragma unroll
   for (int j = 0; j < NLDS; ++j)
     if (n <= caps.c[j]) return TIER_LDS0 + j;
@@ -1985,6 +2001,21 @@
   }
 }
 
+__global__ void __launch_bounds__(256) k_emit_listed(TierLists tl, int tier, const uint32_t *goff,
+                                                     const uint32_t *otag, DirectEmit d,
+                                                     uint32_t m) {
+  uint32_t lo, hi;
+  tl.range(tier, lo, hi);
+  for (uint32_t w = lo + blockIdx.x; w < hi; w += gridDim.x) {
+    const uint32_t g = tl.list[w];
+    const uint32_t b = goff[g], e = goff[g + 1];
+    for (uint32_t x = b + threadIdx.x; x < e; x += blockDim.x) {
+      const uint32_t o = otag[x];
+      d.out_order[x] = d.rows[o < m ? o : x];
+    }
+  }
+}
+
 size_t lds_bytes(uint32_t cap, size_t key_bytes, uint32_t reg_max) {
   const uint32_t nfr = cap / (THRESH + 1) + 2;
   return (size_t)cap * (key_bytes + 2 + 2 + 2 + 1) +
@@ -2021,11 +2052,24 @@
   return heap_segments(heap_queue(scratch, m, ngroups), nheap, key, tag, otag, host_words, st);
 }
 
+void emit_large_groups(uint32_t ngroups, uint32_t m, const uint32_t *goff, const uint32_t *otag,
+                       const void *scratch, DirectEmit direct, hipStream_t st) {
+  if (!m) return;
+  const uint32_t nblk = (ngroups + TCH - 1) / TCH;
+  const uint32_t *list = reinterpret_cast<const uint32_t *>(scratch) + 2 * (size_t)m;
+  const uint8_t *bnd = reinterpret_cast<const uint8_t *>(
+      (reinterpret_cast<uintptr_t>(list + ngroups + 1) + 15) & ~(uintptr_t)15);
+  const uint32_t *bc = reinterpret_cast<const uint32_t *>(
+      (reinterpret_cast<uintptr_t>(bnd + m) + 63) & ~(uintptr_t)63);
+  const uint32_t *boff = bc + (size_t)NTIER * nblk + 1;
+  k_emit_listed<<<1024, 256, 0, st>>>(TierLists{list, boff, nblk}, NTIER - 1, goff, otag, direct, m);
+}
+
 int sort_groups_exact(const uint32_t *gid_sorted, const uint32_t *goff, uint32_t ngroups,
                        uint32_t m, uint64_t *key, uint32_t *tag, uint32_t *otag, void *scratch,
                        ScanScratch ss, uint32_t *host_words, bool narrow_keys, hipStream_t st,
                        hipStream_t side, hipEvent_t ev_fork, hipEvent_t ev_join,
-                       uint32_t *heap_count) {
+                       uint32_t *heap_count, const DirectEmit *direct) {
   if (!m) {
     if (heap_count) (void)hipMemsetAsync(heap_count, 0, 4, st);
     return RK_OK;
@@ -2055,6 +2099,7 @@
   exclusive_scan_u32(bc, boff, (size_t)NL * nblk + 1, ss, st);
   k_tier_lists<<<nblk, 256, 0, st>>>(goff, ngroups, nblk, boff, list, bnd, m);
   const TierLists tl{list, boff, nblk};
+  if (timing) g_ktimer->tier_member_bytes = direct ? 16.0 : 12.0;
   if (timing && g_ktimer->only < 0) g_ktimer->tier_counts = bm;
   auto tier_slot = [&](int u) {
     if (timing && g_ktimer->only < 0 && g_ktimer->n > 0) g_ktimer->tier_slot[u] = g_ktimer->n - 1;
@@ -2099,28 +2144,33 @@
     const int wp = cap <= 512 ? wpb : 1;
     const size_t slab = (lds_bytes(cap, narrow_keys ? 4 : 8, reg_max) + 15) & ~(size_t)15;
     kt_begin(sj, KID_SORT_LDS);
-    if (cap <= half_cap && 2 * slab <= 65536) {
-      if (narrow_keys)
-        k_sort_groups_lds<uint32_t, 1, 32><<<waves / 2, 64, 2 * slab, sj>>>(
-            tl, TIER_LDS0 + j, goff, key, tag, otag, cap, 0u, (uint32_t)slab, small_part);
-      else
-        k_sort_groups_lds<uint64_t, 1, 32><<<waves / 2, 64, 2 * slab, sj>>>(
-            tl, TIER_LDS0 + j, goff, key, tag, otag, cap, 0u, (uint32_t)slab, small_part);
-    } else if (wp == 4) {
-      if (narrow_keys)
-        k_sort_groups_lds<uint32_t, 4><<<waves / 4, 256, 4 * slab, sj>>>(
-            tl, TIER_LDS0 + j, goff, key, tag, otag, cap, reg_max, (uint32_t)slab, small_part);
-      else
-        k_sort_groups_lds<uint64_t, 4><<<waves / 4, 256, 4 * slab, sj>>>(
-            tl, TIER_LDS0 + j, goff, key, tag, otag, cap, reg_max, (uint32_t)slab, small_part);
-    } else {
-      if (narrow_keys)
-        k_sort_groups_lds<uint32_t, 1><<<waves, 64, slab, sj>>>(tl, TIER_LDS0 + j, goff, key, tag,
-                                                                otag, cap, reg_max, (uint32_t)slab, small_part);
-      else
-        k_sort_groups_lds<uint64_t, 1><<<waves, 64, slab, sj>>>(tl, TIER_LDS0 + j, goff, key, tag,
-                                                                otag, cap, reg_max, (uint32_t)slab, small_part);
-    }
+    auto go = [&](auto sink) {
+      using SK = decltype(sink);
+      if (cap <= half_cap && 2 * slab <= 65536) {
+        if (narrow_keys)
+          k_sort_groups_lds<uint32_t, 1, 32, SK><<<waves / 2, 64, 2 * slab, sj>>>(
+              tl, TIER_LDS0 + j, goff, key, tag, sink, cap, 0u, (uint32_t)slab, small_part);
+        else
+          k_sort_groups_lds<uint64_t, 1, 32, SK><<<waves / 2, 64, 2 * slab, sj>>>(
+              tl, TIER_LDS0 + j, goff, key, tag, sink, cap, 0u, (uint32_t)slab, small_part);
+      } else if (wp == 4) {
+        if (narrow_keys)
+          k_sort_groups_lds<uint32_t, 4, 64, SK><<<waves / 4, 256, 4 * slab, sj>>>(
+              tl, TIER_LDS0 + j, goff, key, tag, sink, cap, reg_max, (uint32_t)slab, small_part);
+        else
+          k_sort_groups_lds<uint64_t, 4, 64, SK><<<waves / 4, 256, 4 * slab, sj>>>(
+              tl, TIER_LDS0 + j, goff, key, tag, sink, cap, reg_max, (uint32_t)slab, small_part);
+      } else {
+        if (narrow_keys)
+          k_sort_groups_lds<uint32_t, 1, 64, SK><<<waves, 64, slab, sj>>>(
+              tl, TIER_LDS0 + j, goff, key, tag, sink, cap, reg_max, (uint32_t)slab, small_part);
+        else
+          k_sort_groups_lds<uint64_t, 1, 64, SK><<<waves, 64, slab, sj>>>(
+              tl, TIER_LDS0 + j, goff, key, tag, sink, cap, reg_max, (uint32_t)slab, small_part);
+      }
+    };
+    if (direct) go(RowSink{direct->out_order, direct->rows});
+    else go(TagSink{otag});
     kt_end(sj, KID_SORT_LDS, 0.0);
     tier_slot(TIER_LDS0 + j);
   };
@@ -2132,13 +2182,31 @@
   }();
   auto launch_small = [&](hipStream_t sj) {
     kt_begin(sj, KID_SORT_SMALL);
-    k_sort_small<<<2048, 256, 0, sj>>>(tl, goff, key, tag, otag);
+    static const bool small4 = [] {
+      const char *e = getenv("RK_GS_SMALL4");
+      return !(e && e[0] == '0');
+    }();
+    auto small = [&](auto sink) {
+      using SK = decltype(sink);
+      if (small4) k_sort_small<4, SK><<<2048, 256, 0, sj>>>(tl, 0, goff, key, tag, sink);
+      else k_sort_small<16, SK><<<2048, 256, 0, sj>>>(tl, 0, goff, key, tag, sink);
+      kt_end(sj, KID_SORT_SMALL, 0.0);
+      tier_slot(0);
+      kt_begin(sj, KID_SORT_SMALL);
+      k_sort_small<16, SK><<<2048, 256, 0, sj>>>(tl, 1, goff, key, tag, sink);
+    };
+    if (direct) small(RowSink{direct->out_order, direct->rows});
+    else small(TagSink{otag});
     kt_end(sj, KID_SORT_SMALL, 0.0);
-    tier_slot(0);
+    tier_slot(1);
     kt_begin(sj, KID_SORT_REG);
-    k_sort_groups_reg<2><<<4096, 256, 0, sj>>>(tl, 1, goff, key, tag, otag);
+    if (direct)
+      k_sort_groups_reg<2, RowSink><<<4096, 256, 0, sj>>>(
+          tl, 2, goff, key, tag, RowSink{direct->out_order, direct->rows});
+    else
+      k_sort_groups_reg<2, TagSink><<<4096, 256, 0, sj>>>(tl, 2, goff, key, tag, TagSink{otag});
     kt_end(sj, KID_SORT_REG, 0.0);
-    tier_slot(1);
+    tier_slot(2);
   };
   if (!small_main || !side) launch_small(s2);
   static const int reg1_main = [] {
@@ -2147,9 +2215,13 @@
   }();
   auto launch_reg1 = [&](hipStream_t sj) {
     kt_begin(sj, KID_SORT_REG);
-    k_sort_groups_reg<1><<<4096, 256, 0, sj>>>(tl, 2, goff, key, tag, otag);
+    if (direct)
+      k_sort_groups_reg<1, RowSink><<<4096, 256, 0, sj>>>(
+          tl, 3, goff, key, tag, RowSink{direct->out_order, direct->rows});
+    else
+      k_sort_groups_reg<1, TagSink><<<4096, 256, 0, sj>>>(tl, 3, goff, key, tag, TagSink{otag});
     kt_end(sj, KID_SORT_REG, 0.0);
-    tier_slot(2);
+    tier_slot(3);
   };
   if (!reg1_main || !side) launch_reg1(s2);
   for (int pass = 0; pass < 2; ++pass) {
@@ -2251,6 +2323,7 @@
   }
   kt_end(st, KID_SORT_SEGS, 0.0);
   tier_slot(NTIER);
+  if (direct) k_emit_listed<<<1024, 256, 0, st>>>(tl, NTIER - 1, goff, otag, *direct, m);
   if (side) (void)hipStreamWaitEvent(st, ev_join, 0);
   return hrc;
 }
diff --git a/repkiller_amd/csrc/rk_internal.h b/repkiller_amd/csrc/rk_internal.h
--- a/repkiller_amd/csrc/rk_internal.h
+++ b/repkiller_amd/csrc/rk_internal.h
@@ -54,7 +54,7 @@
   KID_SORT_HEAP, KID_NW_FINE, KID_NW_MFINE, KID_NW_YFINE, KID_COUNT
 };
 extern const char *const kKernelNames[KID_COUNT];
-constexpr int GS_NTIER = 8;
+constexpr int GS_NTIER = 9;
 
 struct KernelTimer {
   static constexpr int MAX = 256;
@@ -66,6 +66,7 @@
   const uint32_t *tier_counts;
   uint32_t tier_nblk;
   int tier_slot[TIERS];
+  double tier_member_bytes = 12.0;
   int only = -1;
   uint32_t *units = nullptr;
   double unit_bytes[MAX];
@@ -191,14 +192,24 @@
 void assign_gid(Proc p, uint32_t m, const uint32_t *newrank, hipStream_t st);
 void group_offsets(const uint32_t *sgid, uint32_t m, uint32_t ngroups, uint32_t *goff,
                    hipStream_t st);
+void group_offsets_emit(const uint32_t *sgid, uint32_t m, uint32_t ngroups, uint32_t *goff,
+                        const uint32_t *mrow, uint8_t *out_rep, uint32_t *out_order,
+                        hipStream_t st);
 void build_records(uint32_t *gmem, const ulonglong2 *hrec, uint32_t m, uint64_t *key,
                    uint32_t *tag, hipStream_t st);
 size_t groupsort_scratch_bytes(uint32_t n);
+struct DirectEmit {
+  const uint32_t *rows;
+  uint32_t *out_order;
+};
 int sort_groups_exact(const uint32_t *gid_sorted, const uint32_t *goff, uint32_t ngroups,
                       uint32_t m, uint64_t *key, uint32_t *tag, uint32_t *otag, void *scratch,
                       ScanScratch ss, uint32_t *host_words, bool narrow_keys, hipStream_t st,
                       hipStream_t side = nullptr, hipEvent_t ev_fork = nullptr,
-                      hipEvent_t ev_join = nullptr, uint32_t *heap_count = nullptr);
+                      hipEvent_t ev_join = nullptr, uint32_t *heap_count = nullptr,
+                      const DirectEmit *direct = nullptr);
+void emit_large_groups(uint32_t ngroups, uint32_t m, const uint32_t *goff, const uint32_t *otag,
+                       const void *scratch, DirectEmit direct, hipStream_t st);
 int sort_groups_heap_deferred(uint32_t ngroups, uint32_t m, uint64_t *key, uint32_t *tag,
                               uint32_t *otag, void *scratch, uint32_t nheap,
                               uint32_t *host_words, hipStream_t st);
```

Result: faster. 5.745 billion fragments/s, median of 6 (+1.8%).
